# guanjq/targetdiff

Hardware: NVIDIA H100
Metric: molecules/sec (1000-step sampling, CrossDocked pocket shape) (higher is better)
Workload: dtype f32 (storage, LayerNorm, softmax, accumulation); GEMM operands as 2-piece bf16 splits on wgmma (3 products, ~16-bit operand mantissa)

## Files before the change

include/tdiff.h:

```cpp
#ifndef TDIFF_H_
#define TDIFF_H_

#include <stddef.h>
#include <stdint.h>

#ifdef __cplusplus
extern "C" {
#endif

#if defined(__GNUC__)
#define TDIFF_API __attribute__((visibility("default")))
#else
#define TDIFF_API
#endif

#define TDIFF_OK 0
#define TDIFF_EINVAL (-1)
#define TDIFF_ECUDA (-2)
#define TDIFF_ESTATE (-3)
#define TDIFF_EWEIGHT (-4)

typedef struct tdiff_engine tdiff_engine;

typedef struct tdiff_config {
  int32_t hidden_dim;
  int32_t n_heads;
  int32_t num_layers;
  int32_t knn;
  int32_t num_r_gaussian;
  int32_t num_classes;
  int32_t protein_feat_dim;
  int32_t num_timesteps;
  int32_t model_mean_type;
  int32_t num_blocks;
  int32_t ew_net_type;
  int32_t x2h_out_fc;
  int32_t time_emb;
  int32_t cutoff_mode;
  int32_t sublayers;
  int32_t reserved[1];
} tdiff_config;

typedef struct tdiff_tensor {
  const char* name;
  const float* data;
  int64_t numel;
} tdiff_tensor;

TDIFF_API int tdiff_create(const tdiff_config* cfg, const tdiff_tensor* h_state_dict, int n_entries, int device, tdiff_engine** out);
TDIFF_API void tdiff_destroy(tdiff_engine* e);
TDIFF_API const char* tdiff_last_error(void);
TDIFF_API const char* tdiff_version(void);

TDIFF_API int tdiff_bind_batch(tdiff_engine* e, int n_graphs, const int32_t* h_protein_counts, const int32_t* h_ligand_counts,
                     const float* d_protein_pos, const float* d_protein_feat, int center_mode, void* stream);

TDIFF_API int tdiff_set_ligand(tdiff_engine* e, const float* d_ligand_pos, const int64_t* d_ligand_v, int apply_center, void* stream);
TDIFF_API int tdiff_get_ligand(tdiff_engine* e, float* d_ligand_pos, int64_t* d_ligand_v, int add_offset, void* stream);
TDIFF_API int tdiff_get_offset(tdiff_engine* e, float* d_offset, void* stream);

TDIFF_API int tdiff_set_time(tdiff_engine* e, const float* d_time_norm, void* stream);

TDIFF_API int tdiff_forward(tdiff_engine* e, float* d_pred_pos, float* d_pred_logits, float* d_final_h, int fix_x, void* stream);

TDIFF_API int tdiff_forward_blocks(tdiff_engine* e, float* d_pred_pos, float* d_pred_logits, float* d_final_h, int fix_x, float* d_block_pos,
                                   float* d_block_logits, void* stream);

TDIFF_API int64_t tdiff_num_edges(tdiff_engine* e, void* stream);
TDIFF_API int tdiff_get_edge_index(tdiff_engine* e, int64_t* d_edge_index, void* stream);
TDIFF_API int tdiff_get_edge_weight(tdiff_engine* e, float* d_e_w, void* stream);
TDIFF_API int tdiff_get_node_pos(tdiff_engine* e, float* d_x, void* stream);

TDIFF_API int tdiff_sample(tdiff_engine* e, int num_steps, const float* d_pos_noise, const float* d_v_uniform, uint64_t seed,
                 float* d_pos_traj, int64_t* d_v_traj, float* d_v0_traj, float* d_vt_traj, int pos_only, void* stream);

TDIFF_API int tdiff_set_fixed(tdiff_engine* e, const uint8_t* d_mask, const float* d_pos0, const int64_t* d_v0, int apply_center,
                              void* stream);
TDIFF_API int tdiff_set_fixed_tape(tdiff_engine* e, const float* d_pos_noise, const float* d_v_uniform);

TDIFF_API int tdiff_sample_seq(tdiff_engine* e, const int32_t* h_time_seq, int num_steps, const float* d_pos_noise, const float* d_v_uniform,
                               uint64_t seed, float* d_pos_traj, int64_t* d_v_traj, float* d_v0_traj, float* d_vt_traj, int pos_only,
                               void* stream);

TDIFF_API int tdiff_set_start(tdiff_engine* e, int t_start, const float* d_pos_noise, const float* d_v_uniform);

TDIFF_API int tdiff_likelihood_terms(tdiff_engine* e, const int32_t* h_time_steps, const uint32_t* h_keys, const float* d_pos_noise,
                                     const float* d_v_uniform, uint64_t seed, float* d_kl_pos, float* d_kl_v, float* d_prior_pos,
                                     float* d_prior_v, float* d_atom_kl_pos, float* d_atom_kl_v, float* d_xt, int64_t* d_vt, void* stream);

TDIFF_API int tdiff_sample_host(tdiff_engine* e, int n_graphs, const int32_t* h_protein_counts, const int32_t* h_ligand_counts,
                      const float* h_protein_pos, const float* h_protein_feat, const float* h_ligand_pos,
                      const int64_t* h_ligand_v, int center_mode, int num_steps, const float* h_pos_noise,
                      const float* h_v_uniform, uint64_t seed, float* h_out_pos, int64_t* h_out_v, float* h_pos_traj,
                      int64_t* h_v_traj, float* h_v0_traj, float* h_vt_traj, int pos_only, void* stream);

TDIFF_API int tdiff_knn_graph(const float* d_x, int n_nodes, const int32_t* h_graph_counts, int n_graphs, int k,
                    int32_t* d_src_slots, int64_t* d_edge_index, int64_t* h_n_edges, void* stream);

TDIFF_API int tdiff_attn_aggregate_h(const float* d_k, const float* d_v, const float* d_e_w, const int32_t* d_src_slots,
                           const float* d_q, const float* d_h_in, float* d_h_out, int n_nodes, int kk, void* stream);
TDIFF_API int tdiff_attn_aggregate_x(const float* d_k, const float* d_v16, const float* d_e_w, const int32_t* d_src_slots,
                           const float* d_q, const float* d_x, const uint8_t* d_mask, float* d_x_out, int n_nodes, int kk,
                           void* stream);
TDIFF_API int tdiff_scatter_mean3(const float* d_src, const int32_t* h_counts, int n_segments, float* d_out, void* stream);

TDIFF_API int tdiff_check_stability(const float* d_pos, const int32_t* d_atomic_num, const int32_t* h_counts, int n_mol, int hs,
                                    int32_t* d_nr_bonds, int32_t* d_stable_atoms, uint8_t* d_mol_stable, void* stream);

TDIFF_API int64_t tdiff_launch_count(tdiff_engine* e);
TDIFF_API int tdiff_edge_mlp_mode(tdiff_engine* e);
TDIFF_API int tdiff_profile(tdiff_engine* e, int enable);
TDIFF_API int tdiff_profile_read(tdiff_engine* e, double* ms_aggregate_h, int64_t* n_aggregate_h, double* ms_aggregate_x,
                       int64_t* n_aggregate_x, double* ms_edge_mlp, int64_t* n_edge_mlp, double* ms_total);

#ifdef __cplusplus
}
#endif
#endif
```

targetdiff_b200/_lib.py:

```python
import ctypes
import os

_HERE = os.path.dirname(os.path.abspath(__file__))
LIB_PATH = os.environ.get('TDIFF_LIB') or os.path.join(_HERE, 'libtdiff.so')

TDIFF_OK, TDIFF_EINVAL, TDIFF_ECUDA, TDIFF_ESTATE, TDIFF_EWEIGHT = 0, -1, -2, -3, -4


class TdiffError(RuntimeError):
    def __init__(self, code, msg):
        super().__init__('libtdiff error %d: %s' % (code, msg))
        self.code = code


class tdiff_config(ctypes.Structure):
    _fields_ = [('hidden_dim', ctypes.c_int32), ('n_heads', ctypes.c_int32), ('num_layers', ctypes.c_int32), ('knn', ctypes.c_int32),
                ('num_r_gaussian', ctypes.c_int32), ('num_classes', ctypes.c_int32), ('protein_feat_dim', ctypes.c_int32),
                ('num_timesteps', ctypes.c_int32), ('model_mean_type', ctypes.c_int32), ('num_blocks', ctypes.c_int32),
                ('ew_net_type', ctypes.c_int32), ('x2h_out_fc', ctypes.c_int32), ('time_emb', ctypes.c_int32), ('cutoff_mode', ctypes.c_int32),
                ('sublayers', ctypes.c_int32), ('reserved', ctypes.c_int32 * 1)]


class tdiff_tensor(ctypes.Structure):
    _fields_ = [('name', ctypes.c_char_p), ('data', ctypes.c_void_p), ('numel', ctypes.c_int64)]


_vp, _i, _i64, _u64 = ctypes.c_void_p, ctypes.c_int, ctypes.c_int64, ctypes.c_uint64
_pi32 = ctypes.POINTER(ctypes.c_int32)

SIGNATURES = {
    'tdiff_create': (_i, [ctypes.POINTER(tdiff_config), ctypes.POINTER(tdiff_tensor), _i, _i, ctypes.POINTER(_vp)]),
    'tdiff_destroy': (None, [_vp]),
    'tdiff_last_error': (ctypes.c_char_p, []),
    'tdiff_version': (ctypes.c_char_p, []),
    'tdiff_bind_batch': (_i, [_vp, _i, _pi32, _pi32, _vp, _vp, _i, _vp]),
    'tdiff_set_ligand': (_i, [_vp, _vp, _vp, _i, _vp]),
    'tdiff_get_ligand': (_i, [_vp, _vp, _vp, _i, _vp]),
    'tdiff_get_offset': (_i, [_vp, _vp, _vp]),
    'tdiff_set_time': (_i, [_vp, _vp, _vp]),
    'tdiff_forward': (_i, [_vp, _vp, _vp, _vp, _i, _vp]),
    'tdiff_forward_blocks': (_i, [_vp, _vp, _vp, _vp, _i, _vp, _vp, _vp]),
    'tdiff_num_edges': (_i64, [_vp, _vp]),
    'tdiff_get_edge_index': (_i, [_vp, _vp, _vp]),
    'tdiff_get_edge_weight': (_i, [_vp, _vp, _vp]),
    'tdiff_get_node_pos': (_i, [_vp, _vp, _vp]),
    'tdiff_sample': (_i, [_vp, _i, _vp, _vp, _u64, _vp, _vp, _vp, _vp, _i, _vp]),
    'tdiff_set_fixed': (_i, [_vp, _vp, _vp, _vp, _i, _vp]),
    'tdiff_set_fixed_tape': (_i, [_vp, _vp, _vp]),
    'tdiff_sample_seq': (_i, [_vp, _pi32, _i, _vp, _vp, _u64, _vp, _vp, _vp, _vp, _i, _vp]),
    'tdiff_set_start': (_i, [_vp, _i, _vp, _vp]),
    'tdiff_likelihood_terms': (_i, [_vp, _pi32, ctypes.POINTER(ctypes.c_uint32), _vp, _vp, _u64, _vp, _vp, _vp, _vp, _vp, _vp, _vp, _vp, _vp]),
    'tdiff_sample_host': (_i, [_vp, _i, _pi32, _pi32, _vp, _vp, _vp, _vp, _i, _i, _vp, _vp, _u64, _vp, _vp, _vp, _vp, _vp, _vp, _i, _vp]),
    'tdiff_knn_graph': (_i, [_vp, _i, _pi32, _i, _i, _vp, _vp, ctypes.POINTER(_i64), _vp]),
    'tdiff_attn_aggregate_h': (_i, [_vp, _vp, _vp, _vp, _vp, _vp, _vp, _i, _i, _vp]),
    'tdiff_attn_aggregate_x': (_i, [_vp, _vp, _vp, _vp, _vp, _vp, _vp, _vp, _i, _i, _vp]),
    'tdiff_scatter_mean3': (_i, [_vp, _pi32, _i, _vp, _vp]),
    'tdiff_check_stability': (_i, [_vp, _vp, _pi32, _i, _i, _vp, _vp, _vp, _vp]),
    'tdiff_launch_count': (_i64, [_vp]),
    'tdiff_edge_mlp_mode': (_i, [_vp]),
    'tdiff_profile': (_i, [_vp, _i]),
    'tdiff_profile_read': (_i, [_vp, ctypes.POINTER(ctypes.c_double), ctypes.POINTER(_i64), ctypes.POINTER(ctypes.c_double),
                                ctypes.POINTER(_i64), ctypes.POINTER(ctypes.c_double), ctypes.POINTER(_i64), ctypes.POINTER(ctypes.c_double)]),
}

_lib = None


def load():
    global _lib
    if _lib is not None:
        return _lib
    if not os.path.exists(LIB_PATH):
        raise RuntimeError('%s not found: build it with `python -m targetdiff_b200.build` (nvcc, sm_90a). '
                           'targetdiff_b200 has no CPU / PyTorch fallback.' % LIB_PATH)
    lib = ctypes.CDLL(LIB_PATH)
    for name, (res, args) in SIGNATURES.items():
        fn = getattr(lib, name)
        fn.restype = res
        fn.argtypes = args
    _lib = lib
    return lib


def last_error():
    return load().tdiff_last_error().decode('utf-8', 'replace')


def check(rc):
    if rc != TDIFF_OK:
        raise TdiffError(rc, last_error())


def i32_array(values):
    arr = (ctypes.c_int32 * len(values))(*[int(v) for v in values])
    return arr
```

targetdiff_b200/csrc/aggregate.cu:

```cuda
#include "tdiff_common.cuh"

#define AGG_WARPS 8
#define AGG_CH 8

__device__ __forceinline__ float4 ldg_stream4(const float* p) {
  float4 r;
  asm volatile("ld.global.nc.L1::no_allocate.v4.f32 {%0,%1,%2,%3}, [%4];" : "=f"(r.x), "=f"(r.y), "=f"(r.z), "=f"(r.w) : "l"(p));
  return r;
}

__device__ __forceinline__ float head_logit(const float4& q, const float4& k) {
  const float s8 = 2.8284271247461903f;
  float s = (__fdiv_rn(q.x * k.x, s8) + __fdiv_rn(q.y * k.y, s8)) + (__fdiv_rn(q.z * k.z, s8) + __fdiv_rn(q.w * k.w, s8));
  return s + __shfl_xor_sync(0xffffffffu, s, 1);
}

__global__ void __launch_bounds__(AGG_WARPS * 32)
aggregate_h_kernel(const float* __restrict__ kbuf, const float* __restrict__ vbuf, const float* __restrict__ e_w,
                   const int* __restrict__ src, const float* __restrict__ q, const float* __restrict__ h_in,
                   float* __restrict__ h_out, int n_nodes, int k) {
  const int lane = threadIdx.x & 31;
  const int n = blockIdx.x * AGG_WARPS + (threadIdx.x >> 5);
  if (n >= n_nodes) return;
  const size_t e0 = (size_t)n * k;
  int deg = 0;
  for (int j = lane; j < k; j += 32) deg += (src[e0 + j] >= 0);
  deg = __reduce_add_sync(0xffffffffu, deg);
  const float4 q4 = *reinterpret_cast<const float4*>(q + (size_t)n * TD_H + 4 * lane);
  const float4 hin = *reinterpret_cast<const float4*>(h_in + (size_t)n * TD_H + 4 * lane);
  float m = -INFINITY, l = 0.0f;
  float4 acc = make_float4(0.f, 0.f, 0.f, 0.f);
  for (int j0 = 0; j0 < deg; j0 += AGG_CH) {
    float4 kr[AGG_CH], vr[AGG_CH];
    float ew[AGG_CH];
#pragma unroll
    for (int c = 0; c < AGG_CH; ++c) {
      if (j0 + c < deg) {
        kr[c] = ldg_stream4(kbuf + (e0 + j0 + c) * TD_H + 4 * lane);
        vr[c] = ldg_stream4(vbuf + (e0 + j0 + c) * TD_H + 4 * lane);
        ew[c] = e_w[e0 + j0 + c];
      }
    }
#pragma unroll
    for (int c = 0; c < AGG_CH; ++c) {
      if (j0 + c < deg) {
        const float s = head_logit(q4, kr[c]);
        const float mn = fmaxf(m, s);
        const float sc = expf(m - mn);
        const float p = expf(s - mn);
        const float pw = p * ew[c];
        l = l * sc + p;
        acc.x = acc.x * sc + pw * vr[c].x;
        acc.y = acc.y * sc + pw * vr[c].y;
        acc.z = acc.z * sc + pw * vr[c].z;
        acc.w = acc.w * sc + pw * vr[c].w;
        m = mn;
      }
    }
  }
  float4 o = hin;
  if (deg > 0) {
    o.x += acc.x / l; o.y += acc.y / l; o.z += acc.z / l; o.w += acc.w / l;
  }
  *reinterpret_cast<float4*>(h_out + (size_t)n * TD_H + 4 * lane) = o;
}

void td_launch_aggregate_h(const float* kbuf, const float* vbuf, const float* e_w, const int* src, const float* q, const float* h_in,
                           float* h_out, int n_nodes, int k, cudaStream_t st) {
  if (n_nodes == 0) return;
  aggregate_h_kernel<<<(n_nodes + AGG_WARPS - 1) / AGG_WARPS, AGG_WARPS * 32, 0, st>>>(kbuf, vbuf, e_w, src, q, h_in, h_out, n_nodes, k);
}

__global__ void __launch_bounds__(AGG_WARPS * 32)
aggregate_x_kernel(const float* __restrict__ kbuf, const float* __restrict__ v16, const float* __restrict__ e_w,
                   const int* __restrict__ src, const float* __restrict__ q, const float4* __restrict__ xm_in,
                   const int* __restrict__ row_nodes, float4* __restrict__ xm_out, int n_rows, int k) {
  const int lane = threadIdx.x & 31;
  const int a = blockIdx.x * AGG_WARPS + (threadIdx.x >> 5);
  if (a >= n_rows) return;
  const int n = row_nodes ? row_nodes[a] : a;
  const size_t e0 = (size_t)n * k;
  const size_t r0 = (size_t)a * k;
  int deg = 0;
  for (int j = lane; j < k; j += 32) deg += (src[e0 + j] >= 0);
  deg = __reduce_add_sync(0xffffffffu, deg);
  const float4 q4 = *reinterpret_cast<const float4*>(q + (size_t)n * TD_H + 4 * lane);
  const float4 xd = xm_in[n];
  float m = -INFINITY, l = 0.0f;
  float ax = 0.f, ay = 0.f, az = 0.f;
  for (int j0 = 0; j0 < deg; j0 += AGG_CH) {
    float4 kr[AGG_CH];
    float vv[AGG_CH];
    float4 xs[AGG_CH];
#pragma unroll
    for (int c = 0; c < AGG_CH; ++c) {
      if (j0 + c < deg) {
        kr[c] = ldg_stream4(kbuf + (r0 + j0 + c) * TD_H + 4 * lane);
        vv[c] = v16[(r0 + j0 + c) * TD_HEADS + (lane >> 1)] * e_w[e0 + j0 + c];
        xs[c] = xm_in[src[e0 + j0 + c]];
      }
    }
#pragma unroll
    for (int c = 0; c < AGG_CH; ++c) {
      if (j0 + c < deg) {
        const float s = head_logit(q4, kr[c]);
        const float mn = fmaxf(m, s);
        const float sc = expf(m - mn);
        const float p = expf(s - mn);
        const float pv = p * vv[c];
        l = l * sc + p;
        ax = ax * sc + pv * (xd.x - xs[c].x);
        ay = ay * sc + pv * (xd.y - xs[c].y);
        az = az * sc + pv * (xd.z - xs[c].z);
        m = mn;
      }
    }
  }
  float dx = 0.f, dy = 0.f, dz = 0.f;
  if (deg > 0) {
    const float w = (lane & 1) ? 0.0f : 1.0f / l;
    dx = warp_sum(ax * w) * (1.0f / TD_HEADS);
    dy = warp_sum(ay * w) * (1.0f / TD_HEADS);
    dz = warp_sum(az * w) * (1.0f / TD_HEADS);
  }
  if (lane == 0) xm_out[n] = make_float4(xd.x + dx * xd.w, xd.y + dy * xd.w, xd.z + dz * xd.w, xd.w);
}

void td_launch_aggregate_x(const float* kbuf, const float* v16, const float* e_w, const int* src, const float* q, const float4* xm_in,
                           const int* row_nodes, float4* xm_out, int n_rows, int k, cudaStream_t st) {
  if (n_rows == 0) return;
  aggregate_x_kernel<<<(n_rows + AGG_WARPS - 1) / AGG_WARPS, AGG_WARPS * 32, 0, st>>>(kbuf, v16, e_w, src, q, xm_in, row_nodes, xm_out,
                                                                                   n_rows, k);
}

__global__ void __launch_bounds__(AGG_WARPS * 32)
aggregate_h_logits_kernel(const float* __restrict__ logits, const float* __restrict__ vbuf, const float* __restrict__ e_w,
                          const int* __restrict__ src, const float* __restrict__ h_in, float* __restrict__ h_out, int n_nodes, int k,
                          const float* __restrict__ ewm_w, float ewm_b) {
  const int lane = threadIdx.x & 31;
  const int n = blockIdx.x * AGG_WARPS + (threadIdx.x >> 5);
  if (n >= n_nodes) return;
  const size_t e0 = (size_t)n * k;
  int deg = 0;
  for (int j = lane; j < k; j += 32) deg += (src[e0 + j] >= 0);
  deg = __reduce_add_sync(0xffffffffu, deg);
  const float4 hin = *reinterpret_cast<const float4*>(h_in + (size_t)n * TD_H + 4 * lane);
  float4 wm = make_float4(0.f, 0.f, 0.f, 0.f);
  if (ewm_w) wm = *reinterpret_cast<const float4*>(ewm_w + 4 * lane);
  float m = -INFINITY, l = 0.0f;
  float4 acc = make_float4(0.f, 0.f, 0.f, 0.f);
  for (int j0 = 0; j0 < deg; j0 += AGG_CH) {
    float4 vr[AGG_CH];
    float ew[AGG_CH], sg[AGG_CH];
#pragma unroll
    for (int c = 0; c < AGG_CH; ++c) {
      if (j0 + c < deg) {
        vr[c] = ldg_stream4(vbuf + (e0 + j0 + c) * TD_H + 4 * lane);
        sg[c] = logits[(e0 + j0 + c) * TD_HEADS + (lane >> 1)];
        ew[c] = e_w[e0 + j0 + c];
      }
    }
    if (ewm_w) {
#pragma unroll
      for (int c = 0; c < AGG_CH; ++c) {
        if (j0 + c < deg) {
          const float dot = warp_sum((vr[c].x * wm.x + vr[c].y * wm.y) + (vr[c].z * wm.z + vr[c].w * wm.w));
          ew[c] = 1.0f / (1.0f + expf(-(dot + ewm_b)));
        }
      }
    }
#pragma unroll
    for (int c = 0; c < AGG_CH; ++c) {
      if (j0 + c < deg) {
        const float s = sg[c];
        const float mn = fmaxf(m, s);
        const float sc = expf(m - mn);
        const float p = expf(s - mn);
        const float pw = p * ew[c];
        l = l * sc + p;
        acc.x = acc.x * sc + pw * vr[c].x;
        acc.y = acc.y * sc + pw * vr[c].y;
        acc.z = acc.z * sc + pw * vr[c].z;
        acc.w = acc.w * sc + pw * vr[c].w;
        m = mn;
      }
    }
  }
  float4 o = hin;
  if (deg > 0) {
    o.x += acc.x / l; o.y += acc.y / l; o.z += acc.z / l; o.w += acc.w / l;
  }
  *reinterpret_cast<float4*>(h_out + (size_t)n * TD_H + 4 * lane) = o;
}

void td_launch_aggregate_h_logits(const float* logits, const float* vbuf, const float* e_w, const int* src, const float* h_in, float* h_out,
                                  int n_nodes, int k, const float* ewm_w, float ewm_b, cudaStream_t st) {
  if (n_nodes == 0) return;
  aggregate_h_logits_kernel<<<(n_nodes + AGG_WARPS - 1) / AGG_WARPS, AGG_WARPS * 32, 0, st>>>(logits, vbuf, e_w, src, h_in, h_out, n_nodes, k,
                                                                                             ewm_w, ewm_b);
}

__global__ void __launch_bounds__(AGG_WARPS * 32)
aggregate_x_logits_kernel(const float* __restrict__ logits, const float* __restrict__ v16, const float* __restrict__ e_w,
                          const int* __restrict__ src, const float4* __restrict__ xm_in, const int* __restrict__ row_nodes,
                          float4* __restrict__ xm_out, int n_rows, int k) {
  const int lane = threadIdx.x & 31;
  const int a = blockIdx.x * AGG_WARPS + (threadIdx.x >> 5);
  if (a >= n_rows) return;
  const int n = row_nodes ? row_nodes[a] : a;
  const size_t e0 = (size_t)n * k, r0 = (size_t)a * k;
  int deg = 0;
  for (int j = lane; j < k; j += 32) deg += (src[e0 + j] >= 0);
  deg = __reduce_add_sync(0xffffffffu, deg);
  const float4 xd = xm_in[n];
  float m = -INFINITY, l = 0.0f;
  float ax = 0.f, ay = 0.f, az = 0.f;
  for (int j = 0; j < deg; ++j) {
    const float s = logits[(r0 + j) * TD_HEADS + (lane >> 1)];
    const float vv = v16[(r0 + j) * TD_HEADS + (lane >> 1)] * e_w[e0 + j];
    const float4 xs = xm_in[src[e0 + j]];
    const float mn = fmaxf(m, s);
    const float sc = expf(m - mn);
    const float p = expf(s - mn);
    const float pv = p * vv;
    l = l * sc + p;
    ax = ax * sc + pv * (xd.x - xs.x);
    ay = ay * sc + pv * (xd.y - xs.y);
    az = az * sc + pv * (xd.z - xs.z);
    m = mn;
  }
  float dx = 0.f, dy = 0.f, dz = 0.f;
  if (deg > 0) {
    const float w = (lane & 1) ? 0.0f : 1.0f / l;
    dx = warp_sum(ax * w) * (1.0f / TD_HEADS);
    dy = warp_sum(ay * w) * (1.0f / TD_HEADS);
    dz = warp_sum(az * w) * (1.0f / TD_HEADS);
  }
  if (lane == 0) xm_out[n] = make_float4(xd.x + dx * xd.w, xd.y + dy * xd.w, xd.z + dz * xd.w, xd.w);
}

void td_launch_aggregate_x_logits(const float* logits, const float* v16, const float* e_w, const int* src, const float4* xm_in,
                                  const int* row_nodes, float4* xm_out, int n_rows, int k, cudaStream_t st) {
  if (n_rows == 0) return;
  aggregate_x_logits_kernel<<<(n_rows + AGG_WARPS - 1) / AGG_WARPS, AGG_WARPS * 32, 0, st>>>(logits, v16, e_w, src, xm_in, row_nodes, xm_out,
                                                                                          n_rows, k);
}
```

targetdiff_b200/csrc/edge_const.cu:

```cuda
#include "tdiff_common.cuh"

#define EC_WARPS 8

__global__ void __launch_bounds__(EC_WARPS * 32)
edge_touch_kernel(const float4* __restrict__ xm, const int* __restrict__ src, int* __restrict__ src_prev, int have_prev, int n_nodes, int k,
                  unsigned char* __restrict__ rel_flag, unsigned char* __restrict__ touch_flag, unsigned char* __restrict__ etype,
                  int* __restrict__ work_list, int* __restrict__ n_work) {
  const int lane = threadIdx.x & 31;
  const int warp0 = blockIdx.x * EC_WARPS + (threadIdx.x >> 5), nwarps = gridDim.x * EC_WARPS;
  for (int node = warp0; node < n_nodes; node += nwarps) {
    const size_t e0 = (size_t)node * k;
    const float4 xd = xm[node];
    bool same = have_prev != 0, touch = xd.w != 0.0f;
    unsigned keep_mask = 0;
    for (int j = lane; j < k; j += 32) {
      const int s = src[e0 + j];
      bool slot_same = false;
      if (src_prev) {
        slot_same = have_prev != 0 && src_prev[e0 + j] == s;
        same = same && slot_same;
        src_prev[e0 + j] = s;
      }
      const bool s_lig = s >= 0 && xm[s].w != 0.0f;
      if (slot_same && !s_lig && xd.w == 0.0f) keep_mask |= 1u << (j >> 5);
      touch = touch || s_lig;
      if (rel_flag && xd.w != 0.0f && s >= 0) rel_flag[s] = 1;
    }
    if (rel_flag && xd.w != 0.0f && lane == 0) rel_flag[node] = 1;
    same = __all_sync(0xffffffffu, same);
    touch = __any_sync(0xffffffffu, touch);
    if (touch_flag && lane == 0) touch_flag[node] = touch ? 1 : 0;
    if (same && !touch) continue;
    if (etype)
      for (int j = lane; j < k; j += 32)
        if (keep_mask & (1u << (j >> 5))) etype[e0 + j] |= 0x80;
    if (lane == 0) work_list[atomicAdd(n_work, 1)] = node;
  }
}

__global__ void __launch_bounds__(EC_WARPS * 32)
edge_gate_kernel(const float4* __restrict__ xm, const int* __restrict__ src, const int* __restrict__ work_list, const int* __restrict__ n_work,
                 int k, const float* __restrict__ offsets, float coeff, const float* __restrict__ w1t, const float* __restrict__ b1,
                 const float* __restrict__ ln_g, const float* __restrict__ ln_b, const float* __restrict__ w2, float b2,
                 unsigned char* __restrict__ etype, float* __restrict__ e_w, int gate_mode, int honour_keep) {
  __shared__ float s_w1t[TD_NG * TD_H];
  __shared__ float s_b1[TD_H], s_g[TD_H], s_b[TD_H], s_w2[TD_H];
  for (int i = threadIdx.x; i < TD_NG * TD_H; i += blockDim.x) s_w1t[i] = w1t[i];
  for (int i = threadIdx.x; i < TD_H; i += blockDim.x) {
    s_b1[i] = b1[i]; s_g[i] = ln_g[i]; s_b[i] = ln_b[i]; s_w2[i] = w2[i];
  }
  __syncthreads();
  const int lane = threadIdx.x & 31;
  const float mu = offsets[lane < TD_NG ? lane : 0];
  const long long warp0 = (long long)blockIdx.x * EC_WARPS + (threadIdx.x >> 5), nwarps = (long long)gridDim.x * EC_WARPS;
  const long long n_items = (long long)(*n_work) * k;
  for (long long item = warp0; item < n_items; item += nwarps) {
    const int node = work_list[item / k];
    const size_t e = (size_t)node * k + (size_t)(item % k);
    const unsigned char keep = honour_keep ? etype[e] : 0;
    if (keep & 0x80) {
      if (lane == 0) etype[e] = keep & 0x7f;
      continue;
    }
    const int s = src[e];
    if (s < 0) {
      if (lane == 0) { etype[e] = 3; e_w[e] = 0.0f; }
      continue;
    }
    const float4 xd = xm[node], xs = xm[s];
    if (gate_mode != 0) {
      if (lane == 0) {
        const bool ns = xs.w != 0.0f, nd = xd.w != 0.0f;
        etype[e] = (unsigned char)(ns ? (nd ? 0 : 1) : (nd ? 2 : 3));
        e_w[e] = 1.0f;
      }
      continue;
    }
    const float dx = xd.x - xs.x, dy = xd.y - xs.y, dz = xd.z - xs.z;
    const float dist = sqrtf(dx * dx + dy * dy + dz * dz);
    const float t = dist - mu;
    const float gj = expf(coeff * (t * t));
    float p[4];
#pragma unroll
    for (int c = 0; c < 4; ++c) p[c] = s_b1[lane + 32 * c];
#pragma unroll
    for (int jj = 0; jj < TD_NG; ++jj) {
      const float g = __shfl_sync(0xffffffffu, gj, jj);
#pragma unroll
      for (int c = 0; c < 4; ++c) p[c] = fmaf(g, s_w1t[jj * TD_H + lane + 32 * c], p[c]);
    }
    ln_relu_128(p, s_g, s_b, lane);
    float acc = (p[0] * s_w2[lane] + p[1] * s_w2[lane + 32]) + (p[2] * s_w2[lane + 64] + p[3] * s_w2[lane + 96]);
    acc = warp_sum(acc) + b2;
    if (lane == 0) {
      const bool ns = xs.w != 0.0f, nd = xd.w != 0.0f;
      const int ty = ns ? (nd ? 0 : 1) : (nd ? 2 : 3);
      etype[e] = (unsigned char)ty;
      e_w[e] = 1.0f / (1.0f + expf(-acc));
    }
  }
}

void td_launch_edge_const(const float4* xm, const int* src, int* src_prev, int have_prev, int n_nodes, int k, const float* offsets, float coeff,
                          const float* w1t, const float* b1, const float* ln_g, const float* ln_b, const float* w2, float b2,
                          unsigned char* etype, float* e_w, unsigned char* rel_flag, unsigned char* touch_flag, int* work_list, int* n_work,
                          int gate_mode, cudaStream_t st) {
  if (n_nodes == 0) return;
  int blocks = (n_nodes + EC_WARPS - 1) / EC_WARPS;
  if (blocks > 148 * 8) blocks = 148 * 8;
  if (rel_flag) cudaMemsetAsync(rel_flag, 0, (size_t)n_nodes, st);
  cudaMemsetAsync(n_work, 0, sizeof(int), st);
  edge_touch_kernel<<<blocks, EC_WARPS * 32, 0, st>>>(xm, src, src_prev, have_prev, n_nodes, k, rel_flag, touch_flag, (gate_mode & 2) ? nullptr : etype,
                                                      work_list, n_work);
  edge_gate_kernel<<<148 * 8, EC_WARPS * 32, 0, st>>>(xm, src, work_list, n_work, k, offsets, coeff, w1t, b1, ln_g, ln_b, w2, b2, etype, e_w, gate_mode & 1,
                                                     (have_prev && !(gate_mode & 2)) ? 1 : 0);
}

__global__ void edge_geom_kernel(const float4* __restrict__ xm, const int* __restrict__ src, const unsigned char* __restrict__ etype, long long n_slots,
                                 int k, float* __restrict__ dist, TdEwR ew) {
  const long long e = (long long)blockIdx.x * blockDim.x + threadIdx.x;
  if (e >= n_slots) return;
  const int s = src[e];
  float d = 0.0f;
  if (s >= 0) {
    const float4 xd = xm[e / k], xs = xm[s];
    const float dx = xd.x - xs.x, dy = xd.y - xs.y, dz = xd.z - xs.z;
    d = sqrtf(dx * dx + dy * dy + dz * dz);
  }
  dist[e] = d;
  if (ew.w_x2h) {
    float ax = ew.b_x2h, ah = ew.b_h2x;
    if (s >= 0) {
      const int ty = etype[e];
#pragma unroll 4
      for (int j = 0; j < TD_NG; ++j) {
        const float t = d - ew.offsets[j];
        const float g = expf(ew.coeff * (t * t));
        ax = fmaf(g, ew.w_x2h[ty * TD_NG + j], ax);
        ah = fmaf(g, ew.w_h2x[ty * TD_NG + j], ah);
      }
    }
    ew.out_x2h[e] = s >= 0 ? 1.0f / (1.0f + expf(-ax)) : 0.0f;
    ew.out_h2x[e] = s >= 0 ? 1.0f / (1.0f + expf(-ah)) : 0.0f;
  }
}

void td_launch_edge_geom(const float4* xm, const int* src, const unsigned char* etype, int n_nodes, int k, float* dist, const TdEwR& ew, cudaStream_t st) {
  const long long n = (long long)n_nodes * k;
  if (n > 0) edge_geom_kernel<<<(int)((n + 255) / 256), 256, 0, st>>>(xm, src, etype, n, k, dist, ew);
}

__global__ void edge_geom_rows_kernel(const float4* __restrict__ xm, const int* __restrict__ src, const unsigned char* __restrict__ etype,
                                      const int* __restrict__ rows, long long n_slots, int k, float* __restrict__ dist,
                                      const float* __restrict__ gate_w, float gate_b, const float* __restrict__ offsets, float coeff,
                                      float* __restrict__ gate) {
  const long long t = (long long)blockIdx.x * blockDim.x + threadIdx.x;
  if (t >= n_slots) return;
  const long long e = (long long)rows[t / k] * k + t % k;
  const int s = src[e];
  float d = 0.0f;
  if (s >= 0) {
    const float4 xd = xm[e / k], xs = xm[s];
    const float dx = xd.x - xs.x, dy = xd.y - xs.y, dz = xd.z - xs.z;
    d = sqrtf(dx * dx + dy * dy + dz * dz);
  }
  dist[e] = d;
  if (gate_w) {
    float a = gate_b;
    if (s >= 0) {
      const int ty = etype[e];
#pragma unroll 4
      for (int j = 0; j < TD_NG; ++j) {
        const float u = d - offsets[j];
        a = fmaf(expf(coeff * (u * u)), gate_w[ty * TD_NG + j], a);
      }
    }
    gate[e] = s >= 0 ? 1.0f / (1.0f + expf(-a)) : 0.0f;
  }
}

void td_launch_edge_geom_rows(const float4* xm, const int* src, const unsigned char* etype, const int* rows, int n_rows, int k, float* dist,
                              const float* gate_w, float gate_b, const float* offsets, float coeff, float* gate, cudaStream_t st) {
  const long long n = (long long)n_rows * k;
  if (n > 0) edge_geom_rows_kernel<<<(int)((n + 255) / 256), 256, 0, st>>>(xm, src, etype, rows, n, k, dist, gate_w, gate_b, offsets, coeff, gate);
}

__global__ void rel_compact_kernel(const unsigned char* __restrict__ flag, int n_nodes, int* __restrict__ rel_list, int* __restrict__ n_rel) {
  const int i = blockIdx.x * blockDim.x + threadIdx.x;
  if (i < n_nodes && flag[i]) rel_list[atomicAdd(n_rel, 1)] = i;
}
void td_launch_rel_compact(const unsigned char* flag, int n_nodes, int* rel_list, int* n_rel, cudaStream_t st) {
  if (n_nodes == 0) return;
  cudaMemsetAsync(n_rel, 0, sizeof(int), st);
  rel_compact_kernel<<<(n_nodes + 255) / 256, 256, 0, st>>>(flag, n_nodes, rel_list, n_rel);
}

__global__ void rel_rows_protein_kernel(const unsigned char* __restrict__ flag, const float4* __restrict__ xm, int n_nodes, int* __restrict__ rel_rows,
                                        int* __restrict__ rel_counts) {
  const int i = blockIdx.x * blockDim.x + threadIdx.x;
  if (i < n_nodes && flag[i] && xm[i].w == 0.0f) rel_rows[atomicAdd(&rel_counts[2], 1)] = i;
}
__global__ void rel_rows_finish_kernel(const int* __restrict__ lig_rows, int n_lig_rows, int pad, int* __restrict__ rel_rows, int* __restrict__ rel_counts) {
  const int n_p = rel_counts[2], n_pp = (n_p + pad - 1) / pad * pad;
  const int i = blockIdx.x * blockDim.x + threadIdx.x;
  if (i < n_pp - n_p) rel_rows[n_p + i] = -1;
  if (i < n_lig_rows) rel_rows[n_pp + i] = lig_rows[i];
  if (i == 0) { rel_counts[0] = n_pp + n_lig_rows; rel_counts[1] = n_pp; }
}
void td_launch_rel_rows(const unsigned char* rel_flag, const float4* xm, int n_nodes, const int* lig_rows, int n_lig_rows, int pad, int* rel_rows,
                        int* rel_counts, cudaStream_t st) {
  cudaMemsetAsync(rel_counts, 0, 4 * sizeof(int), st);
  if (n_nodes > 0) rel_rows_protein_kernel<<<(n_nodes + 255) / 256, 256, 0, st>>>(rel_flag, xm, n_nodes, rel_rows, rel_counts);
  const int n = n_lig_rows > pad ? n_lig_rows : pad;
  rel_rows_finish_kernel<<<(n + 255) / 256, 256, 0, st>>>(lig_rows, n_lig_rows, pad, rel_rows, rel_counts);
}

__global__ void dirty_propagate_kernel(const unsigned char* __restrict__ in, const int* __restrict__ src, int n_nodes, int k, unsigned char* __restrict__ out) {
  const int lane = threadIdx.x & 31;
  const int node = blockIdx.x * (blockDim.x >> 5) + (threadIdx.x >> 5);
  if (node >= n_nodes) return;
  bool d = in[node] != 0;
  for (int j = lane; j < k && !d; j += 32) {
    const int s = src[(size_t)node * k + j];
    if (s >= 0 && in[s]) d = true;
  }
  d = __any_sync(0xffffffffu, d);
  if (lane == 0) out[node] = d ? 1 : 0;
}
void td_launch_dirty_propagate(const unsigned char* in, const int* src, int n_nodes, int k, unsigned char* out, cudaStream_t st) {
  if (n_nodes > 0) dirty_propagate_kernel<<<(n_nodes + 7) / 8, 256, 0, st>>>(in, src, n_nodes, k, out);
}
__global__ void restore_clean_kernel(const unsigned char* __restrict__ dirty, const float4* __restrict__ xm, const float* __restrict__ h_free, int n_nodes,
                                     float* __restrict__ h) {
  const int lane = threadIdx.x & 31;
  const int node = blockIdx.x * (blockDim.x >> 5) + (threadIdx.x >> 5);
  if (node >= n_nodes || dirty[node] || xm[node].w != 0.0f) return;
  reinterpret_cast<float4*>(h + (size_t)node * TD_H)[lane] = reinterpret_cast<const float4*>(h_free + (size_t)node * TD_H)[lane];
}
void td_launch_restore_clean(const unsigned char* dirty, const float4* xm, const float* h_free, int n_nodes, float* h, cudaStream_t st) {
  if (n_nodes > 0) restore_clean_kernel<<<(n_nodes + 7) / 8, 256, 0, st>>>(dirty, xm, h_free, n_nodes, h);
}
```

targetdiff_b200/csrc/engine.cu:

```cuda
#include <math.h>
#include <stdarg.h>
#include <stdio.h>
#include <stdlib.h>
#include <string.h>

#include <list>
#include <map>
#include <string>
#include <vector>

#include "../../include/tdiff.h"
#include "sampler.cuh"
#include "tdiff_common.cuh"

static thread_local char g_err[1024] = "";
static int set_err(int code, const char* fmt, ...) {
  va_list ap;
  va_start(ap, fmt);
  vsnprintf(g_err, sizeof(g_err), fmt, ap);
  va_end(ap);
  return code;
}
#define CK(call)                                                                                       \
  do {                                                                                                 \
    cudaError_t _e = (call);                                                                           \
    if (_e != cudaSuccess) return set_err(TDIFF_ECUDA, "%s failed: %s (%s:%d)", #call, cudaGetErrorString(_e), __FILE__, __LINE__); \
  } while (0)

struct DevBuf {
  void* p = nullptr;
  size_t cap = 0;
  int ensure(size_t bytes) {
    if (bytes <= cap) return 0;
    if (p) cudaFree(p);
    p = nullptr; cap = 0;
    size_t want = bytes + bytes / 8 + 256;
    if (cudaMalloc(&p, want) != cudaSuccess) { (void)cudaGetLastError(); if (cudaMalloc(&p, bytes) != cudaSuccess) { (void)cudaGetLastError(); return -1; } want = bytes; }
    cap = want;
    static const bool poison = getenv("TDIFF_POISON") != nullptr;
    if (poison) {
      cudaMemset(p, 0xFF, want);
      cudaDeviceSynchronize();
    }
    return 0;
  }
  void release() { if (p) cudaFree(p); p = nullptr; cap = 0; }
  template <class T> T* as() const { return reinterpret_cast<T*>(p); }
};

struct TdLayer {
  std::vector<TdSubLayer> x2h, h2x;
  const float* offsets;
  float coeff;
};

enum { EV_AGG_H = 0, EV_AGG_X = 1, EV_EDGE_MLP = 2, EV_TOTAL = 3, EV_KINDS = 4 };
struct EvPair { cudaEvent_t a, b; int kind; };

struct tdiff_engine {
  tdiff_config cfg;
  int device = 0, sm_count = 132;
  float* arena = nullptr;
  std::vector<float> host_arena;
  unsigned char* img_arena = nullptr;
  int mlp_mode = 2;
  bool mlp_v4 = true;
  std::vector<TdLayer> layers;
  const float *w_prot = nullptr, *b_prot = nullptr, *wl_t = nullptr, *bl = nullptr;
  const float *ew_w1t = nullptr, *ew_b1 = nullptr, *ew_g = nullptr, *ew_b = nullptr, *ew_w2 = nullptr, *ew_off = nullptr;
  float ew_b2 = 0.f, ew_coeff = -0.5f;
  int num_blocks = 1, ew_mode = 0 , out_fc = 0, time_emb = 0;
  int num_x2h = 1, num_h2x = 1, sync_twoup = 0;
  const float* w_time = nullptr;
  const float* zeros128 = nullptr;
  DevBuf ew_x2h, ew_h2x, hagg, time_norm;
  DevBuf h_sync;
  const float *hd_w1t = nullptr, *hd_b1 = nullptr, *hd_w2 = nullptr, *hd_b2 = nullptr;
  const float *t_c0 = nullptr, *t_ct = nullptr, *t_logvar = nullptr, *t_la = nullptr, *t_l1ma = nullptr, *t_lca = nullptr, *t_l1mca = nullptr,
              *t_sra = nullptr, *t_srm1 = nullptr, *t_ac = nullptr;
  bool bound = false, has_ligand = false, have_graph = false;
  bool restrict_last = false;
  bool knn_incremental = false;
  bool have_prev = false;
  bool env_no_fused_agg = false, env_no_restrict = false, env_no_graph = false, env_knn_full = false, env_no_slot_keep = false;
  int B = 0, N = 0, Np = 0, Nl = 0, K = 0, max_ng = 0, final_buf = 0;
  int KQ = 0, hybrid = 0;
  DevBuf node_ptr, prot_ptr, prot_node, prot_graph, lig_node, lig_graph, node_lig;
  DevBuf rel_flag, rel_list, n_rel, work_list, n_work, knn_cache;
  DevBuf x2h_rows, lig_rows, rel_rows, rel_counts;
  long long x2h_n_dst = 0, x2h_split = 0, lig_n_dst = 0;
  int row_pad = 4;
  int free_depth = 0;
  int env_free_depth = 2;
  bool free_ready = false;
  DevBuf h_free, dirty, free_rows, free_counts, lig_save;
  long long free_stride = 0;
  DevBuf xm0, xm1, offset, h0, h, P, q, src, src_prev, etype, e_w, dist, kbuf, vbuf, v16, lig_pos, lig_v, logits;
  DevBuf step, err_flag, node_off, total_edges;
  bool has_fixed = false;
  DevBuf fix_mask, fix_pos, fix_v;
  const float *fix_pos_noise = nullptr, *fix_v_uniform = nullptr;
  int start_t = -1;
  const float *start_pos_noise = nullptr, *start_v_uniform = nullptr;
  std::vector<double> cum_log_a, cum_log_av;
  DevBuf seq_buf;
  DevBuf lk_buf, lk_x0, lk_v0;
  std::vector<int32_t> lk_host;
  DevBuf stage[8];
  cudaStream_t own_stream = nullptr;
  cudaEvent_t ev_fork = nullptr, ev_join = nullptr;
  long long launches = 0;
  bool profiling = false;
  std::vector<EvPair> events;
  double ms_acc[EV_KINDS] = {0, 0, 0, 0};
  long long n_acc[EV_KINDS] = {0, 0, 0, 0};
};

namespace {
struct Packer {
  std::map<std::string, const tdiff_tensor*> byname;
  std::vector<float> host;
  std::vector<unsigned char> img;
  std::string missing;
  std::list<std::vector<float>> keep;
  const float* get(const std::string& name, int64_t numel) {
    auto it = byname.find(name);
    if (it == byname.end() || it->second->numel != numel || it->second->data == nullptr) {
      if (missing.empty()) missing = name + (it == byname.end() ? " (absent)" : " (wrong size)");
      return nullptr;
    }
    return it->second->data;
  }
  size_t alloc(size_t n) {
    size_t off = (host.size() + 63) / 64 * 64;
    host.resize(off + n, 0.0f);
    return off;
  }
};

struct MlpOff { size_t tab, ln_g, ln_b, w2t, b2; int nout; long long img, tabcls; };

inline uint16_t bf16_rn(float x) {
  uint32_t u; memcpy(&u, &x, 4);
  if ((u & 0x7fffffffu) > 0x7f800000u) return (uint16_t)((u >> 16) | 0x40);
  u += 0x7fffu + ((u >> 16) & 1u);
  return (uint16_t)(u >> 16);
}
inline float bf16_f(uint16_t b) { uint32_t u = (uint32_t)b << 16; float f; memcpy(&f, &u, 4); return f; }

void pack_umma_image(const float* w2, std::vector<unsigned char>& img, size_t off, int nrows = 128) {
  for (int n = 0; n < nrows; ++n)
    for (int kk = 0; kk < 128; ++kk) {
      float r = w2[(size_t)n * 128 + kk];
      const size_t o = (size_t)(kk / 64) * ((size_t)nrows * 128) + (size_t)n * 128 + (size_t)((((kk % 64) / 8) ^ (n & 7)) * 16) + (size_t)(kk % 8) * 2;
      for (int p = 0; p < 3; ++p) {
        const uint16_t b = bf16_rn(r);
        r = r - bf16_f(b);
        memcpy(&img[off + (size_t)p * ((size_t)nrows * 256) + o], &b, 2);
      }
    }
}

void pack_tabcls_image(const float* tab , std::vector<unsigned char>& img, size_t off) {
  static const int type_of[2][2] = {{3, 1}, {2, 0}};
  for (int cls = 0; cls < 2; ++cls)
    for (int n = 0; n < 128; ++n)
      for (int slot = 0; slot < 64; ++slot) {
        const int half = slot >> 5, sl = slot & 31;
        const int q = (sl & 7) >> 1, m = 2 * (sl >> 3) + (sl & 1);
        int j = -1;
        if (m < 5) j = 5 * q + m;
        else if (m == 5 && q == 3) j = 20;
        float r = j >= 0 ? tab[((size_t)type_of[cls][half] * TD_TAB + j) * TD_H + n] : 0.0f;
        const size_t o = (size_t)n * 128 + (size_t)(((slot >> 3) ^ (n & 7)) * 16) + (size_t)(slot & 7) * 2;
        for (int p = 0; p < 2; ++p) {
          const uint16_t b = bf16_rn(r);
          r = r - bf16_f(b);
          memcpy(&img[off + (size_t)cls * 32768 + (size_t)p * 16384 + o], &b, 2);
        }
      }
}

bool pack_edge_mlp(Packer& pk, const std::string& p, int nout, bool sign_in_w1, MlpOff& o, const float** w1_out) {
  const int KV = 4 + 4 * TD_NG + 2 * TD_H;
  const float* w1_in = pk.get(p + ".net.0.weight", (int64_t)TD_H * KV);
  const float* b1_in = pk.get(p + ".net.0.bias", TD_H);
  const float* g_in = pk.get(p + ".net.1.weight", TD_H);
  const float* b_in = pk.get(p + ".net.1.bias", TD_H);
  const float* w2_in = pk.get(p + ".net.3.weight", (int64_t)nout * TD_H);
  const float* b2_in = pk.get(p + ".net.3.bias", nout);
  if (!w1_in || !b1_in || !g_in || !b_in || !w2_in || !b2_in) return false;
  std::vector<float>& w1v = pk.keep.emplace_back((size_t)TD_H * KV);
  std::vector<float> b1v(TD_H), gv(TD_H), bv(TD_H), w2v((size_t)nout * TD_H), b2v(nout);
  {
    std::vector<double> mw(KV, 0.0), b2acc(b2_in, b2_in + nout);
    double mb = 0.0;
    for (int f = 0; f < TD_H; ++f) {
      for (int j = 0; j < KV; ++j) mw[j] += w1_in[(size_t)f * KV + j];
      mb += b1_in[f];
    }
    for (int f = 0; f < TD_H; ++f) {
      const double s = g_in[f] < 0.0f ? -1.0 : 1.0, ag = fabs((double)g_in[f]), s1 = sign_in_w1 ? s : 1.0;
      for (int j = 0; j < KV; ++j) w1v[(size_t)f * KV + j] = (float)(s1 * (w1_in[(size_t)f * KV + j] - mw[j] / TD_H));
      b1v[f] = (float)(s1 * (b1_in[f] - mb / TD_H));
      gv[f] = (float)(s / s1);
      const float bf = (float)(b_in[f] / ag);
      const bool constant = g_in[f] == 0.0f || !isfinite(bf);
      bv[f] = constant ? 0.0f : bf;
      for (int n = 0; n < nout; ++n) {
        const double w = w2_in[(size_t)n * TD_H + f];
        w2v[(size_t)n * TD_H + f] = constant ? 0.0f : (float)(ag * w);
        if (constant && b_in[f] > 0.0f) b2acc[n] += (double)b_in[f] * w;
      }
    }
    for (int n = 0; n < nout; ++n) b2v[n] = (float)b2acc[n];
  }
  const float *w1 = w1v.data(), *b1 = b1v.data(), *g = gv.data(), *b = bv.data(), *w2 = w2v.data(), *b2 = b2v.data();
  o.nout = nout;
  o.tab = pk.alloc(4 * TD_TAB * TD_H);
  for (int t = 0; t < 4; ++t) {
    for (int j = 0; j < TD_NG; ++j)
      for (int f = 0; f < TD_H; ++f) pk.host[o.tab + (t * TD_TAB + j) * TD_H + f] = w1[(size_t)f * KV + 4 + t * TD_NG + j];
    for (int f = 0; f < TD_H; ++f) pk.host[o.tab + (t * TD_TAB + TD_NG) * TD_H + f] = w1[(size_t)f * KV + t] + b1[f];
  }
  o.ln_g = pk.alloc(TD_H); memcpy(&pk.host[o.ln_g], g, TD_H * sizeof(float));
  o.ln_b = pk.alloc(TD_H); memcpy(&pk.host[o.ln_b], b, TD_H * sizeof(float));
  o.w2t = pk.alloc((size_t)TD_H * nout);
  for (int kk = 0; kk < TD_H; ++kk)
    for (int n = 0; n < nout; ++n) pk.host[o.w2t + (size_t)kk * nout + n] = w2[(size_t)n * TD_H + kk];
  o.b2 = pk.alloc(nout); memcpy(&pk.host[o.b2], b2, nout * sizeof(float));
  o.img = -1; o.tabcls = -1;
  if (nout == TD_H || nout == 16) {
    o.img = (long long)pk.img.size();
    pk.img.resize(pk.img.size() + 3 * (size_t)nout * 256, 0);
    pack_umma_image(w2, pk.img, (size_t)o.img, nout);
    o.tabcls = (long long)pk.img.size();
    pk.img.resize(pk.img.size() + 2 * 32768, 0);
    pack_tabcls_image(&pk.host[o.tab], pk.img, (size_t)o.tabcls);
  }
  *w1_out = w1;
  return true;
}

struct SubOff {
  size_t wn_t, bn; long long wn_img; MlpOff k, v, q;
  long long ew_w = -1; float ew_b = 0.f;
  long long out_wa = -1, out_wb = -1, out_w2 = -1, out_b1 = -1, out_g = -1, out_b = -1, out_b2 = -1;
};

bool pack_sublayer_options(Packer& pk, const std::string& p, int ew_dim, bool out_fc, SubOff& so) {
  if (ew_dim > 0) {
    const float* w = pk.get(p + ".ew_net.0.weight", ew_dim);
    const float* b = pk.get(p + ".ew_net.0.bias", 1);
    if (!w || !b) return false;
    so.ew_w = (long long)pk.alloc(ew_dim);
    memcpy(&pk.host[so.ew_w], w, ew_dim * sizeof(float));
    so.ew_b = b[0];
  }
  if (out_fc) {
    const std::string np = p + ".node_output";
    const float* w1 = pk.get(np + ".net.0.weight", (int64_t)TD_H * 2 * TD_H);
    const float* b1 = pk.get(np + ".net.0.bias", TD_H);
    const float* g = pk.get(np + ".net.1.weight", TD_H);
    const float* b = pk.get(np + ".net.1.bias", TD_H);
    const float* w2 = pk.get(np + ".net.3.weight", (int64_t)TD_H * TD_H);
    const float* b2 = pk.get(np + ".net.3.bias", TD_H);
    if (!w1 || !b1 || !g || !b || !w2 || !b2) return false;
    std::vector<float> blk((size_t)TD_H * TD_H);
    for (int half = 0; half < 2; ++half) {
      for (int n = 0; n < TD_H; ++n)
        for (int kk = 0; kk < TD_H; ++kk) blk[(size_t)n * TD_H + kk] = w1[(size_t)n * 2 * TD_H + half * TD_H + kk];
      long long& dst = half == 0 ? so.out_wa : so.out_wb;
      dst = (long long)pk.img.size();
      pk.img.resize(pk.img.size() + 3 * 32768, 0);
      pack_umma_image(blk.data(), pk.img, (size_t)dst);
    }
    so.out_w2 = (long long)pk.img.size();
    pk.img.resize(pk.img.size() + 3 * 32768, 0);
    pack_umma_image(w2, pk.img, (size_t)so.out_w2);
    so.out_b1 = (long long)pk.alloc(TD_H); memcpy(&pk.host[so.out_b1], b1, TD_H * 4);
    so.out_g = (long long)pk.alloc(TD_H); memcpy(&pk.host[so.out_g], g, TD_H * 4);
    so.out_b = (long long)pk.alloc(TD_H); memcpy(&pk.host[so.out_b], b, TD_H * 4);
    so.out_b2 = (long long)pk.alloc(TD_H); memcpy(&pk.host[so.out_b2], b2, TD_H * 4);
  }
  return true;
}

bool pack_sublayer(Packer& pk, const std::string& p, const char* kn, const char* vn, const char* qn, int nout_v, bool sign_in_w1, SubOff& so) {
  const int KV = 4 + 4 * TD_NG + 2 * TD_H;
  const float *w1k = nullptr, *w1v = nullptr;
  if (!pack_edge_mlp(pk, p + "." + kn, TD_H, sign_in_w1, so.k, &w1k)) return false;
  if (!pack_edge_mlp(pk, p + "." + vn, nout_v, sign_in_w1, so.v, &w1v)) return false;
  const std::string qp = p + "." + qn;
  const float* w1q = pk.get(qp + ".net.0.weight", (int64_t)TD_H * TD_H);
  const float* b1q = pk.get(qp + ".net.0.bias", TD_H);
  const float* gq = pk.get(qp + ".net.1.weight", TD_H);
  const float* bq = pk.get(qp + ".net.1.bias", TD_H);
  const float* w2q = pk.get(qp + ".net.3.weight", (int64_t)TD_H * TD_H);
  const float* b2q = pk.get(qp + ".net.3.bias", TD_H);
  if (!w1q || !b1q || !gq || !bq || !w2q || !b2q) return false;
  so.q.nout = TD_H; so.q.tab = 0; so.q.tabcls = -1;
  so.q.img = (long long)pk.img.size();
  pk.img.resize(pk.img.size() + 3 * 32768, 0);
  pack_umma_image(w2q, pk.img, (size_t)so.q.img);
  so.q.ln_g = pk.alloc(TD_H); memcpy(&pk.host[so.q.ln_g], gq, TD_H * sizeof(float));
  so.q.ln_b = pk.alloc(TD_H); memcpy(&pk.host[so.q.ln_b], bq, TD_H * sizeof(float));
  so.q.w2t = pk.alloc((size_t)TD_H * TD_H);
  for (int kk = 0; kk < TD_H; ++kk)
    for (int n = 0; n < TD_H; ++n) pk.host[so.q.w2t + (size_t)kk * TD_H + n] = w2q[(size_t)n * TD_H + kk];
  so.q.b2 = pk.alloc(TD_H); memcpy(&pk.host[so.q.b2], b2q, TD_H * sizeof(float));
  so.wn_t = pk.alloc((size_t)TD_H * TD_NPROJ);
  so.bn = pk.alloc(TD_NPROJ);
  for (int kk = 0; kk < TD_H; ++kk) {
    float* row = &pk.host[so.wn_t + (size_t)kk * TD_NPROJ];
    for (int c = 0; c < TD_H; ++c) {
      row[c] = w1k[(size_t)c * KV + 4 + 4 * TD_NG + kk];
      row[128 + c] = w1v[(size_t)c * KV + 4 + 4 * TD_NG + kk];
      row[256 + c] = w1k[(size_t)c * KV + 4 + 4 * TD_NG + TD_H + kk];
      row[384 + c] = w1v[(size_t)c * KV + 4 + 4 * TD_NG + TD_H + kk];
      row[512 + c] = w1q[(size_t)c * TD_H + kk];
    }
  }
  for (int c = 0; c < TD_H; ++c) pk.host[so.bn + 512 + c] = b1q[c];
  so.wn_img = (long long)pk.img.size();
  pk.img.resize(pk.img.size() + 5 * 3 * 32768, 0);
  std::vector<float> blk((size_t)TD_H * TD_H);
  for (int y = 0; y < 5; ++y) {
    for (int n = 0; n < TD_H; ++n)
      for (int kk = 0; kk < TD_H; ++kk) blk[(size_t)n * TD_H + kk] = pk.host[so.wn_t + (size_t)kk * TD_NPROJ + y * TD_H + n];
    pack_umma_image(blk.data(), pk.img, (size_t)so.wn_img + (size_t)y * 3 * 32768);
  }
  return true;
}

TdMlp mk_mlp(const float* base, const unsigned char* img_base, const MlpOff& o, int offA, int offB) {
  TdMlp m;
  m.w2_img = (o.img >= 0 && img_base) ? img_base + o.img : nullptr;
  m.tabcls_img = (o.tabcls >= 0 && img_base) ? img_base + o.tabcls : nullptr;
  m.tab = base + o.tab; m.ln_g = base + o.ln_g; m.ln_b = base + o.ln_b; m.w2t = base + o.w2t; m.b2 = base + o.b2;
  m.nout = o.nout; m.offA = offA; m.offB = offB;
  return m;
}
}

extern "C" const char* tdiff_last_error(void) { return g_err; }
extern "C" const char* tdiff_version(void) { return "tdiff-b200 0.1 (sm_90a)"; }

extern "C" int tdiff_create(const tdiff_config* cfg, const tdiff_tensor* sd, int n_entries, int device, tdiff_engine** out) {
  if (!cfg || !sd || !out) return set_err(TDIFF_EINVAL, "null argument");
  *out = nullptr;
  if (cfg->hidden_dim != TD_H || cfg->n_heads != TD_HEADS || cfg->num_r_gaussian != TD_NG)
    return set_err(TDIFF_EINVAL, "unsupported model shape: hidden_dim=%d n_heads=%d num_r_gaussian=%d (kernels are built for 128/16/20)",
                   cfg->hidden_dim, cfg->n_heads, cfg->num_r_gaussian);
  if (cfg->knn < 1 || cfg->knn > TD_KMAX) return set_err(TDIFF_EINVAL, "knn=%d outside 1..%d", cfg->knn, TD_KMAX);
  if (cfg->model_mean_type != 0 && cfg->model_mean_type != 1)
    return set_err(TDIFF_EINVAL, "model_mean_type=%d (0 = C0, 1 = noise)", cfg->model_mean_type);
  for (int r : cfg->reserved)
    if (r != 0) return set_err(TDIFF_EINVAL, "tdiff_config.reserved must be 0");
  int num_x2h = 1, num_h2x = 1, sync_twoup = 0;
  if (cfg->sublayers != 0) {
    const unsigned s = (unsigned)cfg->sublayers;
    num_x2h = (int)(s & 0xffu); num_h2x = (int)((s >> 8) & 0xffu); sync_twoup = (int)((s >> 16) & 0xffu);
    if ((s >> 24) != 1u || num_x2h > 16 || num_h2x > 16 || sync_twoup > 1)
      return set_err(TDIFF_EINVAL, "sublayers=0x%08x: expected 0 or 1<<24 | sync_twoup<<16 | num_h2x<<8 | num_x2h with num_x2h, num_h2x in 0..16 and "
                     "sync_twoup in 0..1", s);
  }
  if (cfg->cutoff_mode != 0 && cfg->cutoff_mode != 1) return set_err(TDIFF_EINVAL, "cutoff_mode=%d (0 = 'knn', 1 = 'hybrid')", cfg->cutoff_mode);
  if (cfg->num_blocks < 0 || cfg->num_blocks > 16 || cfg->ew_net_type < 0 || cfg->ew_net_type > 3 || (cfg->x2h_out_fc != 0 && cfg->x2h_out_fc != 1) ||
      (cfg->time_emb != 0 && cfg->time_emb != 1))
    return set_err(TDIFF_EINVAL, "bad option (num_blocks=%d ew_net_type=%d x2h_out_fc=%d time_emb=%d)", cfg->num_blocks, cfg->ew_net_type,
                   cfg->x2h_out_fc, cfg->time_emb);
  if (cfg->num_layers < 1 || cfg->num_classes < 1 || cfg->num_classes > TD_CMAX || cfg->protein_feat_dim < 1 || cfg->num_timesteps < 1)
    return set_err(TDIFF_EINVAL, "bad config (num_layers=%d num_classes=%d protein_feat_dim=%d num_timesteps=%d)", cfg->num_layers,
                   cfg->num_classes, cfg->protein_feat_dim, cfg->num_timesteps);
  int ndev = 0;
  if (cudaGetDeviceCount(&ndev) != cudaSuccess || ndev == 0) {
    (void)cudaGetLastError();
    return set_err(TDIFF_ECUDA, "no CUDA device: libtdiff has no CPU fallback");
  }
  if (device < 0 || device >= ndev) return set_err(TDIFF_EINVAL, "device %d out of range (%d devices)", device, ndev);
  CK(cudaSetDevice(device));
  cudaDeviceProp prop;
  CK(cudaGetDeviceProperties(&prop, device));
  if (prop.major != 9) return set_err(TDIFF_ECUDA, "device %d is sm_%d%d; this library is built for sm_90a only", device, prop.major, prop.minor);

  tdiff_engine* e = new tdiff_engine();
  e->cfg = *cfg; e->device = device; e->sm_count = prop.multiProcessorCount; e->K = e->KQ = cfg->knn; e->hybrid = cfg->cutoff_mode;
  e->num_blocks = cfg->num_blocks > 1 ? cfg->num_blocks : 1; e->ew_mode = cfg->ew_net_type; e->out_fc = cfg->x2h_out_fc; e->time_emb = cfg->time_emb;
  e->num_x2h = num_x2h; e->num_h2x = num_h2x; e->sync_twoup = sync_twoup;
  if (const char* mode = getenv("TDIFF_EDGE_MLP")) {
    if (!strcmp(mode, "simt")) e->mlp_mode = 0;
    else if (!strcmp(mode, "tc3")) e->mlp_mode = 2;
    else if (!strcmp(mode, "tc3v2")) { e->mlp_mode = 2; e->mlp_v4 = false; }
    else if (!strcmp(mode, "tc6")) e->mlp_mode = 3;
    else { delete e; return set_err(TDIFF_EINVAL, "TDIFF_EDGE_MLP=%s (simt|tc3|tc3v2|tc6)", mode); }
  }
  const bool v4 = e->mlp_mode == 2 && e->mlp_v4;

  Packer pk;
  for (int i = 0; i < n_entries; ++i)
    if (sd[i].name) pk.byname[sd[i].name] = &sd[i];
  const int T = cfg->num_timesteps, KC = cfg->num_classes, F = cfg->protein_feat_dim, L = cfg->num_layers;
  struct { const char* name; size_t off; } tabs[10] = {{"posterior_mean_c0_coef", 0}, {"posterior_mean_ct_coef", 0}, {"posterior_logvar", 0},
      {"log_alphas_v", 0}, {"log_one_minus_alphas_v", 0}, {"log_alphas_cumprod_v", 0}, {"log_one_minus_alphas_cumprod_v", 0},
      {"sqrt_recip_alphas_cumprod", 0}, {"sqrt_recipm1_alphas_cumprod", 0}, {"alphas_cumprod", 0}};
  for (auto& t : tabs) {
    const float* p = pk.get(t.name, T);
    t.off = pk.alloc(T);
    if (p) memcpy(&pk.host[t.off], p, T * sizeof(float));
  }
  const float *betas = pk.get("betas", T), *la_v = pk.get("log_alphas_v", T);
  if (betas && la_v) {
    e->cum_log_a.resize(T); e->cum_log_av.resize(T);
    double sa = 0.0, sv = 0.0;
    for (int i = 0; i < T; ++i) {
      sa += log1p(-(double)betas[i]); e->cum_log_a[i] = sa;
      sv += (double)la_v[i]; e->cum_log_av[i] = sv;
    }
  }
  const float* wp = pk.get("protein_atom_emb.weight", (int64_t)(TD_H - 1) * F);
  const float* bp = pk.get("protein_atom_emb.bias", TD_H - 1);
  const int KIN = KC + (cfg->time_emb ? 1 : 0);
  const float* wl = pk.get("ligand_atom_emb.weight", (int64_t)(TD_H - 1) * KIN);
  const float* blp = pk.get("ligand_atom_emb.bias", TD_H - 1);
  size_t o_wp = pk.alloc((size_t)TD_H * F), o_bp = pk.alloc(TD_H), o_wl = pk.alloc((size_t)KC * TD_H), o_bl = pk.alloc(TD_H),
         o_wtime = pk.alloc(TD_H), o_zeros = pk.alloc(TD_H);
  if (wp && bp && wl && blp) {
    memcpy(&pk.host[o_wp], wp, (size_t)(TD_H - 1) * F * sizeof(float));
    memcpy(&pk.host[o_bp], bp, (TD_H - 1) * sizeof(float));
    for (int v = 0; v < KC; ++v)
      for (int f = 0; f < TD_H - 1; ++f) pk.host[o_wl + (size_t)v * TD_H + f] = wl[(size_t)f * KIN + v];
    if (cfg->time_emb)
      for (int f = 0; f < TD_H - 1; ++f) pk.host[o_wtime + f] = wl[(size_t)f * KIN + KC];
    memcpy(&pk.host[o_bl], blp, (TD_H - 1) * sizeof(float));
  }
  const bool has_gate = cfg->ew_net_type == 0;
  const float* gw1 = has_gate ? pk.get("refine_net.edge_pred_layer.net.0.weight", (int64_t)TD_H * TD_NG) : nullptr;
  const float* gb1 = has_gate ? pk.get("refine_net.edge_pred_layer.net.0.bias", TD_H) : nullptr;
  const float* gg = has_gate ? pk.get("refine_net.edge_pred_layer.net.1.weight", TD_H) : nullptr;
  const float* gb = has_gate ? pk.get("refine_net.edge_pred_layer.net.1.bias", TD_H) : nullptr;
  const float* gw2 = has_gate ? pk.get("refine_net.edge_pred_layer.net.3.weight", TD_H) : nullptr;
  const float* gb2 = has_gate ? pk.get("refine_net.edge_pred_layer.net.3.bias", 1) : nullptr;
  const float* goff = pk.get("refine_net.distance_expansion.offset", TD_NG);
  size_t o_gw1 = pk.alloc((size_t)TD_NG * TD_H), o_gb1 = pk.alloc(TD_H), o_gg = pk.alloc(TD_H), o_gb = pk.alloc(TD_H), o_gw2 = pk.alloc(TD_H),
         o_goff = pk.alloc(TD_NG);
  if (goff) memcpy(&pk.host[o_goff], goff, TD_NG * 4);
  if (gw1 && gb1 && gg && gb && gw2 && gb2 && goff) {
    for (int j = 0; j < TD_NG; ++j)
      for (int f = 0; f < TD_H; ++f) pk.host[o_gw1 + (size_t)j * TD_H + f] = gw1[(size_t)f * TD_NG + j];
    memcpy(&pk.host[o_gb1], gb1, TD_H * 4); memcpy(&pk.host[o_gg], gg, TD_H * 4); memcpy(&pk.host[o_gb], gb, TD_H * 4);
    memcpy(&pk.host[o_gw2], gw2, TD_H * 4); memcpy(&pk.host[o_goff], goff, TD_NG * 4);
    e->ew_b2 = gb2[0];
    const float d = goff[1] - goff[0];
    e->ew_coeff = -0.5f / (d * d);
  }
  const float* hw1 = pk.get("v_inference.0.weight", (int64_t)TD_H * TD_H);
  const float* hb1 = pk.get("v_inference.0.bias", TD_H);
  const float* hw2 = pk.get("v_inference.2.weight", (int64_t)KC * TD_H);
  const float* hb2 = pk.get("v_inference.2.bias", KC);
  size_t o_hw1 = pk.alloc((size_t)TD_H * TD_H), o_hb1 = pk.alloc(TD_H), o_hw2 = pk.alloc((size_t)KC * TD_H), o_hb2 = pk.alloc(KC);
  if (hw1 && hb1 && hw2 && hb2) {
    for (int kk = 0; kk < TD_H; ++kk)
      for (int n = 0; n < TD_H; ++n) pk.host[o_hw1 + (size_t)kk * TD_H + n] = hw1[(size_t)n * TD_H + kk];
    memcpy(&pk.host[o_hb1], hb1, TD_H * 4); memcpy(&pk.host[o_hw2], hw2, (size_t)KC * TD_H * 4); memcpy(&pk.host[o_hb2], hb2, KC * 4);
  }
  std::vector<std::vector<SubOff>> sx(L, std::vector<SubOff>(num_x2h)), sh(L, std::vector<SubOff>(num_h2x));
  std::vector<size_t> o_off(L);
  std::vector<float> coeffs(L, -0.5f);
  for (int l = 0; l < L; ++l) {
    const std::string p = "refine_net.base_block." + std::to_string(l);
    bool ok = true;
    for (int i = 0; ok && i < num_x2h; ++i) ok = pack_sublayer(pk, p + ".x2h_layers." + std::to_string(i), "hk_func", "hv_func", "hq_func", TD_H, v4, sx[l][i]);
    for (int i = 0; ok && i < num_h2x; ++i) ok = pack_sublayer(pk, p + ".h2x_layers." + std::to_string(i), "xk_func", "xv_func", "xq_func", TD_HEADS, v4, sh[l][i]);
    for (int i = 0; ok && i < num_x2h; ++i)
      ok = pack_sublayer_options(pk, p + ".x2h_layers." + std::to_string(i), cfg->ew_net_type == 1 ? 4 * TD_NG : cfg->ew_net_type == 2 ? TD_H : 0,
                                 cfg->x2h_out_fc != 0, sx[l][i]);
    for (int i = 0; ok && i < num_h2x; ++i)
      ok = pack_sublayer_options(pk, p + ".h2x_layers." + std::to_string(i), cfg->ew_net_type == 1 ? 4 * TD_NG : 0, false, sh[l][i]);
    if (!ok) break;
    const float* off = pk.get(p + ".distance_expansion.offset", TD_NG);
    o_off[l] = pk.alloc(TD_NG);
    if (off) {
      memcpy(&pk.host[o_off[l]], off, TD_NG * 4);
      const float d = off[1] - off[0];
      coeffs[l] = -0.5f / (d * d);
    }
  }
  if (!pk.missing.empty()) {
    delete e;
    return set_err(TDIFF_EWEIGHT, "state_dict entry %s", pk.missing.c_str());
  }
  const size_t bytes = pk.host.size() * sizeof(float);
  if (cudaMalloc(&e->arena, bytes) != cudaSuccess) { delete e; return set_err(TDIFF_ECUDA, "cudaMalloc(%zu) for weights failed", bytes); }
  if (cudaMemcpy(e->arena, pk.host.data(), bytes, cudaMemcpyHostToDevice) != cudaSuccess) {
    cudaFree(e->arena); delete e; return set_err(TDIFF_ECUDA, "weight upload failed");
  }
  if (!pk.img.empty()) {
    if (cudaMalloc(&e->img_arena, pk.img.size()) != cudaSuccess ||
        cudaMemcpy(e->img_arena, pk.img.data(), pk.img.size(), cudaMemcpyHostToDevice) != cudaSuccess) {
      cudaFree(e->arena); delete e; return set_err(TDIFF_ECUDA, "weight image upload failed");
    }
  }
  if ((cfg->ew_net_type != 0 || cfg->x2h_out_fc || cfg->cutoff_mode != 0) && !(e->mlp_mode == 2 && e->mlp_v4)) {
    cudaFree(e->arena); cudaFree(e->img_arena); delete e;
    return set_err(TDIFF_EINVAL, "ew_net_type != 'global', x2h_out_fc and cutoff_mode 'hybrid' are implemented (and tested) in the default engine mode only (unset TDIFF_EDGE_MLP)");
  }
  if (cfg->sublayers != 0 && !(num_x2h == 1 && num_h2x == 1 && !sync_twoup) && !(e->mlp_mode == 2 && e->mlp_v4)) {
    cudaFree(e->arena); cudaFree(e->img_arena); delete e;
    return set_err(TDIFF_EINVAL, "num_x2h / num_h2x != 1 and sync_twoup are implemented (and tested) in the default engine mode only (unset TDIFF_EDGE_MLP)");
  }
  e->env_no_fused_agg = getenv("TDIFF_NO_FUSED_AGG") != nullptr;
  e->env_no_restrict = getenv("TDIFF_NO_RESTRICT") != nullptr;
  e->env_no_graph = getenv("TDIFF_NO_GRAPH") != nullptr;
  e->env_knn_full = getenv("TDIFF_KNN_FULL") != nullptr;
  e->env_no_slot_keep = getenv("TDIFF_NO_SLOT_KEEP") != nullptr;
  if (const char* fd = getenv("TDIFF_FREE_DEPTH")) e->env_free_depth = atoi(fd) < 0 ? 0 : (atoi(fd) > 8 ? 8 : atoi(fd));
  e->host_arena = pk.host;
  const float* A = e->arena;
  const unsigned char* IM = e->img_arena;
  e->t_c0 = A + tabs[0].off; e->t_ct = A + tabs[1].off; e->t_logvar = A + tabs[2].off; e->t_la = A + tabs[3].off;
  e->t_l1ma = A + tabs[4].off; e->t_lca = A + tabs[5].off; e->t_l1mca = A + tabs[6].off;
  e->t_sra = A + tabs[7].off; e->t_srm1 = A + tabs[8].off; e->t_ac = A + tabs[9].off;
  e->w_prot = A + o_wp; e->b_prot = A + o_bp; e->wl_t = A + o_wl; e->bl = A + o_bl;
  e->w_time = cfg->time_emb ? A + o_wtime : nullptr; e->zeros128 = A + o_zeros;
  e->ew_w1t = A + o_gw1; e->ew_b1 = A + o_gb1; e->ew_g = A + o_gg; e->ew_b = A + o_gb; e->ew_w2 = A + o_gw2; e->ew_off = A + o_goff;
  e->hd_w1t = A + o_hw1; e->hd_b1 = A + o_hb1; e->hd_w2 = A + o_hw2; e->hd_b2 = A + o_hb2;
  e->layers.resize(L);
  for (int l = 0; l < L; ++l) {
    TdLayer& ly = e->layers[l];
    ly.offsets = A + o_off[l]; ly.coeff = coeffs[l];
    ly.x2h.resize(num_x2h); ly.h2x.resize(num_h2x);
    for (int idx = 0; idx < num_x2h + num_h2x; ++idx) {
      const bool is_h2x = idx >= num_x2h;
      TdSubLayer& sl = is_h2x ? ly.h2x[idx - num_x2h] : ly.x2h[idx];
      const SubOff& so = is_h2x ? sh[l][idx - num_x2h] : sx[l][idx];
      sl.wn_t = A + so.wn_t; sl.bn = A + so.bn; sl.wn_img = IM ? IM + so.wn_img : nullptr;
      sl.k = mk_mlp(A, IM, so.k, 0, 256); sl.v = mk_mlp(A, IM, so.v, 128, 384); sl.q = mk_mlp(A, IM, so.q, 512, 512);
      sl.ew_w = so.ew_w >= 0 ? A + so.ew_w : nullptr; sl.ew_b = so.ew_b;
      sl.out_wa_img = so.out_wa >= 0 ? IM + so.out_wa : nullptr; sl.out_wb_img = so.out_wb >= 0 ? IM + so.out_wb : nullptr;
      sl.out_b1 = so.out_b1 >= 0 ? A + so.out_b1 : nullptr;
      memset(&sl.out, 0, sizeof(sl.out));
      if (so.out_w2 >= 0) {
        sl.out.w2_img = IM + so.out_w2; sl.out.ln_g = A + so.out_g; sl.out.ln_b = A + so.out_b; sl.out.b2 = A + so.out_b2; sl.out.nout = TD_H;
      }
    }
  }
  if (e->step.ensure(sizeof(int)) || e->err_flag.ensure(sizeof(int)) || e->total_edges.ensure(sizeof(long long))) {
    tdiff_destroy(e); return set_err(TDIFF_ECUDA, "cudaMalloc failed");
  }
  cudaMemset(e->err_flag.p, 0, sizeof(int));
  if (cudaStreamCreateWithFlags(&e->own_stream, cudaStreamNonBlocking) != cudaSuccess ||
      cudaEventCreateWithFlags(&e->ev_fork, cudaEventDisableTiming) != cudaSuccess ||
      cudaEventCreateWithFlags(&e->ev_join, cudaEventDisableTiming) != cudaSuccess) {
    tdiff_destroy(e); return set_err(TDIFF_ECUDA, "stream/event creation failed");
  }
  *out = e;
  return TDIFF_OK;
}

extern "C" void tdiff_destroy(tdiff_engine* e) {
  if (!e) return;
  cudaSetDevice(e->device);
  for (auto& ev : e->events) { cudaEventDestroy(ev.a); cudaEventDestroy(ev.b); }
  if (e->own_stream) cudaStreamDestroy(e->own_stream);
  if (e->ev_fork) cudaEventDestroy(e->ev_fork);
  if (e->ev_join) cudaEventDestroy(e->ev_join);
  DevBuf* bufs[] = {&e->node_ptr, &e->prot_ptr, &e->prot_node, &e->prot_graph, &e->lig_node, &e->lig_graph, &e->node_lig, &e->xm0, &e->xm1,
                    &e->rel_flag, &e->rel_list, &e->n_rel, &e->work_list, &e->n_work, &e->knn_cache, &e->x2h_rows, &e->lig_rows, &e->rel_rows, &e->rel_counts, &e->ew_x2h, &e->ew_h2x, &e->h_sync, &e->hagg, &e->time_norm, &e->h_free, &e->dirty, &e->free_rows, &e->free_counts, &e->lig_save, &e->offset, &e->h0, &e->h, &e->P, &e->q, &e->src, &e->src_prev, &e->etype, &e->e_w, &e->dist, &e->kbuf, &e->vbuf, &e->v16, &e->lig_pos,
                    &e->lig_v, &e->logits, &e->step, &e->err_flag, &e->node_off, &e->total_edges, &e->fix_mask, &e->fix_pos, &e->fix_v, &e->seq_buf, &e->lk_buf, &e->lk_x0, &e->lk_v0};
  for (auto* b : bufs) b->release();
  for (auto& b : e->stage) b.release();
  if (e->arena) cudaFree(e->arena);
  if (e->img_arena) cudaFree(e->img_arena);
  delete e;
}

extern "C" int tdiff_bind_batch(tdiff_engine* e, int B, const int32_t* pc, const int32_t* lc, const float* d_ppos, const float* d_pfeat,
                                int center_mode, void* stream) {
  if (!e || !pc || !lc || B < 1) return set_err(TDIFF_EINVAL, "bind_batch: bad arguments");
  if (center_mode != 0 && center_mode != 1) return set_err(TDIFF_EINVAL, "center_mode %d (0 'none' | 1 'protein')", center_mode);
  cudaStream_t st = (cudaStream_t)stream;
  CK(cudaSetDevice(e->device));
  long long N = 0, Np = 0, Nl = 0;
  int max_ng = 0;
  for (int g = 0; g < B; ++g) {
    if (pc[g] < 0 || lc[g] < 0) return set_err(TDIFF_EINVAL, "negative atom count in graph %d", g);
    Np += pc[g]; Nl += lc[g];
    if (pc[g] + lc[g] > max_ng) max_ng = pc[g] + lc[g];
  }
  N = Np + Nl;
  if (N <= 0) return set_err(TDIFF_EINVAL, "empty batch");
  int K = e->KQ;
  if (e->hybrid) {
    int max_lc = 0;
    for (int g = 0; g < B; ++g) {
      if (lc[g] > max_lc) max_lc = lc[g];
      if (lc[g] > 0 && pc[g] < e->KQ)
        return set_err(TDIFF_EINVAL, "cutoff_mode 'hybrid': graph %d has %d protein atoms < k = %d (torch.topk fails in the reference too)", g, pc[g], e->KQ);
    }
    K = e->KQ + (max_lc > 0 ? max_lc - 1 : 0);
    if (K > TD_KMAX)
      return set_err(TDIFF_EINVAL, "cutoff_mode 'hybrid': k + n_ligand - 1 = %d + %d - 1 exceeds the %d neighbour slots per node", e->KQ, max_lc, TD_KMAX);
  }
  if (N * (long long)K >= (1LL << 31) / 1) return set_err(TDIFF_EINVAL, "batch too large: N*k = %lld edge slots", N * K);
  if (max_ng > 2800) return set_err(TDIFF_EINVAL, "graph with %d nodes exceeds the k-NN kernel's shared-memory tile (2800)", max_ng);
  if (Np > 0 && (!d_ppos || !d_pfeat)) return set_err(TDIFF_EINVAL, "null protein arrays");
  e->K = K;
  std::vector<int> node_ptr(B + 1), prot_ptr(B + 1), prot_node(Np), prot_graph(Np), lig_node(Nl), lig_graph(Nl), node_lig(N, -1);
  int n = 0, p = 0, a = 0;
  for (int g = 0; g < B; ++g) {
    node_ptr[g] = n; prot_ptr[g] = p;
    for (int i = 0; i < pc[g]; ++i) { prot_node[p] = n; prot_graph[p] = g; ++p; ++n; }
    for (int i = 0; i < lc[g]; ++i) { lig_node[a] = n; lig_graph[a] = g; node_lig[n] = a; ++a; ++n; }
  }
  node_ptr[B] = n; prot_ptr[B] = p;
  e->bound = false; e->has_ligand = false; e->have_graph = false; e->have_prev = false;
  e->has_fixed = false; e->fix_pos_noise = nullptr; e->fix_v_uniform = nullptr;
  e->start_t = -1; e->start_pos_noise = nullptr; e->start_v_uniform = nullptr;
  e->B = B; e->N = (int)N; e->Np = (int)Np; e->Nl = (int)Nl; e->max_ng = max_ng;
  const size_t slots = (size_t)N * K;
  int bad = 0;
  bad |= e->node_ptr.ensure((B + 1) * 4) | e->prot_ptr.ensure((B + 1) * 4) | e->prot_node.ensure(Np * 4 + 4) | e->prot_graph.ensure(Np * 4 + 4);
  bad |= e->lig_node.ensure(Nl * 4 + 4) | e->lig_graph.ensure(Nl * 4 + 4) | e->node_lig.ensure(N * 4);
  bad |= e->xm0.ensure(N * 16) | e->xm1.ensure(N * 16) | e->offset.ensure((size_t)B * 16);
  bad |= e->h0.ensure(N * TD_H * 4) | e->h.ensure(N * TD_H * 4) | e->P.ensure((size_t)(N + 1) * TD_NPROJ * 4) | e->q.ensure(N * TD_H * 4);
  bad |= e->src.ensure(slots * 4) | e->src_prev.ensure(slots * 4) | e->etype.ensure(slots) | e->e_w.ensure(slots * 4) | e->dist.ensure(slots * 4);
  const bool v4 = e->mlp_mode == 2 && e->mlp_v4;
  int gcd128 = 128;
  while (K % gcd128) gcd128 >>= 1;
  e->row_pad = 128 / gcd128;
  const long long pad = e->row_pad, nPpad = (Np + pad - 1) / pad * pad, nLpad = (Nl + pad - 1) / pad * pad;
  e->x2h_n_dst = nPpad + nLpad; e->x2h_split = nPpad; e->lig_n_dst = nLpad;
  std::vector<int> x2h_rows((size_t)(nPpad + nLpad), -1), lig_rows((size_t)nLpad, -1);
  for (long long i = 0; i < Np; ++i) x2h_rows[i] = prot_node[i];
  for (long long i = 0; i < Nl; ++i) { x2h_rows[nPpad + i] = lig_node[i]; lig_rows[i] = lig_node[i]; }
  if (v4) bad |= e->x2h_rows.ensure(x2h_rows.size() * 4 + 4) | e->lig_rows.ensure(lig_rows.size() * 4 + 4) | e->rel_rows.ensure(x2h_rows.size() * 4 + 4) |
                 e->rel_counts.ensure(16);
  const bool fuse = v4 && K == 32 && !e->env_no_fused_agg && e->ew_mode != 2;
  if (e->ew_mode == 1) bad |= e->ew_x2h.ensure(slots * 4) | e->ew_h2x.ensure(slots * 4);
  if (e->out_fc) bad |= e->hagg.ensure((size_t)N * TD_H * 4);
  if (e->sync_twoup && e->num_x2h > 0 && e->num_h2x > 0) bad |= e->h_sync.ensure((size_t)N * TD_H * 4);
  if (e->time_emb) bad |= e->time_norm.ensure((size_t)B * 4 + 16);
  bad |= e->kbuf.ensure(v4 ? (size_t)(nPpad + nLpad) * K * TD_HEADS * 4 + 64 : slots * TD_H * 4);
  if (!fuse) bad |= e->vbuf.ensure(slots * TD_H * 4);
  bad |= e->v16.ensure((size_t)nLpad * K * TD_HEADS * 4 + 16);
  int min_pc = 1 << 30;
  for (int g = 0; g < B; ++g) if (pc[g] < min_pc) min_pc = pc[g];
  e->free_ready = false;
  e->free_depth = (fuse && !e->hybrid && Nl > 0 && min_pc > K) ? e->env_free_depth : 0;
  const int x2h_evals = (int)e->layers.size() * e->num_x2h;
  if (e->free_depth > x2h_evals - 1) e->free_depth = x2h_evals - 1 > 0 ? x2h_evals - 1 : 0;
  if (e->free_depth > 0)
    bad |= e->h_free.ensure((size_t)e->free_depth * N * TD_H * 4) | e->dirty.ensure((size_t)e->free_depth * N + 16) |
           e->free_rows.ensure((size_t)e->free_depth * x2h_rows.size() * 4 + 4) | e->free_counts.ensure((size_t)e->free_depth * 16) |
           e->lig_save.ensure((size_t)Nl * 20 + 32);
  e->free_stride = (long long)x2h_rows.size();
  bad |= e->lig_pos.ensure(Nl * 16 + 16) | e->lig_v.ensure(Nl * 4 + 4) | e->logits.ensure((size_t)Nl * e->cfg.num_classes * 4 + 4);
  bad |= e->node_off.ensure(N * 8) | e->rel_flag.ensure(N + 16) | e->rel_list.ensure(N * 4 + 64) | e->n_rel.ensure(16) | e->work_list.ensure(N * 4 + 64) | e->n_work.ensure(16);
  e->knn_incremental = !e->env_knn_full && Np > 0;
  if (e->knn_incremental) bad |= e->knn_cache.ensure((size_t)N * (e->KQ + 1) * 8);
  if (bad) return set_err(TDIFF_ECUDA, "out of device memory binding a batch of %lld nodes (%zu edge slots)", N, slots);
  CK(cudaMemcpyAsync(e->node_ptr.p, node_ptr.data(), (B + 1) * 4, cudaMemcpyHostToDevice, st));
  CK(cudaMemcpyAsync(e->prot_ptr.p, prot_ptr.data(), (B + 1) * 4, cudaMemcpyHostToDevice, st));
  if (Np) {
    CK(cudaMemcpyAsync(e->prot_node.p, prot_node.data(), Np * 4, cudaMemcpyHostToDevice, st));
    CK(cudaMemcpyAsync(e->prot_graph.p, prot_graph.data(), Np * 4, cudaMemcpyHostToDevice, st));
  }
  if (Nl) {
    CK(cudaMemcpyAsync(e->lig_node.p, lig_node.data(), Nl * 4, cudaMemcpyHostToDevice, st));
    CK(cudaMemcpyAsync(e->lig_graph.p, lig_graph.data(), Nl * 4, cudaMemcpyHostToDevice, st));
  }
  CK(cudaMemcpyAsync(e->node_lig.p, node_lig.data(), N * 4, cudaMemcpyHostToDevice, st));
  if (v4) {
    if (!x2h_rows.empty()) CK(cudaMemcpyAsync(e->x2h_rows.p, x2h_rows.data(), x2h_rows.size() * 4, cudaMemcpyHostToDevice, st));
    if (!lig_rows.empty()) CK(cudaMemcpyAsync(e->lig_rows.p, lig_rows.data(), lig_rows.size() * 4, cudaMemcpyHostToDevice, st));
  }
  CK(cudaStreamSynchronize(st));
  CK(cudaMemsetAsync(e->offset.p, 0, (size_t)B * 16, st));
  if (e->time_emb) CK(cudaMemsetAsync(e->time_norm.p, 0, (size_t)B * 4, st));
  CK(cudaMemsetAsync(e->h0.p, 0, (size_t)N * TD_H * 4, st));
  CK(cudaMemsetAsync(e->xm0.p, 0, (size_t)N * 16, st));
  CK(cudaMemsetAsync(e->xm1.p, 0, (size_t)N * 16, st));
  CK(cudaMemsetAsync(e->etype.p, 0, slots, st));
  CK(cudaMemsetAsync(e->P.as<float>() + (size_t)N * TD_NPROJ, 0, (size_t)TD_NPROJ * 4, st));
  if (center_mode == 1) td_launch_segment_mean3(d_ppos, e->prot_ptr.as<int>(), B, e->offset.as<float4>(), st);
  td_launch_place_protein(d_ppos, e->prot_node.as<int>(), e->prot_graph.as<int>(), e->offset.as<float4>(), (int)Np, e->xm0.as<float4>(),
                          e->xm1.as<float4>(), st);
  td_launch_protein_embed(d_pfeat, (int)Np, e->cfg.protein_feat_dim, e->w_prot, e->b_prot, e->prot_node.as<int>(), e->h0.as<float>(), st);
  e->launches += 3;
  if (e->knn_incremental) {
    td_launch_knn_cache(e->xm0.as<float4>(), e->node_ptr.as<int>(), e->prot_ptr.as<int>(), B, max_ng, e->KQ, e->knn_cache.as<unsigned long long>(), st);
    e->launches += 1;
  }
  CK(cudaGetLastError());
  e->bound = true;
  return TDIFF_OK;
}

extern "C" int tdiff_set_ligand(tdiff_engine* e, const float* d_pos, const int64_t* d_v, int apply_center, void* stream) {
  if (!e || !e->bound) return set_err(TDIFF_ESTATE, "set_ligand before bind_batch");
  if (e->Nl > 0 && !d_pos) return set_err(TDIFF_EINVAL, "null ligand positions");
  if (!e->has_ligand && e->Nl > 0 && !d_v) return set_err(TDIFF_EINVAL, "ligand types required on first set_ligand");
  cudaStream_t st = (cudaStream_t)stream;
  CK(cudaSetDevice(e->device));
  td_launch_set_ligand(d_pos, (const long long*)d_v, e->lig_graph.as<int>(), e->offset.as<float4>(), apply_center, e->Nl,
                       e->cfg.num_classes, e->lig_pos.as<float4>(), e->lig_v.as<int>(), e->err_flag.as<int>(), st);
  e->launches += 1;
  if (d_v) {
    int flag = 0;
    CK(cudaMemcpyAsync(&flag, e->err_flag.p, sizeof(int), cudaMemcpyDeviceToHost, st));
    CK(cudaStreamSynchronize(st));
    if (flag) {
      cudaMemsetAsync(e->err_flag.p, 0, sizeof(int), st);
      e->has_ligand = false;
      return set_err(TDIFF_EINVAL, "ligand atom type index >= num_classes (%d)", e->cfg.num_classes);
    }
  }
  CK(cudaGetLastError());
  e->has_ligand = true;
  return TDIFF_OK;
}

extern "C" int tdiff_set_fixed(tdiff_engine* e, const uint8_t* d_mask, const float* d_pos0, const int64_t* d_v0, int apply_center, void* stream) {
  if (!e || !e->bound) return set_err(TDIFF_ESTATE, "set_fixed before bind_batch");
  if (!d_mask) {
    e->has_fixed = false;
    return TDIFF_OK;
  }
  if (e->Nl > 0 && (!d_pos0 || !d_v0)) return set_err(TDIFF_EINVAL, "set_fixed: a mask needs target positions and classes");
  cudaStream_t st = (cudaStream_t)stream;
  CK(cudaSetDevice(e->device));
  const size_t Nl = (size_t)e->Nl;
  if (e->fix_mask.ensure(Nl + 16) | e->fix_pos.ensure(Nl * 16 + 16) | e->fix_v.ensure(Nl * 4 + 16))
    return set_err(TDIFF_ECUDA, "out of device memory for the fixed set of %zu ligand atoms", Nl);
  e->has_fixed = false;
  td_launch_set_fixed(d_mask, d_pos0, (const long long*)d_v0, e->lig_graph.as<int>(), e->offset.as<float4>(), apply_center, e->Nl,
                      e->cfg.num_classes, e->fix_mask.as<unsigned char>(), e->fix_pos.as<float4>(), e->fix_v.as<int>(), e->err_flag.as<int>(), st);
  e->launches += 1;
  int flag = 0;
  CK(cudaMemcpyAsync(&flag, e->err_flag.p, sizeof(int), cudaMemcpyDeviceToHost, st));
  CK(cudaStreamSynchronize(st));
  if (flag) {
    cudaMemsetAsync(e->err_flag.p, 0, sizeof(int), st);
    return set_err(TDIFF_EINVAL, "fixed atom class index outside 0..%d", e->cfg.num_classes - 1);
  }
  CK(cudaGetLastError());
  e->has_fixed = true;
  return TDIFF_OK;
}

extern "C" int tdiff_set_fixed_tape(tdiff_engine* e, const float* d_pos_noise, const float* d_v_uniform) {
  if (!e || !e->bound) return set_err(TDIFF_ESTATE, "set_fixed_tape before bind_batch");
  e->fix_pos_noise = d_pos_noise;
  e->fix_v_uniform = d_pos_noise ? d_v_uniform : nullptr;
  return TDIFF_OK;
}

extern "C" int tdiff_set_start(tdiff_engine* e, int t_start, const float* d_pos_noise, const float* d_v_uniform) {
  if (!e || !e->bound) return set_err(TDIFF_ESTATE, "set_start before bind_batch");
  const int T = e->cfg.num_timesteps;
  if (t_start < -1 || t_start > T - 1) return set_err(TDIFF_EINVAL, "set_start: t_start=%d outside -1..%d", t_start, T - 1);
  const bool on = t_start >= 0;
  e->start_t = t_start;
  e->start_pos_noise = on ? d_pos_noise : nullptr;
  e->start_v_uniform = on && d_pos_noise ? d_v_uniform : nullptr;
  return TDIFF_OK;
}

extern "C" int tdiff_get_ligand(tdiff_engine* e, float* d_pos, int64_t* d_v, int add_offset, void* stream) {
  if (!e || !e->has_ligand) return set_err(TDIFF_ESTATE, "get_ligand before set_ligand");
  CK(cudaSetDevice(e->device));
  td_launch_get_ligand(e->lig_pos.as<float4>(), e->lig_v.as<int>(), e->lig_graph.as<int>(), e->offset.as<float4>(), add_offset, e->Nl, d_pos,
                       (long long*)d_v, (cudaStream_t)stream);
  e->launches += 1;
  CK(cudaGetLastError());
  return TDIFF_OK;
}

extern "C" int tdiff_get_offset(tdiff_engine* e, float* d_offset, void* stream) {
  if (!e || !e->bound || !d_offset) return set_err(TDIFF_ESTATE, "get_offset before bind_batch");
  CK(cudaSetDevice(e->device));
  td_launch_gather_xyz(e->offset.as<float4>(), nullptr, e->B, d_offset, (cudaStream_t)stream);
  e->launches += 1;
  CK(cudaGetLastError());
  return TDIFF_OK;
}

namespace {
struct Prof {
  tdiff_engine* e; cudaStream_t st; int kind; bool on; EvPair ev;
  Prof(tdiff_engine* e_, cudaStream_t st_, int kind_) : e(e_), st(st_), kind(kind_), on(e_->profiling) {
    if (on) { cudaEventCreate(&ev.a); cudaEventCreate(&ev.b); ev.kind = kind; cudaEventRecord(ev.a, st); }
  }
  ~Prof() { if (on) { cudaEventRecord(ev.b, st); e->events.push_back(ev); } }
};

enum RowList { ROWS_ALL = 0, ROWS_LIGAND = 1, ROWS_RELEVANT = 2 };
bool fused_logits(const tdiff_engine* e) { return e->mlp_mode == 2 && e->mlp_v4; }
void edge_mlp(tdiff_engine* e, const float* P, const float4* xm, const int* src, const unsigned char* etype, RowList list, int K, const TdMlp& m,
              const float* offsets, float coeff, float* out, cudaStream_t st, const float* e_w, const float* qnode = nullptr,
              const float* agg_logits = nullptr, float* agg_h = nullptr, int key_softmax = 0, int free_layer = -1) {
  if (fused_logits(e) && m.w2_img && m.tabcls_img) {
    const int* rows = list == ROWS_ALL ? e->x2h_rows.as<int>() : list == ROWS_LIGAND ? e->lig_rows.as<int>() : e->rel_rows.as<int>();
    const int* counts = list == ROWS_RELEVANT ? e->rel_counts.as<int>() : nullptr;
    if (free_layer >= 0) {
      rows = e->free_rows.as<int>() + (size_t)free_layer * e->free_stride;
      counts = e->free_counts.as<int>() + 4 * free_layer;
    }
    const long long n_dst = list == ROWS_LIGAND ? e->lig_n_dst : e->x2h_n_dst;
    const long long split = list == ROWS_LIGAND ? 0 : e->x2h_split;
    const int by_slot = (list != ROWS_LIGAND && !key_softmax && agg_logits == nullptr) ? 1 : 0;
    td_launch_edge_mlp_v4(P, e->N, src, etype, e->dist.as<float>(), rows, n_dst, split, counts, K, m,
                          e->host_arena.data() + (offsets - e->arena), coeff, e->host_arena.data() + (m.ln_b - e->arena),
                          e->host_arena.data() + (m.b2 - e->arena), qnode, out, by_slot, agg_logits, e_w, agg_h, key_softmax,
                          e->sm_count, st);
    return;
  }
  const int* row_nodes = list == ROWS_LIGAND ? e->lig_node.as<int>() : nullptr;
  const long long n_rows = (long long)(list == ROWS_LIGAND ? e->Nl : e->N) * K;
  if (e->mlp_mode != 0 && m.nout == TD_H && m.w2_img)
    td_launch_edge_mlp_tc(P, xm, src, etype, e->dist.as<float>(), row_nodes, n_rows, K, m, m.w2_img, e->mlp_mode, offsets, coeff, out, e->sm_count, st);
  else
    td_launch_edge_mlp(P, xm, src, etype, row_nodes, n_rows, K, m, offsets, coeff, out, e->sm_count, st);
}

void node_side(tdiff_engine* e, const float* h, int N, const TdSubLayer& sl, float* P, float* q, cudaStream_t st, const int* rows = nullptr,
               const int* d_n = nullptr) {
  if (fused_logits(e) && sl.wn_img && sl.q.w2_img) {
    td_launch_node_side_v4(h, N, sl.wn_img, sl.bn, sl.q, P, q, rows, d_n, e->sm_count, st);
  } else if (e->mlp_mode != 0 && sl.wn_img && sl.q.w2_img) {
    TdMlp pm = sl.q;
    pm.b2 = sl.bn;
    td_launch_rows_tc(1, h, TD_H, 0, N, pm, sl.wn_img, e->mlp_mode, P, TD_NPROJ, TD_NPROJ / TD_H, rows, d_n, e->sm_count, st);
    td_launch_rows_tc(2, P, TD_NPROJ, 512, N, sl.q, sl.q.w2_img, e->mlp_mode, q, TD_H, 1, rows, d_n, e->sm_count, st);
  } else {
    td_launch_node_proj(h, N, sl.wn_t, sl.bn, P, st);
    td_launch_node_q(P, N, sl.q, q, st);
  }
}

void run_forward(tdiff_engine* e, cudaStream_t st, int fix_x, int free_build = 0, float* blk_pos = nullptr, float* blk_logits = nullptr) {
  const int N = e->N, Nl = e->Nl, K = e->K;
  float4* xm[2] = {e->xm0.as<float4>(), e->xm1.as<float4>()};
  const int* src = e->src.as<int>();
  const unsigned char* etype = e->etype.as<unsigned char>();
  float* h = e->h.as<float>();
  float* P = e->P.as<float>();
  float* q = e->q.as<float>();
  td_launch_scatter_ligand_pos(e->lig_pos.as<float4>(), e->lig_node.as<int>(), Nl, xm[0], st);
  td_launch_init_h(e->h0.as<float>(), xm[0], e->lig_v.as<int>(), e->node_lig.as<int>(), e->wl_t, e->bl, e->w_time, e->time_norm.as<float>(),
                   e->lig_graph.as<int>(), N, h, st);
  e->launches += 2;
  int cur = 0;
  const int KC = e->cfg.num_classes;
  auto snapshot = [&](int i) {
    if (blk_pos) {
      td_launch_gather_xyz(xm[cur], e->lig_node.as<int>(), Nl, blk_pos + (size_t)i * Nl * 3, st);
      e->launches += 1;
    }
    if (blk_logits) {
      td_launch_head(h, e->lig_node.as<int>(), Nl, e->hd_w1t, e->hd_b1, e->hd_w2, e->hd_b2, KC, blk_logits + (size_t)i * Nl * KC, st);
      e->launches += 1;
    }
  };
  if (Nl > 0) snapshot(0);
  const int n_blocks = free_build ? 1 : e->num_blocks;
  for (int blk = 0; blk < n_blocks; ++blk) {
    const int use_free = (!free_build && e->free_ready && blk == 0) ? e->free_depth : 0;
    const bool last_blk = blk + 1 == n_blocks;
    if (e->knn_incremental)
      td_launch_knn_update(xm[cur], e->node_ptr.as<int>(), e->prot_ptr.as<int>(), e->B, e->max_ng, e->KQ, K, e->hybrid, e->knn_cache.as<unsigned long long>(),
                           e->src.as<int>(), st);
    else
      td_launch_knn(xm[cur], e->node_ptr.as<int>(), e->prot_ptr.as<int>(), e->B, e->max_ng, e->KQ, K, e->hybrid, e->src.as<int>(), st);
    td_launch_edge_const(xm[cur], src, e->src_prev.as<int>(), e->have_prev ? 1 : 0, N, K, e->ew_off, e->ew_coeff, e->ew_w1t, e->ew_b1, e->ew_g, e->ew_b, e->ew_w2,
                         e->ew_b2, e->etype.as<unsigned char>(), e->e_w.as<float>(), e->rel_flag.as<unsigned char>(),
                         use_free ? e->dirty.as<unsigned char>() : nullptr, e->work_list.as<int>(), e->n_work.as<int>(), (e->ew_mode != 0 ? 1 : 0) | (e->env_no_slot_keep ? 2 : 0), st);
    e->have_prev = true;
    for (int l = 0; l < use_free; ++l) {
      unsigned char* dl = e->dirty.as<unsigned char>() + (size_t)l * N;
      if (l > 0) td_launch_dirty_propagate(dl - N, src, N, K, dl, st);
      td_launch_rel_rows(dl, xm[cur], N, e->lig_rows.as<int>(), (int)e->lig_n_dst, e->row_pad, e->free_rows.as<int>() + (size_t)l * e->free_stride,
                         e->free_counts.as<int>() + 4 * l, st);
      e->launches += l > 0 ? 3 : 2;
    }
    td_launch_rel_compact(e->rel_flag.as<unsigned char>(), N, e->rel_list.as<int>(), e->n_rel.as<int>(), st);
    e->launches += 4;
    if (fused_logits(e) && e->restrict_last && last_blk && e->num_x2h > 0) {
      td_launch_rel_rows(e->rel_flag.as<unsigned char>(), xm[cur], N, e->lig_rows.as<int>(), (int)e->lig_n_dst, e->row_pad, e->rel_rows.as<int>(),
                         e->rel_counts.as<int>(), st);
      e->launches += 2;
    }
    const float4* xm_blk = xm[cur];
    const int NX = e->num_x2h, NH = e->num_h2x;
    const size_t L = e->layers.size();
    int g = 0;
    for (size_t l = 0; l < L && !(free_build && g >= free_build); ++l) {
      const TdLayer& ly = e->layers[l];
      const float* ew_x = e->ew_mode == 1 ? e->ew_x2h.as<float>() : e->e_w.as<float>();
      const float* ew_h = e->ew_mode == 1 ? e->ew_h2x.as<float>() : e->e_w.as<float>();
      const bool run_h2x = !free_build && !fix_x && Nl > 0 && NH > 0;
      const float* h_h2x = h;
      if (e->sync_twoup && run_h2x && NX > 0) {
        cudaMemcpyAsync(e->h_sync.p, h, (size_t)N * TD_H * 4, cudaMemcpyDeviceToDevice, st);
        h_h2x = e->h_sync.as<float>();
      }
      for (int i = 0; i < NX && !(free_build && g >= free_build); ++i, ++g) {
        const TdSubLayer& sx = ly.x2h[i];
        const int fl = g < use_free ? g : -1;
        node_side(e, h, N, sx, P, q, st);
        if (e->mlp_mode != 0 && (i == 0 || e->ew_mode == 1)) {
          TdEwR ew = {nullptr, nullptr, 0.f, 0.f, ly.offsets, ly.coeff, nullptr, nullptr};
          if (e->ew_mode == 1) {
            const TdSubLayer& sh0 = NH > 0 ? ly.h2x[0] : sx;
            ew.w_x2h = sx.ew_w; ew.w_h2x = sh0.ew_w; ew.b_x2h = sx.ew_b; ew.b_h2x = sh0.ew_b; ew.out_x2h = e->ew_x2h.as<float>(); ew.out_h2x = e->ew_h2x.as<float>();
          }
          td_launch_edge_geom(xm[cur], src, etype, N, K, e->dist.as<float>(), ew, st);
          e->launches += 1;
        }
        const bool fuse_agg = fused_logits(e) && K == 32 && !e->env_no_fused_agg && e->ew_mode != 2;
        const bool sub = fuse_agg && e->restrict_last && last_blk && l + 1 == L && i + 1 == NX && !e->env_no_restrict && !e->out_fc;
        const RowList rl = sub ? ROWS_RELEVANT : ROWS_ALL;
        float* agg_target = h;
        if (e->out_fc) {
          agg_target = e->hagg.as<float>();
          cudaMemsetAsync(agg_target, 0, (size_t)N * TD_H * 4, st);
        }
        {
          Prof pr(e, st, EV_EDGE_MLP);
          edge_mlp(e, P, xm[cur], src, etype, rl, K, sx.k, ly.offsets, ly.coeff, e->kbuf.as<float>(), st, ew_x, fused_logits(e) ? q : nullptr, nullptr,
                   nullptr, fuse_agg ? 1 : 0, fl);
          edge_mlp(e, P, xm[cur], src, etype, rl, K, sx.v, ly.offsets, ly.coeff, e->vbuf.as<float>(), st, ew_x, nullptr,
                   fuse_agg ? e->kbuf.as<float>() : nullptr, fuse_agg ? agg_target : nullptr, 0, fl);
        }
        if (!fuse_agg) {
          Prof pr(e, st, EV_AGG_H);
          if (fused_logits(e))
            td_launch_aggregate_h_logits(e->kbuf.as<float>(), e->vbuf.as<float>(), ew_x, src, e->out_fc ? agg_target : h, agg_target, N, K,
                                         e->ew_mode == 2 ? sx.ew_w : nullptr, sx.ew_b, st);
          else td_launch_aggregate_h(e->kbuf.as<float>(), e->vbuf.as<float>(), e->e_w.as<float>(), src, q, h, h, N, K, st);
        }
        e->launches += fuse_agg ? 4 : 5;
        if (e->out_fc) {
          float* t1 = P;
          float* t2 = P + (size_t)N * TD_H;
          TdMlp m1 = sx.out;
          m1.b2 = e->zeros128;
          td_launch_rows_tc(1, agg_target, TD_H, 0, N, m1, sx.out_wa_img, e->mlp_mode, t1, TD_H, 1, nullptr, nullptr, e->sm_count, st);
          m1.b2 = sx.out_b1;
          td_launch_rows_tc(1, h, TD_H, 0, N, m1, sx.out_wb_img, e->mlp_mode, t2, TD_H, 1, nullptr, nullptr, e->sm_count, st);
          td_launch_add_rows(t1, t2, t1, (long long)N * TD_H, st);
          td_launch_rows_tc(2, t1, TD_H, 0, N, sx.out, sx.out.w2_img, e->mlp_mode, t2, TD_H, 1, nullptr, nullptr, e->sm_count, st);
          td_launch_add_rows(h, t2, h, (long long)N * TD_H, st);
          e->launches += 6;
        }
        if (fl >= 0) {
          td_launch_restore_clean(e->dirty.as<unsigned char>() + (size_t)fl * N, xm_blk, e->h_free.as<float>() + (size_t)fl * N * TD_H, N, h, st);
          e->launches += 1;
        }
        if (free_build) cudaMemcpyAsync(e->h_free.as<float>() + (size_t)g * N * TD_H, h, (size_t)N * TD_H * 4, cudaMemcpyDeviceToDevice, st);
      }
      if (!run_h2x) continue;
      for (int j = 0; j < NH; ++j) {
        const TdSubLayer& sh = ly.h2x[j];
        if (j > 0 || NX == 0) {
          td_launch_edge_geom_rows(xm[cur], src, etype, e->lig_node.as<int>(), Nl, K, e->dist.as<float>(), e->ew_mode == 1 ? sh.ew_w : nullptr, sh.ew_b,
                                   ly.offsets, ly.coeff, e->ew_h2x.as<float>(), st);
          e->launches += 1;
        }
        {
          const bool rel = fused_logits(e) && !e->env_no_restrict;
          node_side(e, h_h2x, N, sh, P, q, st, rel ? e->rel_list.as<int>() : nullptr, rel ? e->n_rel.as<int>() : nullptr);
        }
        {
          Prof pr(e, st, EV_EDGE_MLP);
          edge_mlp(e, P, xm[cur], src, etype, ROWS_LIGAND, K, sh.k, ly.offsets, ly.coeff, e->kbuf.as<float>(), st, ew_h, fused_logits(e) ? q : nullptr);
          edge_mlp(e, P, xm[cur], src, etype, ROWS_LIGAND, K, sh.v, ly.offsets, ly.coeff, e->v16.as<float>(), st, ew_h);
        }
        {
          Prof pr(e, st, EV_AGG_X);
          if (fused_logits(e))
            td_launch_aggregate_x_logits(e->kbuf.as<float>(), e->v16.as<float>(), ew_h, src, xm[cur], e->lig_node.as<int>(), xm[cur ^ 1], Nl, K, st);
          else
            td_launch_aggregate_x(e->kbuf.as<float>(), e->v16.as<float>(), e->e_w.as<float>(), src, q, xm[cur], e->lig_node.as<int>(), xm[cur ^ 1], Nl, K, st);
        }
        e->launches += 5;
        cur ^= 1;
      }
    }
    if (Nl > 0) snapshot(blk + 1);
  }
  if (free_build) return;
  td_launch_head(h, e->lig_node.as<int>(), Nl, e->hd_w1t, e->hd_b1, e->hd_w2, e->hd_b2, e->cfg.num_classes, e->logits.as<float>(), st);
  e->launches += 1;
  e->final_buf = cur;
  e->have_graph = true;
  e->have_prev = true;
}
}

extern "C" int tdiff_set_time(tdiff_engine* e, const float* d_time_norm, void* stream) {
  if (!e || !e->bound) return set_err(TDIFF_ESTATE, "set_time before bind_batch");
  if (!e->time_emb) return TDIFF_OK;
  if (!d_time_norm) return set_err(TDIFF_EINVAL, "null time array");
  CK(cudaSetDevice(e->device));
  CK(cudaMemcpyAsync(e->time_norm.p, d_time_norm, (size_t)e->B * 4, cudaMemcpyDeviceToDevice, (cudaStream_t)stream));
  return TDIFF_OK;
}

namespace {
int forward_impl(tdiff_engine* e, float* d_pred_pos, float* d_pred_logits, float* d_final_h, int fix_x, float* d_block_pos, float* d_block_logits,
                 void* stream) {
  if (!e || !e->bound || !e->has_ligand) return set_err(TDIFF_ESTATE, "forward needs bind_batch + set_ligand first");
  cudaStream_t st = (cudaStream_t)stream;
  CK(cudaSetDevice(e->device));
  Prof* total = new Prof(e, st, EV_TOTAL);
  run_forward(e, st, fix_x, 0, d_block_pos, d_block_logits);
  delete total;
  const float4* xf = e->final_buf ? e->xm1.as<float4>() : e->xm0.as<float4>();
  if (d_pred_pos) { td_launch_gather_xyz(xf, e->lig_node.as<int>(), e->Nl, d_pred_pos, st); e->launches += 1; }
  if (d_pred_logits && e->Nl) CK(cudaMemcpyAsync(d_pred_logits, e->logits.p, (size_t)e->Nl * e->cfg.num_classes * 4, cudaMemcpyDeviceToDevice, st));
  if (d_final_h) CK(cudaMemcpyAsync(d_final_h, e->h.p, (size_t)e->N * TD_H * 4, cudaMemcpyDeviceToDevice, st));
  CK(cudaGetLastError());
  return TDIFF_OK;
}
}

extern "C" int tdiff_forward(tdiff_engine* e, float* d_pred_pos, float* d_pred_logits, float* d_final_h, int fix_x, void* stream) {
  return forward_impl(e, d_pred_pos, d_pred_logits, d_final_h, fix_x, nullptr, nullptr, stream);
}

extern "C" int tdiff_forward_blocks(tdiff_engine* e, float* d_pred_pos, float* d_pred_logits, float* d_final_h, int fix_x, float* d_block_pos,
                                    float* d_block_logits, void* stream) {
  return forward_impl(e, d_pred_pos, d_pred_logits, d_final_h, fix_x, d_block_pos, d_block_logits, stream);
}

extern "C" int64_t tdiff_num_edges(tdiff_engine* e, void* stream) {
  if (!e || !e->have_graph) return set_err(TDIFF_ESTATE, "no graph built yet (run forward first)");
  cudaStream_t st = (cudaStream_t)stream;
  if (cudaSetDevice(e->device) != cudaSuccess) return set_err(TDIFF_ECUDA, "cudaSetDevice failed");
  td_launch_edge_count_scan(e->src.as<int>(), e->N, e->K, e->node_off.as<long long>(), e->total_edges.as<long long>(), st);
  e->launches += 1;
  long long tot = 0;
  if (cudaMemcpyAsync(&tot, e->total_edges.p, 8, cudaMemcpyDeviceToHost, st) != cudaSuccess || cudaStreamSynchronize(st) != cudaSuccess)
    return set_err(TDIFF_ECUDA, "num_edges: %s", cudaGetErrorString(cudaGetLastError()));
  return tot;
}

extern "C" int tdiff_get_edge_index(tdiff_engine* e, int64_t* d_edge_index, void* stream) {
  if (!e || !e->have_graph || !d_edge_index) return set_err(TDIFF_ESTATE, "no graph built yet (run forward first)");
  cudaStream_t st = (cudaStream_t)stream;
  CK(cudaSetDevice(e->device));
  td_launch_edge_count_scan(e->src.as<int>(), e->N, e->K, e->node_off.as<long long>(), e->total_edges.as<long long>(), st);
  td_launch_edge_compact(e->src.as<int>(), nullptr, e->N, e->K, e->node_off.as<long long>(), e->total_edges.as<long long>(),
                         (long long*)d_edge_index, nullptr, st);
  e->launches += 2;
  CK(cudaGetLastError());
  return TDIFF_OK;
}

extern "C" int tdiff_get_edge_weight(tdiff_engine* e, float* d_e_w, void* stream) {
  if (!e || !e->have_graph || !d_e_w) return set_err(TDIFF_ESTATE, "no graph built yet (run forward first)");
  cudaStream_t st = (cudaStream_t)stream;
  CK(cudaSetDevice(e->device));
  td_launch_edge_count_scan(e->src.as<int>(), e->N, e->K, e->node_off.as<long long>(), e->total_edges.as<long long>(), st);
  td_launch_edge_compact(e->src.as<int>(), e->e_w.as<float>(), e->N, e->K, e->node_off.as<long long>(), e->total_edges.as<long long>(), nullptr,
                         d_e_w, st);
  e->launches += 2;
  CK(cudaGetLastError());
  return TDIFF_OK;
}

extern "C" int tdiff_get_node_pos(tdiff_engine* e, float* d_x, void* stream) {
  if (!e || !e->have_graph || !d_x) return set_err(TDIFF_ESTATE, "no forward run yet");
  CK(cudaSetDevice(e->device));
  td_launch_gather_xyz(e->final_buf ? e->xm1.as<float4>() : e->xm0.as<float4>(), nullptr, e->N, d_x, (cudaStream_t)stream);
  e->launches += 1;
  CK(cudaGetLastError());
  return TDIFF_OK;
}

namespace {
void build_free_cache(tdiff_engine* e, cudaStream_t st) {
  const size_t Nl = (size_t)e->Nl;
  char* sv = e->lig_save.as<char>();
  cudaMemcpyAsync(sv, e->lig_pos.p, Nl * 16, cudaMemcpyDeviceToDevice, st);
  cudaMemcpyAsync(sv + Nl * 16, e->lig_v.p, Nl * 4, cudaMemcpyDeviceToDevice, st);
  td_launch_park_ligand(e->lig_pos.as<float4>(), e->lig_v.as<int>(), e->Nl, st);
  const bool had_prev = e->have_prev;
  e->have_prev = false;
  run_forward(e, st, 1, e->free_depth);
  e->have_prev = false;
  (void)had_prev;
  cudaMemcpyAsync(e->lig_pos.p, sv, Nl * 16, cudaMemcpyDeviceToDevice, st);
  cudaMemcpyAsync(e->lig_v.p, sv + Nl * 16, Nl * 4, cudaMemcpyDeviceToDevice, st);
  e->launches += 1;
  e->free_ready = true;
}

void run_step(tdiff_engine* e, cudaStream_t st, const TdStepArgs& base) {
  if (e->time_emb) {
    if (base.seq_t) td_launch_set_time_seq(base.step, base.seq_t, e->cfg.num_timesteps, e->B, e->time_norm.as<float>(), st);
    else td_launch_set_time(base.step, base.t_start, e->cfg.num_timesteps, e->B, e->time_norm.as<float>(), st);
    e->launches += 1;
  }
  e->restrict_last = true;
  run_forward(e, st, 0);
  e->restrict_last = false;
  TdStepArgs A = base;
  A.xm_final = e->final_buf ? e->xm1.as<float4>() : e->xm0.as<float4>();
  td_launch_step_epilogue(A, st);
  e->launches += 2;
}
void seq_tables(const tdiff_engine* e, const int32_t* seq, int S, std::vector<int>& it, std::vector<float>& ft) {
  const float* H = e->host_arena.data();
  auto tab = [&](const float* dev, int t) { return H[(dev - e->arena) + t]; };
  it.assign(2 * (size_t)S, 0);
  ft.assign(5 * (size_t)S, 0.0f);
  for (int s = 0; s < S; ++s) {
    const int t = seq[s], p = s + 1 < S ? seq[s + 1] : t - 1;
    it[s] = t; it[S + s] = p;
    float* f = ft.data() + s;
    if (p == t - 1) {
      f[0] = tab(e->t_c0, t); f[S] = tab(e->t_ct, t); f[2 * S] = tab(e->t_logvar, t); f[3 * S] = tab(e->t_la, t); f[4 * S] = tab(e->t_l1ma, t);
      continue;
    }
    const double lt = e->cum_log_a[t], lp = e->cum_log_a[p];
    const double om_t = -expm1(lt), om_p = -expm1(lp), om_a = -expm1(lt - lp);
    const double lam = e->cum_log_av[t] - e->cum_log_av[p];
    f[0] = (float)(sqrt(exp(lp)) * om_a / om_t);
    f[S] = (float)(sqrt(exp(lt - lp)) * om_p / om_t);
    f[2 * S] = (float)log(om_p * om_a / om_t);
    f[3 * S] = (float)lam;
    f[4 * S] = (float)log(1.0 - exp(lam) + 1e-40);
  }
}

int sample_chain(tdiff_engine* e, const int32_t* time_seq, int num_steps, const float* d_pos_noise, const float* d_v_uniform, uint64_t seed,
                 float* d_pos_traj, int64_t* d_v_traj, float* d_v0_traj, float* d_vt_traj, int pos_only, void* stream) {
  if (!e || !e->bound || !e->has_ligand) return set_err(TDIFF_ESTATE, "sample needs bind_batch + set_ligand first");
  const int T = e->cfg.num_timesteps;
  const bool start = e->start_t >= 0;
  if (start && !time_seq)
    return set_err(TDIFF_EINVAL, "a start is armed (tdiff_set_start, t_start=%d): run the chain with tdiff_sample_seq from t_start", e->start_t);
  if (num_steps < 0 || num_steps > T) return set_err(TDIFF_EINVAL, "num_steps=%d outside 0..%d", num_steps, T);
  if (time_seq) {
    if (num_steps < 1) return set_err(TDIFF_EINVAL, "time sequence: empty (num_steps=%d)", num_steps);
    if (start && time_seq[0] != e->start_t)
      return set_err(TDIFF_EINVAL, "time sequence: starts at %d, not at the start time t_start = %d", time_seq[0], e->start_t);
    if (!start && time_seq[0] != T - 1) return set_err(TDIFF_EINVAL, "time sequence: starts at %d, not at T - 1 = %d", time_seq[0], T - 1);
    for (int s = 1; s < num_steps; ++s) {
      if (time_seq[s] >= time_seq[s - 1])
        return set_err(TDIFF_EINVAL, "time sequence: not strictly decreasing at step %d (%d after %d)", s, time_seq[s], time_seq[s - 1]);
      if (time_seq[s] < 0) return set_err(TDIFF_EINVAL, "time sequence: negative time %d at step %d", time_seq[s], s);
    }
  }
  if ((d_pos_noise == nullptr) != (d_v_uniform == nullptr) && !pos_only)
    return set_err(TDIFF_EINVAL, "noise tape needs both pos_noise and v_uniform (or neither for Philox)");
  if (e->has_fixed) {
    if ((d_pos_noise != nullptr) != (e->fix_pos_noise != nullptr))
      return set_err(TDIFF_EINVAL, d_pos_noise ? "fixed atoms with a noise tape need a fixed-atom tape (tdiff_set_fixed_tape)"
                                               : "a fixed-atom tape is set but the chain has no noise tape (clear it, or pass both)");
    if (d_pos_noise && !pos_only && !e->fix_v_uniform)
      return set_err(TDIFF_EINVAL, "the fixed-atom tape needs v_uniform unless pos_only");
  }
  if (start) {
    if ((d_pos_noise != nullptr) != (e->start_pos_noise != nullptr))
      return set_err(TDIFF_EINVAL, d_pos_noise ? "a start with a noise tape needs a start tape (tdiff_set_start)"
                                               : "a start tape is set but the chain has no noise tape (clear it, or pass both)");
    if (d_pos_noise && !pos_only && !e->start_v_uniform)
      return set_err(TDIFF_EINVAL, "the start tape needs v_uniform unless pos_only");
  }
  cudaStream_t st = (cudaStream_t)stream;
  CK(cudaSetDevice(e->device));
  if (num_steps == 0) return TDIFF_OK;
  TdStepArgs A;
  memset(&A, 0, sizeof(A));
  A.n_lig = e->Nl; A.n_classes = e->cfg.num_classes; A.t_start = start ? e->start_t : T - 1; A.pos_only = pos_only;
  A.step = e->step.as<int>(); A.lig_node = e->lig_node.as<int>(); A.lig_graph = e->lig_graph.as<int>();
  A.logits = e->logits.as<float>(); A.offset = e->offset.as<float4>();
  A.c0 = e->t_c0; A.ct = e->t_ct; A.logvar = e->t_logvar; A.la_v = e->t_la; A.l1ma_v = e->t_l1ma; A.lca_v = e->t_lca; A.l1mca_v = e->t_l1mca;
  A.sra = e->t_sra; A.srm1 = e->t_srm1; A.mean_noise = e->cfg.model_mean_type == 1;
  A.log_k = (float)log((double)e->cfg.num_classes);
  A.pos_noise = d_pos_noise; A.v_uniform = d_v_uniform; A.seed = seed;
  A.lig_pos = e->lig_pos.as<float4>(); A.lig_v = e->lig_v.as<int>();
  A.pos_traj = d_pos_traj; A.v_traj = (long long*)d_v_traj; A.v0_traj = d_v0_traj; A.vt_traj = d_vt_traj;
  if (e->has_fixed) {
    A.fix_mask = e->fix_mask.as<unsigned char>(); A.fix_pos = e->fix_pos.as<float4>(); A.fix_v = e->fix_v.as<int>(); A.ac = e->t_ac;
    A.fix_pos_noise = e->fix_pos_noise; A.fix_v_uniform = e->fix_v_uniform;
  }
  if (start) { A.ac = e->t_ac; A.start_pos_noise = e->start_pos_noise; A.start_v_uniform = e->start_v_uniform; }
  if (time_seq) {
    std::vector<int> it;
    std::vector<float> ft;
    seq_tables(e, time_seq, num_steps, it, ft);
    const size_t S = (size_t)num_steps;
    if (e->seq_buf.ensure(S * 28)) return set_err(TDIFF_ECUDA, "out of device memory for the tables of a %d-step time sequence", num_steps);
    CK(cudaMemcpyAsync(e->seq_buf.p, it.data(), S * 8, cudaMemcpyHostToDevice, st));
    CK(cudaMemcpyAsync(e->seq_buf.as<char>() + S * 8, ft.data(), S * 20, cudaMemcpyHostToDevice, st));
    const int* si = e->seq_buf.as<int>();
    const float* sf = (const float*)(si + 2 * S);
    A.seq_t = si; A.seq_p = si + S;
    A.seq_c0 = sf; A.seq_ct = sf + S; A.seq_logvar = sf + 2 * S; A.seq_la = sf + 3 * S; A.seq_l1ma = sf + 4 * S;
  }
  CK(cudaMemsetAsync(e->step.p, 0, sizeof(int), st));
  if (start) {
    td_launch_start_init(A, st);
    e->launches += 1;
  } else if (e->has_fixed) {
    td_launch_fixed_init(A, st);
    e->launches += 1;
  }
  if (e->free_depth > 0 && !e->free_ready) build_free_cache(e, st);
  const bool eager = e->profiling || e->env_no_graph;
  Prof* total = new Prof(e, st, EV_TOTAL);
  run_step(e, st, A);
  int done = 1;
  if (!eager && num_steps > 2) {
    cudaStream_t cs = e->own_stream;
    CK(cudaEventRecord(e->ev_fork, st));
    CK(cudaStreamWaitEvent(cs, e->ev_fork, 0));
    cudaGraph_t graph = nullptr;
    cudaGraphExec_t exec = nullptr;
    const long long before = e->launches;
    cudaError_t ce = cudaStreamBeginCapture(cs, cudaStreamCaptureModeThreadLocal);
    if (ce == cudaSuccess) {
      run_step(e, cs, A);
      ce = cudaStreamEndCapture(cs, &graph);
    }
    const long long per_step = e->launches - before;
    e->launches = before;
    if (ce == cudaSuccess) ce = cudaGraphInstantiate(&exec, graph, 0);
    if (ce != cudaSuccess) {
      if (graph) cudaGraphDestroy(graph);
      (void)cudaGetLastError();
      delete total;
      return set_err(TDIFF_ECUDA, "CUDA graph capture of the sampling step failed: %s", cudaGetErrorString(ce));
    }
    for (; done < num_steps; ++done) {
      ce = cudaGraphLaunch(exec, cs);
      if (ce != cudaSuccess) break;
      e->launches += per_step;
    }
    if (ce == cudaSuccess) ce = cudaEventRecord(e->ev_join, cs);
    if (ce == cudaSuccess) ce = cudaStreamWaitEvent(st, e->ev_join, 0);
    cudaGraphExecDestroy(exec);
    cudaGraphDestroy(graph);
    if (ce != cudaSuccess) { delete total; return set_err(TDIFF_ECUDA, "cudaGraphLaunch failed: %s", cudaGetErrorString(ce)); }
  }
  for (; done < num_steps; ++done) run_step(e, st, A);
  delete total;
  CK(cudaGetLastError());
  return TDIFF_OK;
}
}

extern "C" int tdiff_sample(tdiff_engine* e, int num_steps, const float* d_pos_noise, const float* d_v_uniform, uint64_t seed,
                            float* d_pos_traj, int64_t* d_v_traj, float* d_v0_traj, float* d_vt_traj, int pos_only, void* stream) {
  return sample_chain(e, nullptr, num_steps, d_pos_noise, d_v_uniform, seed, d_pos_traj, d_v_traj, d_v0_traj, d_vt_traj, pos_only, stream);
}

extern "C" int tdiff_sample_seq(tdiff_engine* e, const int32_t* h_time_seq, int num_steps, const float* d_pos_noise, const float* d_v_uniform,
                                uint64_t seed, float* d_pos_traj, int64_t* d_v_traj, float* d_v0_traj, float* d_vt_traj, int pos_only,
                                void* stream) {
  if (!h_time_seq) return set_err(TDIFF_EINVAL, "time sequence: null pointer");
  return sample_chain(e, h_time_seq, num_steps, d_pos_noise, d_v_uniform, seed, d_pos_traj, d_v_traj, d_v0_traj, d_vt_traj, pos_only, stream);
}

extern "C" int tdiff_likelihood_terms(tdiff_engine* e, const int32_t* h_time_steps, const uint32_t* h_keys, const float* d_pos_noise,
                                      const float* d_v_uniform, uint64_t seed, float* d_kl_pos, float* d_kl_v, float* d_prior_pos,
                                      float* d_prior_v, float* d_atom_kl_pos, float* d_atom_kl_v, float* d_xt, int64_t* d_vt, void* stream) {
  if (!e || !e->bound || !e->has_ligand) return set_err(TDIFF_ESTATE, "likelihood_terms needs bind_batch + set_ligand first");
  const int T = e->cfg.num_timesteps, B = e->B;
  if (!h_time_steps) return set_err(TDIFF_EINVAL, "likelihood_terms: null time steps");
  if (e->cfg.model_mean_type != 0)
    return set_err(TDIFF_EINVAL, "likelihood_terms needs model_mean_type C0 (the reference raises for 'noise' too)");
  if (T >= (1 << 24)) return set_err(TDIFF_EINVAL, "likelihood_terms: T = %d does not fit the stream's 24-bit time field", T);
  for (int g = 0; g < B; ++g)
    if (h_time_steps[g] < 0 || h_time_steps[g] > T - 1)
      return set_err(TDIFF_EINVAL, "likelihood_terms: time step %d of graph %d outside 0..%d", h_time_steps[g], g, T - 1);
  if ((d_pos_noise == nullptr) != (d_v_uniform == nullptr))
    return set_err(TDIFF_EINVAL, "likelihood_terms: the tape needs both pos_noise and v_uniform (or neither for Philox)");
  cudaStream_t st = (cudaStream_t)stream;
  CK(cudaSetDevice(e->device));
  const size_t Nl = (size_t)e->Nl;
  if (e->lk_buf.ensure((size_t)B * 8 + 16) | e->lk_x0.ensure(Nl * 16 + 16) | e->lk_v0.ensure(Nl * 4 + 16))
    return set_err(TDIFF_ECUDA, "out of device memory for likelihood scoring of %d graphs", B);
  e->lk_host.resize(2 * (size_t)B);
  for (int g = 0; g < B; ++g) {
    e->lk_host[g] = h_time_steps[g];
    e->lk_host[B + g] = (int32_t)(h_keys ? h_keys[g] : (uint32_t)g);
  }
  CK(cudaMemcpyAsync(e->lk_buf.p, e->lk_host.data(), (size_t)B * 8, cudaMemcpyHostToDevice, st));
  TdLikelihoodArgs L;
  memset(&L, 0, sizeof(L));
  TdStepArgs& A = L.A;
  A.n_lig = e->Nl; A.n_classes = e->cfg.num_classes; A.pos_only = 0; A.seed = seed;
  A.lig_graph = e->lig_graph.as<int>(); A.lig_pos = e->lig_pos.as<float4>(); A.lig_v = e->lig_v.as<int>();
  A.ac = e->t_ac; A.lca_v = e->t_lca; A.l1mca_v = e->t_l1mca; A.log_k = (float)log((double)e->cfg.num_classes);
  A.lk_t = e->lk_buf.as<int>(); A.lk_key = (const unsigned*)(e->lk_buf.as<int>() + B);
  A.lk_pos_noise = d_pos_noise; A.lk_v_uniform = d_v_uniform;
  L.n_graphs = B; L.n_timesteps = T;
  L.node_ptr = e->node_ptr.as<int>(); L.prot_ptr = e->prot_ptr.as<int>(); L.lig_node = e->lig_node.as<int>();
  L.logits = e->logits.as<float>();
  L.c0 = e->t_c0; L.ct = e->t_ct; L.logvar = e->t_logvar; L.la_v = e->t_la; L.l1ma_v = e->t_l1ma;
  L.x0 = e->lk_x0.as<float4>(); L.v0 = e->lk_v0.as<int>();
  L.time_norm = e->time_emb ? e->time_norm.as<float>() : nullptr;
  L.kl_pos = d_kl_pos; L.kl_v = d_kl_v; L.prior_pos = d_prior_pos; L.prior_v = d_prior_v;
  L.atom_kl_pos = d_atom_kl_pos; L.atom_kl_v = d_atom_kl_v; L.xt = d_xt; L.vt = (long long*)d_vt;
  td_launch_likelihood_init(L, st);
  e->launches += 1;
  Prof* total = new Prof(e, st, EV_TOTAL);
  run_forward(e, st, 0);
  delete total;
  L.xm_final = e->final_buf ? e->xm1.as<float4>() : e->xm0.as<float4>();
  td_launch_likelihood_epilogue(L, st);
  e->launches += 1;
  CK(cudaGetLastError());
  return TDIFF_OK;
}

extern "C" int tdiff_sample_host(tdiff_engine* e, int B, const int32_t* pc, const int32_t* lc, const float* h_ppos, const float* h_pfeat,
                                 const float* h_lpos, const int64_t* h_lv, int center_mode, int num_steps, const float* h_pos_noise,
                                 const float* h_v_uniform, uint64_t seed, float* h_out_pos, int64_t* h_out_v, float* h_pos_traj,
                                 int64_t* h_v_traj, float* h_v0_traj, float* h_vt_traj, int pos_only, void* stream) {
  if (!e || !pc || !lc || B < 1) return set_err(TDIFF_EINVAL, "sample_host: bad arguments");
  cudaStream_t st = (cudaStream_t)stream;
  CK(cudaSetDevice(e->device));
  size_t Np = 0, Nl = 0;
  for (int g = 0; g < B; ++g) { Np += pc[g] > 0 ? pc[g] : 0; Nl += lc[g] > 0 ? lc[g] : 0; }
  const int F = e->cfg.protein_feat_dim, KC = e->cfg.num_classes;
  const size_t S = num_steps > 0 ? num_steps : 0;
  DevBuf* sb = e->stage;
  int bad = sb[0].ensure(Np * 12 + 16) | sb[1].ensure(Np * F * 4 + 16) | sb[2].ensure(Nl * 12 + 16) | sb[3].ensure(Nl * 8 + 16);
  if (h_pos_noise) bad |= sb[4].ensure(S * Nl * 12 + 16);
  if (h_v_uniform) bad |= sb[5].ensure(S * Nl * KC * 4 + 16);
  const size_t o_pos = 0, o_v = (o_pos + (h_pos_traj ? S * Nl * 12 : 0) + 15) / 16 * 16,
               o_v0 = (o_v + (h_v_traj ? S * Nl * 8 : 0) + 15) / 16 * 16,
               o_vt = o_v0 + (h_v0_traj ? S * Nl * KC * 4 : 0), o_end = o_vt + (h_vt_traj ? S * Nl * KC * 4 : 0);
  bad |= sb[6].ensure(o_end + 16) | sb[7].ensure(Nl * 12 + Nl * 8 + 32);
  if (bad) return set_err(TDIFF_ECUDA, "out of device memory staging host buffers");
  if (Np) {
    CK(cudaMemcpyAsync(sb[0].p, h_ppos, Np * 12, cudaMemcpyHostToDevice, st));
    CK(cudaMemcpyAsync(sb[1].p, h_pfeat, Np * F * 4, cudaMemcpyHostToDevice, st));
  }
  if (Nl) {
    CK(cudaMemcpyAsync(sb[2].p, h_lpos, Nl * 12, cudaMemcpyHostToDevice, st));
    CK(cudaMemcpyAsync(sb[3].p, h_lv, Nl * 8, cudaMemcpyHostToDevice, st));
  }
  if (h_pos_noise && S * Nl) CK(cudaMemcpyAsync(sb[4].p, h_pos_noise, S * Nl * 12, cudaMemcpyHostToDevice, st));
  if (h_v_uniform && S * Nl) CK(cudaMemcpyAsync(sb[5].p, h_v_uniform, S * Nl * KC * 4, cudaMemcpyHostToDevice, st));
  int rc = tdiff_bind_batch(e, B, pc, lc, sb[0].as<float>(), sb[1].as<float>(), center_mode, st);
  if (rc) return rc;
  rc = tdiff_set_ligand(e, sb[2].as<float>(), sb[3].as<int64_t>(), center_mode == 1, st);
  if (rc) return rc;
  char* tb = sb[6].as<char>();
  rc = tdiff_sample(e, num_steps, h_pos_noise ? sb[4].as<float>() : nullptr, h_v_uniform ? sb[5].as<float>() : nullptr, seed,
                    h_pos_traj ? (float*)(tb + o_pos) : nullptr, h_v_traj ? (int64_t*)(tb + o_v) : nullptr,
                    h_v0_traj ? (float*)(tb + o_v0) : nullptr, h_vt_traj ? (float*)(tb + o_vt) : nullptr, pos_only, st);
  if (rc) return rc;
  float* d_opos = sb[7].as<float>();
  int64_t* d_ov = (int64_t*)(sb[7].as<char>() + (Nl * 12 + 15) / 16 * 16);
  rc = tdiff_get_ligand(e, d_opos, d_ov, 1, st);
  if (rc) return rc;
  if (Nl) {
    if (h_out_pos) CK(cudaMemcpyAsync(h_out_pos, d_opos, Nl * 12, cudaMemcpyDeviceToHost, st));
    if (h_out_v) CK(cudaMemcpyAsync(h_out_v, d_ov, Nl * 8, cudaMemcpyDeviceToHost, st));
    if (S) {
      if (h_pos_traj) CK(cudaMemcpyAsync(h_pos_traj, tb + o_pos, S * Nl * 12, cudaMemcpyDeviceToHost, st));
      if (h_v_traj) CK(cudaMemcpyAsync(h_v_traj, tb + o_v, S * Nl * 8, cudaMemcpyDeviceToHost, st));
      if (h_v0_traj) CK(cudaMemcpyAsync(h_v0_traj, tb + o_v0, S * Nl * KC * 4, cudaMemcpyDeviceToHost, st));
      if (h_vt_traj) CK(cudaMemcpyAsync(h_vt_traj, tb + o_vt, S * Nl * KC * 4, cudaMemcpyDeviceToHost, st));
    }
  }
  CK(cudaStreamSynchronize(st));
  return TDIFF_OK;
}

extern "C" int tdiff_knn_graph(const float* d_x, int n_nodes, const int32_t* h_counts, int n_graphs, int k, int32_t* d_src_slots,
                               int64_t* d_edge_index, int64_t* h_n_edges, void* stream) {
  if (!d_x || !h_counts || !d_src_slots || n_nodes < 0 || n_graphs < 1 || k < 1 || k > TD_KMAX) return set_err(TDIFF_EINVAL, "knn_graph: bad arguments");
  cudaStream_t st = (cudaStream_t)stream;
  std::vector<int> ptr(n_graphs + 1, 0);
  int max_ng = 0;
  for (int g = 0; g < n_graphs; ++g) {
    if (h_counts[g] < 0) return set_err(TDIFF_EINVAL, "negative count");
    ptr[g + 1] = ptr[g] + h_counts[g];
    if (h_counts[g] > max_ng) max_ng = h_counts[g];
  }
  if (ptr[n_graphs] != n_nodes) return set_err(TDIFF_EINVAL, "graph counts sum to %d, expected %d nodes", ptr[n_graphs], n_nodes);
  if (max_ng > 2800) return set_err(TDIFF_EINVAL, "graph with %d nodes exceeds the k-NN kernel's shared-memory tile (2800)", max_ng);
  if (n_nodes == 0) { if (h_n_edges) *h_n_edges = 0; return TDIFF_OK; }
  DevBuf xm, dptr, off, tot;
  int rc = TDIFF_OK;
  if (xm.ensure((size_t)n_nodes * 16) || dptr.ensure((n_graphs + 1) * 4) || off.ensure((size_t)n_nodes * 8) || tot.ensure(8)) {
    rc = set_err(TDIFF_ECUDA, "out of device memory");
  } else {
    cudaMemcpyAsync(dptr.p, ptr.data(), (n_graphs + 1) * 4, cudaMemcpyHostToDevice, st);
    td_launch_pack_xyzm(d_x, nullptr, n_nodes, xm.as<float4>(), st);
    td_launch_knn(xm.as<float4>(), dptr.as<int>(), nullptr, n_graphs, max_ng, k, k, 0, d_src_slots, st);
    td_launch_edge_count_scan(d_src_slots, n_nodes, k, off.as<long long>(), tot.as<long long>(), st);
    if (d_edge_index) td_launch_edge_compact(d_src_slots, nullptr, n_nodes, k, off.as<long long>(), tot.as<long long>(), (long long*)d_edge_index, nullptr, st);
    long long t = 0;
    cudaMemcpyAsync(&t, tot.p, 8, cudaMemcpyDeviceToHost, st);
    cudaError_t ce = cudaStreamSynchronize(st);
    if (ce == cudaSuccess) ce = cudaGetLastError();
    if (ce != cudaSuccess) rc = set_err(TDIFF_ECUDA, "knn_graph: %s", cudaGetErrorString(ce));
    else if (h_n_edges) *h_n_edges = t;
  }
  xm.release(); dptr.release(); off.release(); tot.release();
  return rc;
}

extern "C" int tdiff_attn_aggregate_h(const float* d_k, const float* d_v, const float* d_e_w, const int32_t* d_src, const float* d_q,
                                      const float* d_h_in, float* d_h_out, int n_nodes, int kk, void* stream) {
  if (!d_k || !d_v || !d_e_w || !d_src || !d_q || !d_h_in || !d_h_out || n_nodes < 0 || kk < 1 || kk > TD_KMAX)
    return set_err(TDIFF_EINVAL, "attn_aggregate_h: bad arguments");
  td_launch_aggregate_h(d_k, d_v, d_e_w, d_src, d_q, d_h_in, d_h_out, n_nodes, kk, (cudaStream_t)stream);
  CK(cudaGetLastError());
  return TDIFF_OK;
}

extern "C" int tdiff_attn_aggregate_x(const float* d_k, const float* d_v16, const float* d_e_w, const int32_t* d_src, const float* d_q,
                                      const float* d_x, const uint8_t* d_mask, float* d_x_out, int n_nodes, int kk, void* stream) {
  if (!d_k || !d_v16 || !d_e_w || !d_src || !d_q || !d_x || !d_mask || !d_x_out || n_nodes < 0 || kk < 1 || kk > TD_KMAX)
    return set_err(TDIFF_EINVAL, "attn_aggregate_x: bad arguments");
  cudaStream_t st = (cudaStream_t)stream;
  if (n_nodes == 0) return TDIFF_OK;
  DevBuf a, b;
  if (a.ensure((size_t)n_nodes * 16) || b.ensure((size_t)n_nodes * 16)) { a.release(); b.release(); return set_err(TDIFF_ECUDA, "out of device memory"); }
  td_launch_pack_xyzm(d_x, d_mask, n_nodes, a.as<float4>(), st);
  td_launch_aggregate_x(d_k, d_v16, d_e_w, d_src, d_q, a.as<float4>(), nullptr, b.as<float4>(), n_nodes, kk, st);
  td_launch_gather_xyz(b.as<float4>(), nullptr, n_nodes, d_x_out, st);
  cudaError_t ce = cudaStreamSynchronize(st);
  if (ce == cudaSuccess) ce = cudaGetLastError();
  a.release(); b.release();
  if (ce != cudaSuccess) return set_err(TDIFF_ECUDA, "attn_aggregate_x: %s", cudaGetErrorString(ce));
  return TDIFF_OK;
}

extern "C" int tdiff_scatter_mean3(const float* d_src, const int32_t* h_counts, int n_segments, float* d_out, void* stream) {
  if (!d_src || !h_counts || !d_out || n_segments < 1) return set_err(TDIFF_EINVAL, "scatter_mean3: bad arguments");
  cudaStream_t st = (cudaStream_t)stream;
  std::vector<int> ptr(n_segments + 1, 0);
  for (int g = 0; g < n_segments; ++g) ptr[g + 1] = ptr[g] + (h_counts[g] > 0 ? h_counts[g] : 0);
  DevBuf dptr, o4;
  if (dptr.ensure((n_segments + 1) * 4) || o4.ensure((size_t)n_segments * 16)) { dptr.release(); o4.release(); return set_err(TDIFF_ECUDA, "out of device memory"); }
  cudaMemcpyAsync(dptr.p, ptr.data(), (n_segments + 1) * 4, cudaMemcpyHostToDevice, st);
  td_launch_segment_mean3(d_src, dptr.as<int>(), n_segments, o4.as<float4>(), st);
  td_launch_gather_xyz(o4.as<float4>(), nullptr, n_segments, d_out, st);
  cudaError_t ce = cudaStreamSynchronize(st);
  if (ce == cudaSuccess) ce = cudaGetLastError();
  dptr.release(); o4.release();
  if (ce != cudaSuccess) return set_err(TDIFF_ECUDA, "scatter_mean3: %s", cudaGetErrorString(ce));
  return TDIFF_OK;
}

extern "C" int tdiff_check_stability(const float* d_pos, const int32_t* d_atomic_num, const int32_t* h_counts, int n_mol, int hs, int32_t* d_nr_bonds,
                                     int32_t* d_stable_atoms, uint8_t* d_mol_stable, void* stream) {
  if (!d_pos || !d_atomic_num || !h_counts || !d_stable_atoms || !d_mol_stable || n_mol < 0) return set_err(TDIFF_EINVAL, "check_stability: bad arguments");
  if (n_mol == 0) return TDIFF_OK;
  cudaStream_t st = (cudaStream_t)stream;
  std::vector<int> ptr(n_mol + 1, 0);
  for (int m = 0; m < n_mol; ++m) {
    if (h_counts[m] < 0) return set_err(TDIFF_EINVAL, "negative atom count");
    ptr[m + 1] = ptr[m] + h_counts[m];
  }
  DevBuf dptr, derr;
  if (dptr.ensure((n_mol + 1) * 4) || derr.ensure(4)) { dptr.release(); derr.release(); return set_err(TDIFF_ECUDA, "out of device memory"); }
  cudaMemcpyAsync(dptr.p, ptr.data(), (n_mol + 1) * 4, cudaMemcpyHostToDevice, st);
  cudaMemsetAsync(derr.p, 0, 4, st);
  td_launch_check_stability(d_pos, d_atomic_num, dptr.as<int>(), n_mol, hs, d_nr_bonds, d_stable_atoms, d_mol_stable, derr.as<int>(), st);
  int flag = 0;
  cudaMemcpyAsync(&flag, derr.p, 4, cudaMemcpyDeviceToHost, st);
  cudaError_t ce = cudaStreamSynchronize(st);
  if (ce == cudaSuccess) ce = cudaGetLastError();
  dptr.release(); derr.release();
  if (ce != cudaSuccess) return set_err(TDIFF_ECUDA, "check_stability: %s", cudaGetErrorString(ce));
  if (flag) return set_err(TDIFF_EINVAL, "check_stability: atomic number outside the reference's table (H C N O F P S Cl)");
  return TDIFF_OK;
}

extern "C" int64_t tdiff_launch_count(tdiff_engine* e) { return e ? e->launches : 0; }
extern "C" int tdiff_edge_mlp_mode(tdiff_engine* e) { return !e ? TDIFF_EINVAL : (e->mlp_mode == 2 && e->mlp_v4) ? 5 : e->mlp_mode; }

extern "C" int tdiff_profile(tdiff_engine* e, int enable) {
  if (!e) return set_err(TDIFF_EINVAL, "null engine");
  e->profiling = enable != 0;
  if (enable) {
    for (int i = 0; i < EV_KINDS; ++i) { e->ms_acc[i] = 0; e->n_acc[i] = 0; }
  }
  return TDIFF_OK;
}

extern "C" int tdiff_profile_read(tdiff_engine* e, double* ms_h, int64_t* n_h, double* ms_x, int64_t* n_x, double* ms_mlp, int64_t* n_mlp,
                                  double* ms_total) {
  if (!e) return set_err(TDIFF_EINVAL, "null engine");
  CK(cudaSetDevice(e->device));
  CK(cudaDeviceSynchronize());
  for (auto& ev : e->events) {
    float ms = 0.f;
    if (cudaEventElapsedTime(&ms, ev.a, ev.b) == cudaSuccess) { e->ms_acc[ev.kind] += ms; e->n_acc[ev.kind] += 1; }
    cudaEventDestroy(ev.a); cudaEventDestroy(ev.b);
  }
  e->events.clear();
  if (ms_h) *ms_h = e->ms_acc[EV_AGG_H];
  if (n_h) *n_h = e->n_acc[EV_AGG_H];
  if (ms_x) *ms_x = e->ms_acc[EV_AGG_X];
  if (n_x) *n_x = e->n_acc[EV_AGG_X];
  if (ms_mlp) *ms_mlp = e->ms_acc[EV_EDGE_MLP];
  if (n_mlp) *n_mlp = e->n_acc[EV_EDGE_MLP];
  if (ms_total) *ms_total = e->ms_acc[EV_TOTAL];
  return TDIFF_OK;
}
```

targetdiff_b200/csrc/node_side.cu:

```cuda
#include "tdiff_common.cuh"
#include "hopper_mma.cuh"

namespace ns {

constexpr int kWG = 3;
constexpr int kThreads = kWG * 128;
constexpr int kTile = 64;
constexpr int kAtom = 128 * 128;
constexpr int kPiece = 2 * kAtom;
constexpr int kBlock = 2 * kPiece;
constexpr int kImgStride = 3 * kPiece;
constexpr int kHBuf = kTile * TD_H * 4;
constexpr size_t kSmem = 1024 + 2 * kBlock + kWG * kHBuf + 4 * TD_H * sizeof(float);
static_assert(kSmem <= 227 * 1024, "shared-memory map");

__device__ __forceinline__ uint32_t smem_u32(const void* p) { return (uint32_t)__cvta_generic_to_shared(p); }
__device__ __forceinline__ uint32_t cvt_bf16x2(float hi, float lo) {
  uint32_t d;
  asm("cvt.rn.bf16x2.f32 %0, %1, %2;" : "=r"(d) : "f"(hi), "f"(lo));
  return d;
}
__device__ __forceinline__ void stg64(float* p, float a, float b) { asm volatile("st.global.v2.f32 [%0], {%1,%2};" ::"l"(p), "f"(a), "f"(b) : "memory"); }
__device__ __forceinline__ void fence_proxy_async() { asm volatile("fence.proxy.async.shared::cta;" ::: "memory"); }

__device__ __forceinline__ void stage_weights(unsigned char* sW, const unsigned char* w0, const unsigned char* w1, float* sPar,
                                              const float* p0, const float* p1, const float* p2, const float* p3) {
  for (int i = threadIdx.x; i < kBlock / 16; i += kThreads) {
    reinterpret_cast<uint4*>(sW)[i] = reinterpret_cast<const uint4*>(w0)[i];
    reinterpret_cast<uint4*>(sW + kBlock)[i] = reinterpret_cast<const uint4*>(w1)[i];
  }
  for (int i = threadIdx.x; i < TD_H; i += kThreads) {
    if (p0) sPar[i] = p0[i];
    if (p1) sPar[TD_H + i] = p1[i];
    if (p2) sPar[2 * TD_H + i] = p2[i];
    if (p3) sPar[3 * TD_H + i] = p3[i];
  }
  fence_proxy_async();
  __syncthreads();
}

struct Rows {
  const int* list;
  const int* d_n;
  long long n;
};

__device__ __forceinline__ uint32_t chunk_pos(int r, int c) { return (uint32_t)(r * 512 + ((c ^ ((r & 3) << 1)) << 4)); }
__device__ __forceinline__ void bar_sync_wg(int wg) { asm volatile("bar.sync %0, 128;" ::"r"(1 + wg) : "memory"); }

__device__ __forceinline__ void load_tile_async(uint32_t buf, const float* __restrict__ in, const Rows& rw, long long n, long long tile, int t) {
  const int l = t & 31;
#pragma unroll 1
  for (int r = t >> 5; r < kTile; r += 4) {
    const long long i = tile * kTile + r;
    const long long node = i < n ? (rw.list ? (long long)rw.list[i] : i) : 0;
    asm volatile("cp.async.cg.shared.global [%0], [%1], 16, %2;" ::"r"(buf + chunk_pos(r, l)), "l"(in + (size_t)node * TD_H + 4 * l),
                 "r"(i < n ? 16 : 0) : "memory");
  }
  asm volatile("cp.async.commit_group;" ::: "memory");
}

__device__ __forceinline__ void read_tile(uint32_t buf, int w, int l, float (&x)[64]) {
  const int s = (l >> 2) & 3;
  const uint32_t base = buf + (uint32_t)(16 * w + (l >> 2)) * 512 + ((l & 3) >> 1) * 16 + (l & 1) * 8;
#pragma unroll
  for (int j = 0; j < 4; ++j) {
    const uint32_t p = base + ((j ^ s) << 5);
#pragma unroll
    for (int hh = 0; hh < 2; ++hh)
#pragma unroll
      for (int I = 0; I < 4; ++I) {
        const int i = 4 * I + j;
        float2 v;
        asm volatile("ld.shared.v2.f32 {%0, %1}, [%2];" : "=f"(v.x), "=f"(v.y) : "r"(p + hh * 8 * 512 + I * 128));
        x[4 * i + 2 * hh] = v.x;
        x[4 * i + 2 * hh + 1] = v.y;
      }
  }
}

__device__ __forceinline__ void split_frag(const float (&x)[64], uint32_t (&a)[2][8][4]) {
#pragma unroll
  for (int kk = 0; kk < 8; ++kk)
#pragma unroll
    for (int j = 0; j < 4; ++j) {
      const int e = 4 * (2 * kk + (j >> 1)) + 2 * (j & 1);
      const float x0 = x[e], x1 = x[e + 1];
      const uint32_t v = cvt_bf16x2(x1, x0);
      a[0][kk][j] = v;
      a[1][kk][j] = cvt_bf16x2(x1 - __uint_as_float(v & 0xffff0000u), x0 - __uint_as_float(v << 16));
    }
}

__device__ __forceinline__ void mma_block(float (&d)[64], const uint32_t (&a)[2][8][4], uint32_t w_addr) {
  wgmma_fence();
#pragma unroll
  for (int t = 0; t < 3; ++t) {
    const int pa = t == 2 ? 1 : 0, pb = t == 1 ? 1 : 0;
#pragma unroll
    for (int kk = 0; kk < 8; ++kk)
      wgmma_n128_rs(d, a[pa][kk], gmma_desc_sw128(w_addr + pb * kPiece + (kk >> 2) * kAtom + (kk & 3) * 32), (t | kk) ? 1u : 0u);
  }
  wgmma_commit();
  wgmma_wait_all();
}

__device__ __forceinline__ void store_rows(float* __restrict__ out, int ldo, int col0, const int (&prow)[2], int l, const float (&d)[64],
                                           const float* sBias) {
#pragma unroll
  for (int hh = 0; hh < 2; ++hh) {
    if (prow[hh] < 0) continue;
    float* o = out + (size_t)prow[hh] * ldo + col0;
#pragma unroll
    for (int i = 0; i < 16; ++i) {
      const int c = 8 * i + 2 * (l & 3);
      stg64(o + c, d[4 * i + 2 * hh] + sBias[c], d[4 * i + 2 * hh + 1] + sBias[c + 1]);
    }
  }
}

__device__ __forceinline__ void next_tile(uint32_t buf, const float* __restrict__ in, const Rows& rw, long long n, long long next, int wg, int t,
                                          float (&x)[64]) {
  asm volatile("cp.async.wait_all;" ::: "memory");
  bar_sync_wg(wg);
  read_tile(buf, t >> 5, t & 31, x);
  bar_sync_wg(wg);
  if (next >= 0) load_tile_async(buf, in, rw, n, next, t);
}

__device__ __forceinline__ void tile_rows(const Rows& rw, long long n, long long tile, int w, int l, int (&prow)[2]) {
#pragma unroll
  for (int hh = 0; hh < 2; ++hh) {
    const long long i = tile * kTile + 16 * w + (l >> 2) + 8 * hh;
    prow[hh] = i < n ? (rw.list ? rw.list[i] : (int)i) : -1;
  }
}

}

__global__ void __launch_bounds__(ns::kThreads, 1)
node_proj_kernel(const float* __restrict__ h, const unsigned char* __restrict__ wn_img, const float* __restrict__ bn, float* __restrict__ P,
                 ns::Rows rw) {
  using namespace ns;
  extern __shared__ unsigned char smem_raw[];
  unsigned char* sW = reinterpret_cast<unsigned char*>((reinterpret_cast<uintptr_t>(smem_raw) + 1023) & ~(uintptr_t)1023);
  float* sBias = reinterpret_cast<float*>(sW + 2 * kBlock + kWG * kHBuf);
  const int g = blockIdx.y;
  const long long n = rw.d_n ? (long long)*rw.d_n : rw.n;
  const long long n_tiles = (n + kTile - 1) / kTile, stride = (long long)gridDim.x * kWG;
  const int t = threadIdx.x & 127, l = t & 31, w = t >> 5;
  const int wg = __shfl_sync(0xffffffffu, threadIdx.x >> 7, 0);
  const uint32_t buf = smem_u32(sW + 2 * kBlock) + wg * kHBuf, w_addr = smem_u32(sW);
  long long tile = blockIdx.x * kWG + wg;
  if (tile < n_tiles) load_tile_async(buf, h, rw, n, tile, t);
  stage_weights(sW, wn_img + (size_t)(2 * g) * kImgStride, wn_img + (size_t)(2 * g + 1) * kImgStride, sBias, bn + 256 * g, bn + 256 * g + 128,
                nullptr, nullptr);
#pragma unroll 1
  for (; tile < n_tiles; tile += stride) {
    int prow[2];
    tile_rows(rw, n, tile, w, l, prow);
    uint32_t a[2][8][4];
    {
      float x[64];
      next_tile(buf, h, rw, n, tile + stride < n_tiles ? tile + stride : -1, wg, t, x);
      split_frag(x, a);
    }
#pragma unroll 1
    for (int j = 0; j < 2; ++j) {
      float d[64];
      mma_block(d, a, w_addr + j * kBlock);
      store_rows(P, TD_NPROJ, 256 * g + 128 * j, prow, l, d, sBias + 128 * j);
    }
  }
}

__global__ void __launch_bounds__(ns::kThreads, 1)
node_query_kernel(const float* __restrict__ h, const unsigned char* __restrict__ wq_img, const float* __restrict__ bq, TdMlp m,
                  float* __restrict__ q, ns::Rows rw) {
  using namespace ns;
  extern __shared__ unsigned char smem_raw[];
  unsigned char* sW = reinterpret_cast<unsigned char*>((reinterpret_cast<uintptr_t>(smem_raw) + 1023) & ~(uintptr_t)1023);
  float* sBq = reinterpret_cast<float*>(sW + 2 * kBlock + kWG * kHBuf);
  float* sG = sBq + TD_H;
  float* sB = sG + TD_H;
  float* sB2 = sB + TD_H;
  const long long n = rw.d_n ? (long long)*rw.d_n : rw.n;
  const long long n_tiles = (n + kTile - 1) / kTile, stride = (long long)gridDim.x * kWG;
  const int t = threadIdx.x & 127, l = t & 31, w = t >> 5;
  const int wg = __shfl_sync(0xffffffffu, threadIdx.x >> 7, 0);
  const uint32_t buf = smem_u32(sW + 2 * kBlock) + wg * kHBuf, w_addr = smem_u32(sW);
  long long tile = blockIdx.x * kWG + wg;
  if (tile < n_tiles) load_tile_async(buf, h, rw, n, tile, t);
  stage_weights(sW, wq_img, m.w2_img, sBq, bq, m.ln_g, m.ln_b, m.b2);
#pragma unroll 1
  for (; tile < n_tiles; tile += stride) {
    uint32_t a[2][8][4];
    float d[64];
    next_tile(buf, h, rw, n, tile + stride < n_tiles ? tile + stride : -1, wg, t, d);
    split_frag(d, a);
    mma_block(d, a, w_addr);
#pragma unroll
    for (int hh = 0; hh < 2; ++hh) {
      float s = 0.f;
#pragma unroll
      for (int i = 0; i < 16; ++i) {
        const int c = 8 * i + 2 * (l & 3);
        d[4 * i + 2 * hh] += sBq[c];
        d[4 * i + 2 * hh + 1] += sBq[c + 1];
        s += d[4 * i + 2 * hh] + d[4 * i + 2 * hh + 1];
      }
      s += __shfl_xor_sync(0xffffffffu, s, 1);
      s += __shfl_xor_sync(0xffffffffu, s, 2);
      const float mean = s * (1.0f / 128.0f);
      float v = 0.f;
#pragma unroll
      for (int i = 0; i < 16; ++i) {
        const float e0 = d[4 * i + 2 * hh] - mean, e1 = d[4 * i + 2 * hh + 1] - mean;
        d[4 * i + 2 * hh] = e0;
        d[4 * i + 2 * hh + 1] = e1;
        v += e0 * e0 + e1 * e1;
      }
      v += __shfl_xor_sync(0xffffffffu, v, 1);
      v += __shfl_xor_sync(0xffffffffu, v, 2);
      const float rstd = 1.0f / sqrtf(v * (1.0f / 128.0f) + 1e-5f);
#pragma unroll
      for (int i = 0; i < 16; ++i) {
        const int c = 8 * i + 2 * (l & 3);
        d[4 * i + 2 * hh] = fmaxf(d[4 * i + 2 * hh] * rstd * sG[c] + sB[c], 0.f);
        d[4 * i + 2 * hh + 1] = fmaxf(d[4 * i + 2 * hh + 1] * rstd * sG[c + 1] + sB[c + 1], 0.f);
      }
    }
    split_frag(d, a);
    mma_block(d, a, w_addr + kBlock);
    int prow[2];
    tile_rows(rw, n, tile, w, l, prow);
    store_rows(q, TD_H, 0, prow, l, d, sB2);
  }
}

void td_launch_node_side_v4(const float* h, long long n_rows, const unsigned char* wn_img, const float* bn, const TdMlp& q_mlp, float* P,
                            float* q, const int* rows, const int* d_n, int sm_count, cudaStream_t st) {
  using namespace ns;
  if (n_rows == 0) return;
  static size_t opted_p[TD_MAX_DEVICES] = {0}, opted_q[TD_MAX_DEVICES] = {0};
  td_opt_in_smem(node_proj_kernel, kSmem, opted_p);
  td_opt_in_smem(node_query_kernel, kSmem, opted_q);
  const Rows rw = {rows, d_n, n_rows};
  const long long slots = (n_rows + kTile - 1) / kTile;
  const long long ctas = (slots + kWG - 1) / kWG;
  const int per = sm_count / 2 > 0 ? sm_count / 2 : 1;
  node_proj_kernel<<<dim3((unsigned)(ctas < per ? ctas : per), 2), kThreads, kSmem, st>>>(h, wn_img, bn, P, rw);
  node_query_kernel<<<(unsigned)(ctas < sm_count ? ctas : sm_count), kThreads, kSmem, st>>>(h, wn_img + 4 * (size_t)kImgStride, bn + 512, q_mlp,
                                                                                           q, rw);
}
```

targetdiff_b200/csrc/tdiff_common.cuh:

```cuda
#pragma once
#include <cuda_runtime.h>
#include <stdint.h>

#define TD_H 128
#define TD_HEADS 16
#define TD_HD 8
#define TD_NG 20
#define TD_TAB 21
#define TD_KMAX 64
#define TD_NPROJ 640
#define TD_CMAX 24

struct TdMlp {
  const float* tab;
  const float* ln_g;
  const float* ln_b;
  const float* w2t;
  const float* b2;
  int nout;
  int offA, offB;
  const unsigned char* w2_img;
  const unsigned char* tabcls_img;
};

struct TdEwR {
  const float* w_x2h;
  const float* w_h2x;
  float b_x2h, b_h2x;
  const float* offsets;
  float coeff;
  float* out_x2h;
  float* out_h2x;
};

struct TdSubLayer {
  const float* wn_t;
  const float* bn;
  const unsigned char* wn_img;
  TdMlp k, v, q;
  const float* ew_w;
  float ew_b;
  const unsigned char* out_wa_img;
  const unsigned char* out_wb_img;
  const float* out_b1;
  TdMlp out;
};

__device__ __forceinline__ float warp_sum(float v) {
#pragma unroll
  for (int o = 16; o > 0; o >>= 1) v += __shfl_xor_sync(0xffffffffu, v, o);
  return v;
}
__device__ __forceinline__ float warp_max(float v) {
#pragma unroll
  for (int o = 16; o > 0; o >>= 1) v = fmaxf(v, __shfl_xor_sync(0xffffffffu, v, o));
  return v;
}

__device__ __forceinline__ void ln_relu_128(float (&p)[4], const float* __restrict__ g, const float* __restrict__ b, int lane) {
  float s = warp_sum((p[0] + p[1]) + (p[2] + p[3]));
  float mean = s * (1.0f / 128.0f);
  float d0 = p[0] - mean, d1 = p[1] - mean, d2 = p[2] - mean, d3 = p[3] - mean;
  float var = warp_sum((d0 * d0 + d1 * d1) + (d2 * d2 + d3 * d3)) * (1.0f / 128.0f);
  float rstd = 1.0f / sqrtf(var + 1e-5f);
  p[0] = fmaxf(d0 * rstd * g[lane] + b[lane], 0.0f);
  p[1] = fmaxf(d1 * rstd * g[lane + 32] + b[lane + 32], 0.0f);
  p[2] = fmaxf(d2 * rstd * g[lane + 64] + b[lane + 64], 0.0f);
  p[3] = fmaxf(d3 * rstd * g[lane + 96] + b[lane + 96], 0.0f);
}

#define TD_LDA 132
#define TD_GEMM_THREADS 512

__device__ __forceinline__ void tile_gemm_128(const float* __restrict__ As, const float* __restrict__ Bs, float (&acc)[4][8],
                                              int ty, int tx) {
#pragma unroll
  for (int i = 0; i < 4; ++i)
#pragma unroll
    for (int j = 0; j < 8; ++j) acc[i][j] = 0.0f;
#pragma unroll 2
  for (int kk = 0; kk < 128; kk += 4) {
    float4 a[4];
#pragma unroll
    for (int i = 0; i < 4; ++i) a[i] = *reinterpret_cast<const float4*>(As + (ty + 32 * i) * TD_LDA + kk);
#pragma unroll
    for (int k4 = 0; k4 < 4; ++k4) {
      float4 b0 = *reinterpret_cast<const float4*>(Bs + (kk + k4) * 128 + 4 * tx);
      float4 b1 = *reinterpret_cast<const float4*>(Bs + (kk + k4) * 128 + 64 + 4 * tx);
#pragma unroll
      for (int i = 0; i < 4; ++i) {
        float av = (k4 == 0) ? a[i].x : (k4 == 1) ? a[i].y : (k4 == 2) ? a[i].z : a[i].w;
        acc[i][0] = fmaf(av, b0.x, acc[i][0]);
        acc[i][1] = fmaf(av, b0.y, acc[i][1]);
        acc[i][2] = fmaf(av, b0.z, acc[i][2]);
        acc[i][3] = fmaf(av, b0.w, acc[i][3]);
        acc[i][4] = fmaf(av, b1.x, acc[i][4]);
        acc[i][5] = fmaf(av, b1.y, acc[i][5]);
        acc[i][6] = fmaf(av, b1.z, acc[i][6]);
        acc[i][7] = fmaf(av, b1.w, acc[i][7]);
      }
    }
  }
}

#define TD_MAX_DEVICES 64
template <class Kernel>
inline void td_opt_in_smem(Kernel kernel, size_t bytes, size_t (&done)[TD_MAX_DEVICES]) {
  int dev = 0;
  const bool known = cudaGetDevice(&dev) == cudaSuccess && dev >= 0 && dev < TD_MAX_DEVICES;
  if (known && bytes <= done[dev]) return;
  cudaFuncSetAttribute(kernel, cudaFuncAttributeMaxDynamicSharedMemorySize, (int)bytes);
  if (known) done[dev] = bytes;
}

void td_launch_knn(const float4* xm, const int* node_ptr, const int* prot_ptr, int n_graphs, int max_nodes_per_graph, int k, int stride, int hybrid,
                   int* src, cudaStream_t st);
void td_launch_knn_cache(const float4* xm, const int* node_ptr, const int* prot_ptr, int n_graphs, int max_ng, int k, unsigned long long* cache,
                         cudaStream_t st);
void td_launch_knn_update(const float4* xm, const int* node_ptr, const int* prot_ptr, int n_graphs, int max_ng, int k, int stride, int hybrid,
                          const unsigned long long* cache, int* src, cudaStream_t st);
void td_launch_edge_const(const float4* xm, const int* src, int* src_prev, int have_prev, int n_nodes, int k, const float* offsets, float coeff,
                          const float* w1t, const float* b1, const float* ln_g, const float* ln_b, const float* w2, float b2,
                          unsigned char* etype, float* e_w, unsigned char* rel_flag, unsigned char* touch_flag, int* work_list, int* n_work,
                          int gate_mode, cudaStream_t st);
void td_launch_dirty_propagate(const unsigned char* in, const int* src, int n_nodes, int k, unsigned char* out, cudaStream_t st);
void td_launch_restore_clean(const unsigned char* dirty, const float4* xm, const float* h_free, int n_nodes, float* h, cudaStream_t st);
void td_launch_rel_rows(const unsigned char* rel_flag, const float4* xm, int n_nodes, const int* lig_rows, int n_lig_rows, int pad, int* rel_rows,
                        int* rel_counts, cudaStream_t st);
void td_launch_protein_embed(const float* feat, int n_protein, int fdim, const float* w, const float* b, const int* prot_node,
                             float* h0, cudaStream_t st);
void td_launch_init_h(const float* h0, const float4* xm, const int* lig_v, const int* node_lig, const float* wl_t, const float* bl,
                      const float* w_time, const float* time_norm, const int* lig_graph, int n_nodes, float* h, cudaStream_t st);
void td_launch_node_proj(const float* h, int n_nodes, const float* wn_t, const float* bn, float* P, cudaStream_t st);
void td_launch_node_q(const float* P, int n_nodes, TdMlp q, float* qout, cudaStream_t st);
void td_launch_edge_mlp(const float* P, const float4* xm, const int* src, const unsigned char* etype, const int* row_nodes,
                        long long n_rows, int k, TdMlp m, const float* offsets, float coeff, float* out, int sm_count, cudaStream_t st);
void td_launch_edge_geom(const float4* xm, const int* src, const unsigned char* etype, int n_nodes, int k, float* dist, const TdEwR& ew, cudaStream_t st);
void td_launch_edge_geom_rows(const float4* xm, const int* src, const unsigned char* etype, const int* rows, int n_rows, int k, float* dist,
                              const float* gate_w, float gate_b, const float* offsets, float coeff, float* gate, cudaStream_t st);
void td_launch_add_rows(const float* a, const float* b, float* out, long long n_floats, cudaStream_t st);
void td_launch_set_time(const int* step, int t_start, int n_timesteps, int n_graphs, float* time_norm, cudaStream_t st);
void td_launch_set_time_seq(const int* step, const int* time_seq, int n_timesteps, int n_graphs, float* time_norm, cudaStream_t st);
void td_launch_edge_mlp_tc(const float* P, const float4* xm, const int* src, const unsigned char* etype, const float* dist,
                           const int* row_nodes, long long n_rows, int k, TdMlp m, const unsigned char* w2_image, int pieces, const float* offsets, float coeff,
                           float* out, int sm_count, cudaStream_t st);
void td_launch_edge_mlp_v4(const float* P, int zero_row, const int* src, const unsigned char* etype, const float* dist, const int* row_nodes, long long n_dst,
                           long long split_dst, const int* d_counts, int k, const TdMlp& m, const float* h_offsets, float coeff,
                           const float* h_ln_b, const float* h_b2, const float* qnode, float* out, int out_by_slot,
                           const float* agg_logits, const float* agg_e_w, float* agg_h, int key_softmax, int sm_count, cudaStream_t st);
void td_launch_rows_tc(int mode, const float* in, int ldi, int in_off, long long n_rows, TdMlp m, const unsigned char* w_image, int pieces, float* out,
                       int ldo, int nblocks, const int* row_list, const int* d_n_rows, int sm_count, cudaStream_t st);
void td_launch_node_side_v4(const float* h, long long n_rows, const unsigned char* wn_img, const float* bn, const TdMlp& q_mlp, float* P,
                            float* q, const int* rows, const int* d_n, int sm_count, cudaStream_t st);
void td_launch_rel_compact(const unsigned char* flag, int n_nodes, int* rel_list, int* n_rel, cudaStream_t st);
void td_launch_aggregate_h(const float* kbuf, const float* vbuf, const float* e_w, const int* src, const float* q, const float* h_in,
                           float* h_out, int n_nodes, int k, cudaStream_t st);
void td_launch_aggregate_x(const float* kbuf, const float* v16, const float* e_w, const int* src, const float* q, const float4* xm_in,
                           const int* row_nodes, float4* xm_out, int n_rows, int k, cudaStream_t st);
void td_launch_aggregate_h_logits(const float* logits, const float* vbuf, const float* e_w, const int* src, const float* h_in, float* h_out,
                                  int n_nodes, int k, const float* ewm_w, float ewm_b, cudaStream_t st);
void td_launch_aggregate_x_logits(const float* logits, const float* v16, const float* e_w, const int* src, const float4* xm_in,
                                  const int* row_nodes, float4* xm_out, int n_rows, int k, cudaStream_t st);
void td_launch_head(const float* h, const int* lig_node, int n_lig, const float* w1t, const float* b1, const float* w2, const float* b2,
                    int n_classes, float* logits, cudaStream_t st);
void td_launch_check_stability(const float* pos, const int* atomic_num, const int* mol_ptr, int n_mol, int hs, int* nr_bonds, int* stable_atoms,
                               unsigned char* mol_stable, int* err, cudaStream_t st);
```

Before: 18.50.

## Restrict last-block layers to per-layer dependency cone of ligand rows

Adds a per-graph BFS kernel that computes, for each x2h evaluation in the last block, the set of protein nodes whose outputs can still reach the ligand, and builds per-layer compacted row lists. Node-side projection, edge MLP and h aggregation are then run only over those cone rows instead of a single relevant-row list. This is meant to skip computation on protein nodes that cannot influence the final ligand prediction. It costs an extra list-building kernel, larger row buffers, and more complex bookkeeping that must match the dependency structure exactly. Node loading also now shuffles row indices across the warp.

```diff
diff --git a/include/tdiff.h b/include/tdiff.h
--- a/include/tdiff.h
+++ b/include/tdiff.h
@@ -112,6 +112,7 @@
 TDIFF_API int tdiff_profile(tdiff_engine* e, int enable);
 TDIFF_API int tdiff_profile_read(tdiff_engine* e, double* ms_aggregate_h, int64_t* n_aggregate_h, double* ms_aggregate_x,
                        int64_t* n_aggregate_x, double* ms_edge_mlp, int64_t* n_edge_mlp, double* ms_total);
+TDIFF_API int tdiff_get_cone(tdiff_engine* e, int32_t* h_dims, int32_t* h_counts, int32_t* h_rows);
 
 #ifdef __cplusplus
 }
diff --git a/targetdiff_b200/_lib.py b/targetdiff_b200/_lib.py
--- a/targetdiff_b200/_lib.py
+++ b/targetdiff_b200/_lib.py
@@ -61,6 +61,7 @@
     'tdiff_profile': (_i, [_vp, _i]),
     'tdiff_profile_read': (_i, [_vp, ctypes.POINTER(ctypes.c_double), ctypes.POINTER(_i64), ctypes.POINTER(ctypes.c_double),
                                 ctypes.POINTER(_i64), ctypes.POINTER(ctypes.c_double), ctypes.POINTER(_i64), ctypes.POINTER(ctypes.c_double)]),
+    'tdiff_get_cone': (_i, [_vp, _vp, _vp, _vp]),
 }
 
 _lib = None
diff --git a/targetdiff_b200/csrc/aggregate.cu b/targetdiff_b200/csrc/aggregate.cu
--- a/targetdiff_b200/csrc/aggregate.cu
+++ b/targetdiff_b200/csrc/aggregate.cu
@@ -135,11 +135,13 @@
 
 __global__ void __launch_bounds__(AGG_WARPS * 32)
 aggregate_h_logits_kernel(const float* __restrict__ logits, const float* __restrict__ vbuf, const float* __restrict__ e_w,
-                          const int* __restrict__ src, const float* __restrict__ h_in, float* __restrict__ h_out, int n_nodes, int k,
+                          const int* __restrict__ src, const float* __restrict__ h_in, float* __restrict__ h_out, TdRows dst, int k,
                           const float* __restrict__ ewm_w, float ewm_b) {
   const int lane = threadIdx.x & 31;
-  const int n = blockIdx.x * AGG_WARPS + (threadIdx.x >> 5);
-  if (n >= n_nodes) return;
+  const long long a = (long long)blockIdx.x * AGG_WARPS + (threadIdx.x >> 5);
+  if (a >= (dst.d_n ? (long long)*dst.d_n : dst.n)) return;
+  const int n = dst.list ? dst.list[a] : (int)a;
+  if (n < 0) return;
   const size_t e0 = (size_t)n * k;
   int deg = 0;
   for (int j = lane; j < k; j += 32) deg += (src[e0 + j] >= 0);
@@ -194,10 +196,10 @@
 }
 
 void td_launch_aggregate_h_logits(const float* logits, const float* vbuf, const float* e_w, const int* src, const float* h_in, float* h_out,
-                                  int n_nodes, int k, const float* ewm_w, float ewm_b, cudaStream_t st) {
-  if (n_nodes == 0) return;
-  aggregate_h_logits_kernel<<<(n_nodes + AGG_WARPS - 1) / AGG_WARPS, AGG_WARPS * 32, 0, st>>>(logits, vbuf, e_w, src, h_in, h_out, n_nodes, k,
-                                                                                             ewm_w, ewm_b);
+                                  const TdRows& dst, int k, const float* ewm_w, float ewm_b, cudaStream_t st) {
+  if (dst.n == 0) return;
+  aggregate_h_logits_kernel<<<(unsigned)((dst.n + AGG_WARPS - 1) / AGG_WARPS), AGG_WARPS * 32, 0, st>>>(logits, vbuf, e_w, src, h_in, h_out, dst, k,
+                                                                                                       ewm_w, ewm_b);
 }
 
 __global__ void __launch_bounds__(AGG_WARPS * 32)
diff --git a/targetdiff_b200/csrc/edge_const.cu b/targetdiff_b200/csrc/edge_const.cu
--- a/targetdiff_b200/csrc/edge_const.cu
+++ b/targetdiff_b200/csrc/edge_const.cu
@@ -200,7 +200,10 @@
   const int i = blockIdx.x * blockDim.x + threadIdx.x;
   if (i < n_nodes && flag[i] && xm[i].w == 0.0f) rel_rows[atomicAdd(&rel_counts[2], 1)] = i;
 }
-__global__ void rel_rows_finish_kernel(const int* __restrict__ lig_rows, int n_lig_rows, int pad, int* __restrict__ rel_rows, int* __restrict__ rel_counts) {
+__global__ void rel_rows_finish_kernel(const int* __restrict__ lig_rows, int n_lig_rows, int pad, int* __restrict__ rows, long long stride,
+                                       int* __restrict__ counts) {
+  int* rel_rows = rows + (size_t)blockIdx.y * stride;
+  int* rel_counts = counts + 4 * blockIdx.y;
   const int n_p = rel_counts[2], n_pp = (n_p + pad - 1) / pad * pad;
   const int i = blockIdx.x * blockDim.x + threadIdx.x;
   if (i < n_pp - n_p) rel_rows[n_p + i] = -1;
@@ -212,7 +215,77 @@
   cudaMemsetAsync(rel_counts, 0, 4 * sizeof(int), st);
   if (n_nodes > 0) rel_rows_protein_kernel<<<(n_nodes + 255) / 256, 256, 0, st>>>(rel_flag, xm, n_nodes, rel_rows, rel_counts);
   const int n = n_lig_rows > pad ? n_lig_rows : pad;
-  rel_rows_finish_kernel<<<(n + 255) / 256, 256, 0, st>>>(lig_rows, n_lig_rows, pad, rel_rows, rel_counts);
+  rel_rows_finish_kernel<<<(n + 255) / 256, 256, 0, st>>>(lig_rows, n_lig_rows, pad, rel_rows, 0, rel_counts);
+}
+
+#define CONE_THREADS 512
+__global__ void __launch_bounds__(CONE_THREADS)
+cone_lists_kernel(const unsigned char* __restrict__ rel_flag, const int* __restrict__ src, const int* __restrict__ node_ptr,
+                  const float4* __restrict__ xm, int n_nodes, int k, int G, int max_ng, const unsigned char* __restrict__ dirty, int n_dirty,
+                  int* __restrict__ rows, long long stride, int* __restrict__ counts) {
+  extern __shared__ int s_dist[];
+  int* s_cnt = s_dist + max_ng;
+  int* s_base = s_cnt + 2 * G;
+  const int n0 = node_ptr[blockIdx.x], ng = node_ptr[blockIdx.x + 1] - n0;
+  const int lane = threadIdx.x & 31, warp = threadIdx.x >> 5, nw = blockDim.x >> 5;
+  constexpr int kFar = 1 << 30;
+  for (int i = threadIdx.x; i < ng; i += blockDim.x) s_dist[i] = rel_flag[n0 + i] ? 0 : kFar;
+  for (int i = threadIdx.x; i < 2 * G; i += blockDim.x) s_cnt[i] = 0;
+  __syncthreads();
+  for (int r = 0; r < G; ++r) {
+    bool grew = false;
+    for (int i = warp; i < ng; i += nw) {
+      if (s_dist[i] != r) continue;
+      for (int j = lane; j < k; j += 32) {
+        const int s = src[(size_t)(n0 + i) * k + j];
+        if (s >= 0 && s_dist[s - n0] > r + 1) { s_dist[s - n0] = r + 1; grew = true; }
+      }
+    }
+    if (!__syncthreads_or(grew)) break;
+  }
+  const unsigned lt = (1u << lane) - 1u;
+  for (int pass = 0; pass < 2; ++pass) {
+    for (int i0 = 32 * warp; i0 < ng; i0 += 32 * nw) {
+      const int i = i0 + lane, n = n0 + i;
+      const int d = i < ng ? s_dist[i] : kFar;
+      const bool prot = i < ng && xm[n].w == 0.0f;
+      for (int g = 0; g < G; ++g) {
+        const bool a = prot && d <= G - 1 - g && (g >= n_dirty || dirty[(size_t)g * n_nodes + n]);
+        const bool b = prot && d <= G - g;
+        const unsigned ma = __ballot_sync(0xffffffffu, a), mb = __ballot_sync(0xffffffffu, b);
+        int oa = 0, ob = 0;
+        if (lane == 0) {
+          if (ma) oa = atomicAdd(&s_cnt[2 * g], __popc(ma));
+          if (mb) ob = atomicAdd(&s_cnt[2 * g + 1], __popc(mb));
+        }
+        if (pass == 0) continue;
+        oa = __shfl_sync(0xffffffffu, oa, 0);
+        ob = __shfl_sync(0xffffffffu, ob, 0);
+        if (a) rows[(size_t)(2 * g) * stride + s_base[2 * g] + oa + __popc(ma & lt)] = n;
+        if (b) rows[(size_t)(2 * g + 1) * stride + s_base[2 * g + 1] + ob + __popc(mb & lt)] = n;
+      }
+    }
+    __syncthreads();
+    if (pass == 0) {
+      for (int t = threadIdx.x; t < 2 * G; t += blockDim.x) {
+        s_base[t] = s_cnt[t] ? atomicAdd(&counts[4 * t + 2], s_cnt[t]) : 0;
+        s_cnt[t] = 0;
+      }
+      __syncthreads();
+    }
+  }
+}
+void td_launch_cone_lists(const unsigned char* rel_flag, const int* src, const int* node_ptr, const float4* xm, int n_graphs, int max_ng, int n_nodes,
+                          int k, int G, const unsigned char* dirty, int n_dirty, const int* lig_rows, int n_lig_rows, int pad, int* rows,
+                          long long stride, int* counts, cudaStream_t st) {
+  if (G <= 0) return;
+  cudaMemsetAsync(counts, 0, (size_t)G * 8 * sizeof(int), st);
+  const size_t smem = ((size_t)max_ng + 4 * (size_t)G) * sizeof(int);
+  static size_t opted[TD_MAX_DEVICES] = {0};
+  td_opt_in_smem(cone_lists_kernel, smem, opted);
+  cone_lists_kernel<<<n_graphs, CONE_THREADS, smem, st>>>(rel_flag, src, node_ptr, xm, n_nodes, k, G, max_ng, dirty, n_dirty, rows, stride, counts);
+  const int n = n_lig_rows > pad ? n_lig_rows : pad;
+  rel_rows_finish_kernel<<<dim3((n + 255) / 256, 2 * G), 256, 0, st>>>(lig_rows, n_lig_rows, pad, rows, stride, counts);
 }
 
 __global__ void dirty_propagate_kernel(const unsigned char* __restrict__ in, const int* __restrict__ src, int n_nodes, int k, unsigned char* __restrict__ out) {
diff --git a/targetdiff_b200/csrc/engine.cu b/targetdiff_b200/csrc/engine.cu
--- a/targetdiff_b200/csrc/engine.cu
+++ b/targetdiff_b200/csrc/engine.cu
@@ -87,8 +87,10 @@
   int KQ = 0, hybrid = 0;
   DevBuf node_ptr, prot_ptr, prot_node, prot_graph, lig_node, lig_graph, node_lig;
   DevBuf rel_flag, rel_list, n_rel, work_list, n_work, knn_cache;
-  DevBuf x2h_rows, lig_rows, rel_rows, rel_counts;
+  DevBuf x2h_rows, lig_rows;
   long long x2h_n_dst = 0, x2h_split = 0, lig_n_dst = 0;
+  DevBuf cone_rows, cone_counts;
+  int cone_evals = 0;
   int row_pad = 4;
   int free_depth = 0;
   int env_free_depth = 2;
@@ -566,7 +568,7 @@
   if (e->ev_fork) cudaEventDestroy(e->ev_fork);
   if (e->ev_join) cudaEventDestroy(e->ev_join);
   DevBuf* bufs[] = {&e->node_ptr, &e->prot_ptr, &e->prot_node, &e->prot_graph, &e->lig_node, &e->lig_graph, &e->node_lig, &e->xm0, &e->xm1,
-                    &e->rel_flag, &e->rel_list, &e->n_rel, &e->work_list, &e->n_work, &e->knn_cache, &e->x2h_rows, &e->lig_rows, &e->rel_rows, &e->rel_counts, &e->ew_x2h, &e->ew_h2x, &e->h_sync, &e->hagg, &e->time_norm, &e->h_free, &e->dirty, &e->free_rows, &e->free_counts, &e->lig_save, &e->offset, &e->h0, &e->h, &e->P, &e->q, &e->src, &e->src_prev, &e->etype, &e->e_w, &e->dist, &e->kbuf, &e->vbuf, &e->v16, &e->lig_pos,
+                    &e->rel_flag, &e->rel_list, &e->n_rel, &e->work_list, &e->n_work, &e->knn_cache, &e->x2h_rows, &e->lig_rows, &e->cone_rows, &e->cone_counts, &e->ew_x2h, &e->ew_h2x, &e->h_sync, &e->hagg, &e->time_norm, &e->h_free, &e->dirty, &e->free_rows, &e->free_counts, &e->lig_save, &e->offset, &e->h0, &e->h, &e->P, &e->q, &e->src, &e->src_prev, &e->etype, &e->e_w, &e->dist, &e->kbuf, &e->vbuf, &e->v16, &e->lig_pos,
                     &e->lig_v, &e->logits, &e->step, &e->err_flag, &e->node_off, &e->total_edges, &e->fix_mask, &e->fix_pos, &e->fix_v, &e->seq_buf, &e->lk_buf, &e->lk_x0, &e->lk_v0};
   for (auto* b : bufs) b->release();
   for (auto& b : e->stage) b.release();
@@ -614,7 +616,7 @@
     for (int i = 0; i < lc[g]; ++i) { lig_node[a] = n; lig_graph[a] = g; node_lig[n] = a; ++a; ++n; }
   }
   node_ptr[B] = n; prot_ptr[B] = p;
-  e->bound = false; e->has_ligand = false; e->have_graph = false; e->have_prev = false;
+  e->bound = false; e->has_ligand = false; e->have_graph = false; e->have_prev = false; e->cone_evals = 0;
   e->has_fixed = false; e->fix_pos_noise = nullptr; e->fix_v_uniform = nullptr;
   e->start_t = -1; e->start_pos_noise = nullptr; e->start_v_uniform = nullptr;
   e->B = B; e->N = (int)N; e->Np = (int)Np; e->Nl = (int)Nl; e->max_ng = max_ng;
@@ -634,8 +636,9 @@
   std::vector<int> x2h_rows((size_t)(nPpad + nLpad), -1), lig_rows((size_t)nLpad, -1);
   for (long long i = 0; i < Np; ++i) x2h_rows[i] = prot_node[i];
   for (long long i = 0; i < Nl; ++i) { x2h_rows[nPpad + i] = lig_node[i]; lig_rows[i] = lig_node[i]; }
-  if (v4) bad |= e->x2h_rows.ensure(x2h_rows.size() * 4 + 4) | e->lig_rows.ensure(lig_rows.size() * 4 + 4) | e->rel_rows.ensure(x2h_rows.size() * 4 + 4) |
-                 e->rel_counts.ensure(16);
+  const size_t x2h_evals = e->layers.size() * (size_t)e->num_x2h;
+  if (v4) bad |= e->x2h_rows.ensure(x2h_rows.size() * 4 + 4) | e->lig_rows.ensure(lig_rows.size() * 4 + 4) |
+                 e->cone_rows.ensure(2 * x2h_evals * x2h_rows.size() * 4 + 4) | e->cone_counts.ensure(2 * x2h_evals * 16 + 16);
   const bool fuse = v4 && K == 32 && !e->env_no_fused_agg && e->ew_mode != 2;
   if (e->ew_mode == 1) bad |= e->ew_x2h.ensure(slots * 4) | e->ew_h2x.ensure(slots * 4);
   if (e->out_fc) bad |= e->hagg.ensure((size_t)N * TD_H * 4);
@@ -648,8 +651,7 @@
   for (int g = 0; g < B; ++g) if (pc[g] < min_pc) min_pc = pc[g];
   e->free_ready = false;
   e->free_depth = (fuse && !e->hybrid && Nl > 0 && min_pc > K) ? e->env_free_depth : 0;
-  const int x2h_evals = (int)e->layers.size() * e->num_x2h;
-  if (e->free_depth > x2h_evals - 1) e->free_depth = x2h_evals - 1 > 0 ? x2h_evals - 1 : 0;
+  if (e->free_depth > (int)x2h_evals - 1) e->free_depth = (int)x2h_evals - 1 > 0 ? (int)x2h_evals - 1 : 0;
   if (e->free_depth > 0)
     bad |= e->h_free.ensure((size_t)e->free_depth * N * TD_H * 4) | e->dirty.ensure((size_t)e->free_depth * N + 16) |
            e->free_rows.ensure((size_t)e->free_depth * x2h_rows.size() * 4 + 4) | e->free_counts.ensure((size_t)e->free_depth * 16) |
@@ -795,22 +797,21 @@
   ~Prof() { if (on) { cudaEventRecord(ev.b, st); e->events.push_back(ev); } }
 };
 
-enum RowList { ROWS_ALL = 0, ROWS_LIGAND = 1, ROWS_RELEVANT = 2 };
+enum RowList { ROWS_ALL = 0, ROWS_LIGAND = 1 };
+struct SubRows {
+  const int* rows = nullptr;
+  const int* counts = nullptr;
+};
 bool fused_logits(const tdiff_engine* e) { return e->mlp_mode == 2 && e->mlp_v4; }
 void edge_mlp(tdiff_engine* e, const float* P, const float4* xm, const int* src, const unsigned char* etype, RowList list, int K, const TdMlp& m,
               const float* offsets, float coeff, float* out, cudaStream_t st, const float* e_w, const float* qnode = nullptr,
-              const float* agg_logits = nullptr, float* agg_h = nullptr, int key_softmax = 0, int free_layer = -1) {
+              const float* agg_logits = nullptr, float* agg_h = nullptr, int key_softmax = 0, SubRows sub = SubRows()) {
   if (fused_logits(e) && m.w2_img && m.tabcls_img) {
-    const int* rows = list == ROWS_ALL ? e->x2h_rows.as<int>() : list == ROWS_LIGAND ? e->lig_rows.as<int>() : e->rel_rows.as<int>();
-    const int* counts = list == ROWS_RELEVANT ? e->rel_counts.as<int>() : nullptr;
-    if (free_layer >= 0) {
-      rows = e->free_rows.as<int>() + (size_t)free_layer * e->free_stride;
-      counts = e->free_counts.as<int>() + 4 * free_layer;
-    }
+    const int* rows = sub.rows ? sub.rows : list == ROWS_ALL ? e->x2h_rows.as<int>() : e->lig_rows.as<int>();
     const long long n_dst = list == ROWS_LIGAND ? e->lig_n_dst : e->x2h_n_dst;
     const long long split = list == ROWS_LIGAND ? 0 : e->x2h_split;
     const int by_slot = (list != ROWS_LIGAND && !key_softmax && agg_logits == nullptr) ? 1 : 0;
-    td_launch_edge_mlp_v4(P, e->N, src, etype, e->dist.as<float>(), rows, n_dst, split, counts, K, m,
+    td_launch_edge_mlp_v4(P, e->N, src, etype, e->dist.as<float>(), rows, n_dst, split, sub.counts, K, m,
                           e->host_arena.data() + (offsets - e->arena), coeff, e->host_arena.data() + (m.ln_b - e->arena),
                           e->host_arena.data() + (m.b2 - e->arena), qnode, out, by_slot, agg_logits, e_w, agg_h, key_softmax,
                           e->sm_count, st);
@@ -824,15 +825,16 @@
     td_launch_edge_mlp(P, xm, src, etype, row_nodes, n_rows, K, m, offsets, coeff, out, e->sm_count, st);
 }
 
-void node_side(tdiff_engine* e, const float* h, int N, const TdSubLayer& sl, float* P, float* q, cudaStream_t st, const int* rows = nullptr,
-               const int* d_n = nullptr) {
+void node_side(tdiff_engine* e, const float* h, int N, const TdSubLayer& sl, float* P, float* q, cudaStream_t st, const TdRows* rows_a = nullptr,
+               const TdRows* rows_b = nullptr) {
   if (fused_logits(e) && sl.wn_img && sl.q.w2_img) {
-    td_launch_node_side_v4(h, N, sl.wn_img, sl.bn, sl.q, P, q, rows, d_n, e->sm_count, st);
+    const TdRows all = {nullptr, nullptr, N};
+    td_launch_node_side_v4(h, sl.wn_img, sl.bn, sl.q, P, q, rows_a ? *rows_a : all, rows_b ? *rows_b : all, e->sm_count, st);
   } else if (e->mlp_mode != 0 && sl.wn_img && sl.q.w2_img) {
     TdMlp pm = sl.q;
     pm.b2 = sl.bn;
-    td_launch_rows_tc(1, h, TD_H, 0, N, pm, sl.wn_img, e->mlp_mode, P, TD_NPROJ, TD_NPROJ / TD_H, rows, d_n, e->sm_count, st);
-    td_launch_rows_tc(2, P, TD_NPROJ, 512, N, sl.q, sl.q.w2_img, e->mlp_mode, q, TD_H, 1, rows, d_n, e->sm_count, st);
+    td_launch_rows_tc(1, h, TD_H, 0, N, pm, sl.wn_img, e->mlp_mode, P, TD_NPROJ, TD_NPROJ / TD_H, nullptr, nullptr, e->sm_count, st);
+    td_launch_rows_tc(2, P, TD_NPROJ, 512, N, sl.q, sl.q.w2_img, e->mlp_mode, q, TD_H, 1, nullptr, nullptr, e->sm_count, st);
   } else {
     td_launch_node_proj(h, N, sl.wn_t, sl.bn, P, st);
     td_launch_node_q(P, N, sl.q, q, st);
@@ -886,14 +888,18 @@
     }
     td_launch_rel_compact(e->rel_flag.as<unsigned char>(), N, e->rel_list.as<int>(), e->n_rel.as<int>(), st);
     e->launches += 4;
-    if (fused_logits(e) && e->restrict_last && last_blk && e->num_x2h > 0) {
-      td_launch_rel_rows(e->rel_flag.as<unsigned char>(), xm[cur], N, e->lig_rows.as<int>(), (int)e->lig_n_dst, e->row_pad, e->rel_rows.as<int>(),
-                         e->rel_counts.as<int>(), st);
-      e->launches += 2;
-    }
     const float4* xm_blk = xm[cur];
     const int NX = e->num_x2h, NH = e->num_h2x;
     const size_t L = e->layers.size();
+    const bool cone = fused_logits(e) && e->restrict_last && last_blk && NX > 0 && !e->env_no_restrict && !e->out_fc;
+    const long long cone_stride = e->free_stride;
+    if (cone) {
+      td_launch_cone_lists(e->rel_flag.as<unsigned char>(), src, e->node_ptr.as<int>(), xm_blk, e->B, e->max_ng, N, K, (int)L * NX,
+                           use_free ? e->dirty.as<unsigned char>() : nullptr, use_free, e->lig_rows.as<int>(), (int)e->lig_n_dst, e->row_pad,
+                           e->cone_rows.as<int>(), cone_stride, e->cone_counts.as<int>(), st);
+      e->launches += 2;
+      e->cone_evals = (int)L * NX;
+    }
     int g = 0;
     for (size_t l = 0; l < L && !(free_build && g >= free_build); ++l) {
       const TdLayer& ly = e->layers[l];
@@ -908,7 +914,18 @@
       for (int i = 0; i < NX && !(free_build && g >= free_build); ++i, ++g) {
         const TdSubLayer& sx = ly.x2h[i];
         const int fl = g < use_free ? g : -1;
-        node_side(e, h, N, sx, P, q, st);
+        SubRows sub;
+        TdRows rows_a = {nullptr, nullptr, N}, rows_b = {nullptr, nullptr, N};
+        if (cone) {
+          sub.rows = e->cone_rows.as<int>() + (size_t)(2 * g) * cone_stride;
+          sub.counts = e->cone_counts.as<int>() + 8 * g;
+          rows_a = {sub.rows, sub.counts, e->x2h_n_dst};
+          rows_b = {sub.rows + cone_stride, sub.counts + 4, e->x2h_n_dst};
+        } else if (fl >= 0) {
+          sub.rows = e->free_rows.as<int>() + (size_t)fl * e->free_stride;
+          sub.counts = e->free_counts.as<int>() + 4 * fl;
+        }
+        node_side(e, h, N, sx, P, q, st, &rows_a, &rows_b);
         if (e->mlp_mode != 0 && (i == 0 || e->ew_mode == 1)) {
           TdEwR ew = {nullptr, nullptr, 0.f, 0.f, ly.offsets, ly.coeff, nullptr, nullptr};
           if (e->ew_mode == 1) {
@@ -919,8 +936,6 @@
           e->launches += 1;
         }
         const bool fuse_agg = fused_logits(e) && K == 32 && !e->env_no_fused_agg && e->ew_mode != 2;
-        const bool sub = fuse_agg && e->restrict_last && last_blk && l + 1 == L && i + 1 == NX && !e->env_no_restrict && !e->out_fc;
-        const RowList rl = sub ? ROWS_RELEVANT : ROWS_ALL;
         float* agg_target = h;
         if (e->out_fc) {
           agg_target = e->hagg.as<float>();
@@ -928,16 +943,16 @@
         }
         {
           Prof pr(e, st, EV_EDGE_MLP);
-          edge_mlp(e, P, xm[cur], src, etype, rl, K, sx.k, ly.offsets, ly.coeff, e->kbuf.as<float>(), st, ew_x, fused_logits(e) ? q : nullptr, nullptr,
-                   nullptr, fuse_agg ? 1 : 0, fl);
-          edge_mlp(e, P, xm[cur], src, etype, rl, K, sx.v, ly.offsets, ly.coeff, e->vbuf.as<float>(), st, ew_x, nullptr,
-                   fuse_agg ? e->kbuf.as<float>() : nullptr, fuse_agg ? agg_target : nullptr, 0, fl);
+          edge_mlp(e, P, xm[cur], src, etype, ROWS_ALL, K, sx.k, ly.offsets, ly.coeff, e->kbuf.as<float>(), st, ew_x, fused_logits(e) ? q : nullptr,
+                   nullptr, nullptr, fuse_agg ? 1 : 0, sub);
+          edge_mlp(e, P, xm[cur], src, etype, ROWS_ALL, K, sx.v, ly.offsets, ly.coeff, e->vbuf.as<float>(), st, ew_x, nullptr,
+                   fuse_agg ? e->kbuf.as<float>() : nullptr, fuse_agg ? agg_target : nullptr, 0, sub);
         }
         if (!fuse_agg) {
           Prof pr(e, st, EV_AGG_H);
           if (fused_logits(e))
-            td_launch_aggregate_h_logits(e->kbuf.as<float>(), e->vbuf.as<float>(), ew_x, src, e->out_fc ? agg_target : h, agg_target, N, K,
-                                         e->ew_mode == 2 ? sx.ew_w : nullptr, sx.ew_b, st);
+            td_launch_aggregate_h_logits(e->kbuf.as<float>(), e->vbuf.as<float>(), ew_x, src, e->out_fc ? agg_target : h, agg_target,
+                                         sub.rows ? rows_a : TdRows{nullptr, nullptr, N}, K, e->ew_mode == 2 ? sx.ew_w : nullptr, sx.ew_b, st);
           else td_launch_aggregate_h(e->kbuf.as<float>(), e->vbuf.as<float>(), e->e_w.as<float>(), src, q, h, h, N, K, st);
         }
         e->launches += fuse_agg ? 4 : 5;
@@ -968,9 +983,11 @@
                                    ly.offsets, ly.coeff, e->ew_h2x.as<float>(), st);
           e->launches += 1;
         }
-        {
-          const bool rel = fused_logits(e) && !e->env_no_restrict;
-          node_side(e, h_h2x, N, sh, P, q, st, rel ? e->rel_list.as<int>() : nullptr, rel ? e->n_rel.as<int>() : nullptr);
+        if (fused_logits(e) && !e->env_no_restrict) {
+          const TdRows rows_a = {e->lig_node.as<int>(), nullptr, Nl}, rows_b = {e->rel_list.as<int>(), e->n_rel.as<int>(), N};
+          node_side(e, h_h2x, N, sh, P, q, st, &rows_a, &rows_b);
+        } else {
+          node_side(e, h_h2x, N, sh, P, q, st);
         }
         {
           Prof pr(e, st, EV_EDGE_MLP);
@@ -1482,6 +1499,17 @@
 }
 
 extern "C" int64_t tdiff_launch_count(tdiff_engine* e) { return e ? e->launches : 0; }
+
+extern "C" int tdiff_get_cone(tdiff_engine* e, int32_t* h_dims, int32_t* h_counts, int32_t* h_rows) {
+  if (!e || !h_dims) return set_err(TDIFF_EINVAL, "get_cone: bad arguments");
+  if (!e->bound || e->cone_evals == 0) return set_err(TDIFF_ESTATE, "get_cone: no sampling step has built the cone lists of this batch");
+  CK(cudaSetDevice(e->device));
+  const size_t G = (size_t)e->cone_evals, stride = (size_t)e->free_stride;
+  h_dims[0] = (int32_t)G; h_dims[1] = (int32_t)stride;
+  if (h_counts) CK(cudaMemcpy(h_counts, e->cone_counts.p, 2 * G * 16, cudaMemcpyDeviceToHost));
+  if (h_rows) CK(cudaMemcpy(h_rows, e->cone_rows.p, 2 * G * stride * 4, cudaMemcpyDeviceToHost));
+  return TDIFF_OK;
+}
 extern "C" int tdiff_edge_mlp_mode(tdiff_engine* e) { return !e ? TDIFF_EINVAL : (e->mlp_mode == 2 && e->mlp_v4) ? 5 : e->mlp_mode; }
 
 extern "C" int tdiff_profile(tdiff_engine* e, int enable) {
diff --git a/targetdiff_b200/csrc/node_side.cu b/targetdiff_b200/csrc/node_side.cu
--- a/targetdiff_b200/csrc/node_side.cu
+++ b/targetdiff_b200/csrc/node_side.cu
@@ -39,23 +39,23 @@
   __syncthreads();
 }
 
-struct Rows {
-  const int* list;
-  const int* d_n;
-  long long n;
-};
+using Rows = TdRows;
 
 __device__ __forceinline__ uint32_t chunk_pos(int r, int c) { return (uint32_t)(r * 512 + ((c ^ ((r & 3) << 1)) << 4)); }
 __device__ __forceinline__ void bar_sync_wg(int wg) { asm volatile("bar.sync %0, 128;" ::"r"(1 + wg) : "memory"); }
 
 __device__ __forceinline__ void load_tile_async(uint32_t buf, const float* __restrict__ in, const Rows& rw, long long n, long long tile, int t) {
   const int l = t & 31;
-#pragma unroll 1
-  for (int r = t >> 5; r < kTile; r += 4) {
-    const long long i = tile * kTile + r;
-    const long long node = i < n ? (rw.list ? (long long)rw.list[i] : i) : 0;
-    asm volatile("cp.async.cg.shared.global [%0], [%1], 16, %2;" ::"r"(buf + chunk_pos(r, l)), "l"(in + (size_t)node * TD_H + 4 * l),
-                 "r"(i < n ? 16 : 0) : "memory");
+  long long mine = -1;
+  if (l < kTile / 4) {
+    const long long i = tile * kTile + (t >> 5) + 4 * l;
+    mine = i < n ? (rw.list ? (long long)rw.list[i] : i) : -1;
+  }
+#pragma unroll 1
+  for (int r = t >> 5, j = 0; r < kTile; r += 4, ++j) {
+    const long long node = __shfl_sync(0xffffffffu, mine, j);
+    asm volatile("cp.async.cg.shared.global [%0], [%1], 16, %2;" ::"r"(buf + chunk_pos(r, l)), "l"(in + (size_t)(node >= 0 ? node : 0) * TD_H + 4 * l),
+                 "r"(node >= 0 ? 16 : 0) : "memory");
   }
   asm volatile("cp.async.commit_group;" ::: "memory");
 }
@@ -140,8 +140,9 @@
 
 __global__ void __launch_bounds__(ns::kThreads, 1)
 node_proj_kernel(const float* __restrict__ h, const unsigned char* __restrict__ wn_img, const float* __restrict__ bn, float* __restrict__ P,
-                 ns::Rows rw) {
+                 const ns::Rows rw_a, const ns::Rows rw_b) {
   using namespace ns;
+  const Rows rw = blockIdx.y ? rw_b : rw_a;
   extern __shared__ unsigned char smem_raw[];
   unsigned char* sW = reinterpret_cast<unsigned char*>((reinterpret_cast<uintptr_t>(smem_raw) + 1023) & ~(uintptr_t)1023);
   float* sBias = reinterpret_cast<float*>(sW + 2 * kBlock + kWG * kHBuf);
@@ -238,18 +239,18 @@
   }
 }
 
-void td_launch_node_side_v4(const float* h, long long n_rows, const unsigned char* wn_img, const float* bn, const TdMlp& q_mlp, float* P,
-                            float* q, const int* rows, const int* d_n, int sm_count, cudaStream_t st) {
+void td_launch_node_side_v4(const float* h, const unsigned char* wn_img, const float* bn, const TdMlp& q_mlp, float* P, float* q, const TdRows& rows_a,
+                            const TdRows& rows_b, int sm_count, cudaStream_t st) {
   using namespace ns;
-  if (n_rows == 0) return;
+  if (rows_a.n == 0 && rows_b.n == 0) return;
   static size_t opted_p[TD_MAX_DEVICES] = {0}, opted_q[TD_MAX_DEVICES] = {0};
   td_opt_in_smem(node_proj_kernel, kSmem, opted_p);
   td_opt_in_smem(node_query_kernel, kSmem, opted_q);
-  const Rows rw = {rows, d_n, n_rows};
-  const long long slots = (n_rows + kTile - 1) / kTile;
-  const long long ctas = (slots + kWG - 1) / kWG;
+  auto ctas = [](long long n_rows) { return ((n_rows + kTile - 1) / kTile + kWG - 1) / kWG; };
+  const long long cp = ctas(rows_a.n > rows_b.n ? rows_a.n : rows_b.n), cq = ctas(rows_a.n);
   const int per = sm_count / 2 > 0 ? sm_count / 2 : 1;
-  node_proj_kernel<<<dim3((unsigned)(ctas < per ? ctas : per), 2), kThreads, kSmem, st>>>(h, wn_img, bn, P, rw);
-  node_query_kernel<<<(unsigned)(ctas < sm_count ? ctas : sm_count), kThreads, kSmem, st>>>(h, wn_img + 4 * (size_t)kImgStride, bn + 512, q_mlp,
-                                                                                           q, rw);
-}
+  node_proj_kernel<<<dim3((unsigned)(cp < per ? cp : per), 2), kThreads, kSmem, st>>>(h, wn_img, bn, P, rows_a, rows_b);
+  if (cq > 0)
+    node_query_kernel<<<(unsigned)(cq < sm_count ? cq : sm_count), kThreads, kSmem, st>>>(h, wn_img + 4 * (size_t)kImgStride, bn + 512, q_mlp, q,
+                                                                                         rows_a);
+}
diff --git a/targetdiff_b200/csrc/tdiff_common.cuh b/targetdiff_b200/csrc/tdiff_common.cuh
--- a/targetdiff_b200/csrc/tdiff_common.cuh
+++ b/targetdiff_b200/csrc/tdiff_common.cuh
@@ -127,6 +127,9 @@
 void td_launch_restore_clean(const unsigned char* dirty, const float4* xm, const float* h_free, int n_nodes, float* h, cudaStream_t st);
 void td_launch_rel_rows(const unsigned char* rel_flag, const float4* xm, int n_nodes, const int* lig_rows, int n_lig_rows, int pad, int* rel_rows,
                         int* rel_counts, cudaStream_t st);
+void td_launch_cone_lists(const unsigned char* rel_flag, const int* src, const int* node_ptr, const float4* xm, int n_graphs, int max_ng, int n_nodes,
+                          int k, int G, const unsigned char* dirty, int n_dirty, const int* lig_rows, int n_lig_rows, int pad, int* rows,
+                          long long stride, int* counts, cudaStream_t st);
 void td_launch_protein_embed(const float* feat, int n_protein, int fdim, const float* w, const float* b, const int* prot_node,
                              float* h0, cudaStream_t st);
 void td_launch_init_h(const float* h0, const float4* xm, const int* lig_v, const int* node_lig, const float* wl_t, const float* bl,
@@ -150,15 +153,20 @@
                            const float* agg_logits, const float* agg_e_w, float* agg_h, int key_softmax, int sm_count, cudaStream_t st);
 void td_launch_rows_tc(int mode, const float* in, int ldi, int in_off, long long n_rows, TdMlp m, const unsigned char* w_image, int pieces, float* out,
                        int ldo, int nblocks, const int* row_list, const int* d_n_rows, int sm_count, cudaStream_t st);
-void td_launch_node_side_v4(const float* h, long long n_rows, const unsigned char* wn_img, const float* bn, const TdMlp& q_mlp, float* P,
-                            float* q, const int* rows, const int* d_n, int sm_count, cudaStream_t st);
+struct TdRows {
+  const int* list;
+  const int* d_n;
+  long long n;
+};
+void td_launch_node_side_v4(const float* h, const unsigned char* wn_img, const float* bn, const TdMlp& q_mlp, float* P, float* q, const TdRows& rows_a,
+                            const TdRows& rows_b, int sm_count, cudaStream_t st);
 void td_launch_rel_compact(const unsigned char* flag, int n_nodes, int* rel_list, int* n_rel, cudaStream_t st);
 void td_launch_aggregate_h(const float* kbuf, const float* vbuf, const float* e_w, const int* src, const float* q, const float* h_in,
                            float* h_out, int n_nodes, int k, cudaStream_t st);
 void td_launch_aggregate_x(const float* kbuf, const float* v16, const float* e_w, const int* src, const float* q, const float4* xm_in,
                            const int* row_nodes, float4* xm_out, int n_rows, int k, cudaStream_t st);
 void td_launch_aggregate_h_logits(const float* logits, const float* vbuf, const float* e_w, const int* src, const float* h_in, float* h_out,
-                                  int n_nodes, int k, const float* ewm_w, float ewm_b, cudaStream_t st);
+                                  const TdRows& dst, int k, const float* ewm_w, float ewm_b, cudaStream_t st);
 void td_launch_aggregate_x_logits(const float* logits, const float* v16, const float* e_w, const int* src, const float4* xm_in,
                                   const int* row_nodes, float4* xm_out, int n_rows, int k, cudaStream_t st);
 void td_launch_head(const float* h, const int* lig_node, int n_lig, const float* w1t, const float* b1, const float* w2, const float* b2,
```

New measurement: 19.29, median of 6. 1.04x the previous value.
